# JettHuang/jet-pbrt

Hardware: AMD Instinct MI355X
Metric: Msamples/sec (whole node) + per-pixel L2 vs CPU ref, cornell_box 1024spp (higher is better)
Workload: dtype f32

## Files before the change

### jet-pbrt_amd/csrc/jp_common.h

```cpp
#pragma once
#include "jp_shading.h"

using namespace jp;

extern __shared__ float4 s_dyn[];

#define JP_SHADE_CLASSES 6

struct DevCounters
{
	unsigned int n_queue[2];
	unsigned int n_shadow;
	unsigned int pad;
	unsigned long long closest, closest_hit, shadow, shadow_occ;
	unsigned long long cert_fallback;
};

struct Queues
{
	float4 *ray_o[2], *ray_d[2], *beta[2];
	float2 *hit;
	float4 *lacc;
	float4 *sh_o;
	float4 *sh_d, *sh_c;
	unsigned int *blk_q[2], *blk_sh;
	unsigned int cap;
	unsigned int R;
};

struct RenderConst
{
	int width, height, spp, max_depth;
	unsigned int seed;
	int band_rows, shard_index, shard_count;
	int npix;
	int local_rows;
	int s0, sbatch;
	int n_planes;
	int tiled;
	int compact;
	int slot_bits;
	int sampler_debug;
	int class_mask;
	int lane_index, lane_count, lane_rows;
};

__device__ __forceinline__ float rngf(const RenderConst& rc, uint32_t key, uint32_t dim) { return rc.sampler_debug ? 0.5f : jp_rng_float(key, dim); }

#define FLAG_BOUNCE(f) ((f) & 0xff)
#define FLAG_SPEC(f)   (((f) >> 8) & 1)
#define FLAG_DIM(f)    (((unsigned)(f)) >> 16)
#define MK_FLAGS(bounce, spec, dim) (((bounce) & 0xff) | ((spec) ? 0x100 : 0) | ((int)(dim) << 16))

__device__ __forceinline__ void pixel_of(const RenderConst& rc, int pix, int& x, int& y)
{
	int lx, r;
	if (rc.tiled)
	{
		const int t = pix >> 6, i = pix & 63, tpr = rc.width >> 4;
		const int ty = t / tpr, tx = t - ty * tpr;
		lx = (tx << 4) + (i & 15); r = (ty << 2) + (i >> 4);
	}
	else { r = pix / rc.width; lx = pix - r * rc.width; }
	x = lx;
	if (rc.lane_count > 1) { const int m = r / rc.lane_rows; r = (rc.lane_index + m * rc.lane_count) * rc.lane_rows + (r - m * rc.lane_rows); }
	const int j = r / rc.band_rows;
	y = (rc.shard_index + j * rc.shard_count) * rc.band_rows + (r - j * rc.band_rows);
}

__device__ __forceinline__ unsigned int wave_take(unsigned int* ctr, unsigned int n)
{
	unsigned int v = 0;
	if ((threadIdx.x & 63) == 0) v = atomicAdd(ctr, n);
	return (unsigned int)__builtin_amdgcn_readfirstlane((int)v);
}


#define JP_TEX_IMAGE_TAG 0x80000000u
#define JP_TEX_COLOR_TAG 0x40000000u
struct TexView
{
	const int4* desc;
	const float4* col;
	const unsigned int* texels;
	const int* mat_tex;
	const float2* prim_uv;
	unsigned int* side;
};
```

### jet-pbrt_amd/csrc/jp_device.h

```cpp
#pragma once
#include <hip/hip_runtime.h>
#include <stdint.h>
#include "jetpbrt_amd.h"
#include "jp_counter_rng.h"

#define JP_BLOCK 256
#define JP_STACK_DEPTH 32

namespace jp
{
struct V3 { float x, y, z; };
__device__ __forceinline__ V3 mk(float x, float y, float z) { V3 v; v.x = x; v.y = y; v.z = z; return v; }
__device__ __forceinline__ V3 operator+(V3 a, V3 b) { return mk(a.x + b.x, a.y + b.y, a.z + b.z); }
__device__ __forceinline__ V3 operator-(V3 a, V3 b) { return mk(a.x - b.x, a.y - b.y, a.z - b.z); }
__device__ __forceinline__ V3 operator-(V3 a) { return mk(-a.x, -a.y, -a.z); }
__device__ __forceinline__ V3 operator*(V3 a, float s) { return mk(a.x * s, a.y * s, a.z * s); }
__device__ __forceinline__ V3 operator*(float s, V3 a) { return mk(a.x * s, a.y * s, a.z * s); }
__device__ __forceinline__ V3 operator/(V3 a, float s) { return mk(a.x / s, a.y / s, a.z / s); }
__device__ __forceinline__ V3 cmul(V3 a, V3 b) { return mk(a.x * b.x, a.y * b.y, a.z * b.z); }
__device__ __forceinline__ V3 cdiv(V3 a, V3 b) { return mk(a.x / b.x, a.y / b.y, a.z / b.z); }
__device__ __forceinline__ V3 splat(float v) { return mk(v, v, v); }
__device__ __forceinline__ V3 csqrt(V3 a) { return mk(sqrtf(a.x), sqrtf(a.y), sqrtf(a.z)); }
__device__ __forceinline__ float dot(V3 a, V3 b) { return a.x * b.x + a.y * b.y + a.z * b.z; }
__device__ __forceinline__ float len2(V3 a) { return a.x * a.x + a.y * a.y + a.z * a.z; }
__device__ __forceinline__ float len(V3 a) { return sqrtf(len2(a)); }
__device__ __forceinline__ V3 normalize(V3 a) { return a / len(a); }
__device__ __forceinline__ V3 cross(V3 a, V3 v) { return mk(a.y * v.z - a.z * v.y, a.z * v.x - a.x * v.z, a.x * v.y - a.y * v.x); }
__device__ __forceinline__ float absdot(V3 a, V3 b) { return fabsf(dot(a, b)); }
__device__ __forceinline__ bool isblack(V3 c) { return c.x == 0.f && c.y == 0.f && c.z == 0.f; }
__device__ __forceinline__ float smin(float a, float b) { return (b < a) ? b : a; }
__device__ __forceinline__ float smax(float a, float b) { return (a < b) ? b : a; }
__device__ __forceinline__ float maxcomp(V3 c) { float m = (c.y < c.z) ? c.z : c.y; return (c.x < m) ? m : c.x; }
__device__ __forceinline__ float clampf(float v, float lo, float hi) { if (v < lo) return lo; else if (v > hi) return hi; else return v; }
__device__ __forceinline__ V3 xyz(float4 v) { return mk(v.x, v.y, v.z); }

#define JP_PI      3.14159274101257324219f
#define JP_INF     __int_as_float(0x7f800000)

struct SceneView
{
	const float4* nodes; int n_nodes;
	const float4* prims; const int4* meta; int n_prims;
	const float4* mats;
	const int* mat_type; int n_mats;
	const float4* lights;
	int n_lights;
	const float4* shade_tab;
	float3 env_sum;
	int n_env;
	float world_radius;
	JpCamera cam;
	const float4* flat; int n_flat;
	const uint4* wide; int n_wide;
	const uint4* q4; int n_q4;
	const float4* refbox; float cert_pad, cert_pad_eye;
};

__device__ __forceinline__ bool tri_hit(V3 p0, V3 p1, V3 p2, V3 n, V3 o, V3 d, float tmin, float& tmax)
{
	const V3 oa = p0 - o;
	const float distance = dot(n, oa) / dot(n, d);
	if (!((distance > tmin) && (distance < tmax))) return false;
	const V3 ob = p1 - o, oc = p2 - o;
	const V3 v0 = cross(oc, ob), v1 = cross(ob, oa), v2 = cross(oa, oc);
	const float v0d = dot(v0, d), v1d = dot(v1, d), v2d = dot(v2, d);
	if (((v0d < 0) && (v1d < 0) && (v2d < 0)) || ((v0d >= 0) && (v1d >= 0) && (v2d >= 0))) { tmax = distance; return true; }
	return false;
}
__device__ __forceinline__ bool rect_hit(V3 p0, V3 p1, V3 p2, V3 p3, V3 n, V3 o, V3 d, float tmin, float& tmax)
{
	const V3 oa = p0 - o;
	const float distance = dot(n, oa) / dot(n, d);
	if (!((distance > tmin) && (distance < tmax))) return false;
	const V3 ob = p1 - o, oc = p2 - o, od = p3 - o;
	const V3 v0 = cross(oc, ob), v1 = cross(ob, oa), v2 = cross(oa, od), v3 = cross(od, oc);
	const float v0d = dot(v0, d), v1d = dot(v1, d), v2d = dot(v2, d), v3d = dot(v3, d);
	if (((v0d < 0) && (v1d < 0) && (v2d < 0) && (v3d < 0)) || ((v0d >= 0) && (v1d >= 0) && (v2d >= 0) && (v3d >= 0))) { tmax = distance; return true; }
	return false;
}
__device__ __forceinline__ bool sph_hit(V3 c, float r, V3 o, V3 d, float tmin, float& tmax)
{
	V3 oc = o - c;
	float a = len2(d);
	float half_b = dot(oc, d);
	float cc = len2(oc) - r * r;
	float disc = half_b * half_b - a * cc;
	if (disc > 0.0f)
	{
		float root = sqrtf(disc);
		float time;
		float root1 = (-half_b - root) / a;
		if (root1 < tmax && root1 > tmin) time = root1;
		else
		{
			float root2 = (-half_b + root) / a;
			if (root2 < tmax && root2 > tmin) time = root2;
			else return false;
		}
		tmax = time;
		return true;
	}
	return false;
}

__device__ __forceinline__ bool disk_hit(V3 c, float r, V3 n, V3 o, V3 d, float tmin, float& tmax)
{
	const float dn = dot(d, n);
	if (fabsf(dn - 0.f) <= 1.1920928955078125e-07f * smax(1.f, smax(fabsf(dn), fabsf(0.f)))) return false;
	const V3 op = c - o;
	const float distance = dot(n, op) / dot(n, d);
	if ((distance > tmin) && (distance < tmax))
	{
		const V3 hp = o + distance * d;
		if (len(c - hp) <= r) { tmax = distance; return true; }
	}
	return false;
}

template <int kS, typename PrimPtr>
__device__ __forceinline__ bool prim_hit(PrimPtr prims, int pi, V3 o, V3 d, float tmin, float& tmax)
{
	const float4 g0 = prims[kS * pi + 0], g1 = prims[kS * pi + 1], g2 = prims[kS * pi + 2], g3 = prims[kS * pi + 3];
	const int type = __float_as_int(g3.w);
	if (type == JP_SHAPE_TRIANGLE) return tri_hit(xyz(g0), xyz(g1), xyz(g2), xyz(g3), o, d, tmin, tmax);
	if (type == JP_SHAPE_SPHERE) return sph_hit(xyz(g0), g0.w, o, d, tmin, tmax);
	if (type == JP_SHAPE_DISK) return disk_hit(xyz(g0), g0.w, xyz(g1), o, d, tmin, tmax);
	return rect_hit(xyz(g0), xyz(g1), xyz(g2), mk(g0.w, g1.w, g2.w), xyz(g3), o, d, tmin, tmax);
}

template <bool kAnyHit, int kS, typename NodePtr, typename PrimPtr>
__device__ __forceinline__ int traverse(NodePtr nodes, PrimPtr prims, V3 o, V3 d, float tmin, float& tmax, int* stack)
{
	const float ix = 1.0f / d.x, iy = 1.0f / d.y, iz = 1.0f / d.z;
	int hit = -1, sp = 0, cur = 0;
	for (;;)
	{
		bool alive = true;
		while (cur >= 0)
		{
			const float4 n0 = nodes[kS * cur + 0], n1 = nodes[kS * cur + 1], n2 = nodes[kS * cur + 2], n3 = nodes[kS * cur + 3];
			const float lx0 = (n0.x - o.x) * ix, lx1 = (n0.w - o.x) * ix;
			const float ly0 = (n0.y - o.y) * iy, ly1 = (n1.x - o.y) * iy;
			const float lz0 = (n0.z - o.z) * iz, lz1 = (n1.y - o.z) * iz;
			const float ln = fmaxf(fmaxf(fminf(lx0, lx1), fminf(ly0, ly1)), fmaxf(fminf(lz0, lz1), tmin));
			const float lf = fminf(fminf(fmaxf(lx0, lx1), fmaxf(ly0, ly1)), fminf(fmaxf(lz0, lz1), tmax));
			const float rx0 = (n1.z - o.x) * ix, rx1 = (n2.y - o.x) * ix;
			const float ry0 = (n1.w - o.y) * iy, ry1 = (n2.z - o.y) * iy;
			const float rz0 = (n2.x - o.z) * iz, rz1 = (n2.w - o.z) * iz;
			const float rn = fmaxf(fmaxf(fminf(rx0, rx1), fminf(ry0, ry1)), fmaxf(fminf(rz0, rz1), tmin));
			const float rf = fminf(fminf(fmaxf(rx0, rx1), fmaxf(ry0, ry1)), fminf(fmaxf(rz0, rz1), tmax));
			const bool hl = ln <= lf * 1.000002f, hr = rn <= rf * 1.000002f;
			const int cl = __float_as_int(n3.x), cr = __float_as_int(n3.y);
			if (hl && hr)
			{
				const bool leftFirst = kAnyHit ? true : (ln <= rn);
				cur = leftFirst ? cl : cr;
				stack[sp * JP_BLOCK] = leftFirst ? cr : cl; sp++;
			}
			else if (hl) cur = cl;
			else if (hr) cur = cr;
			else if (sp > 0) { sp--; cur = stack[sp * JP_BLOCK]; }
			else { alive = false; break; }
		}
		if (!alive) break;
		const int e = -cur - 1, first = e >> 4, count = (e & 15) + 1;
		for (int k = 0; k < count; k++)
			if (prim_hit<kS>(prims, first + k, o, d, tmin, tmax)) { hit = first + k; if (kAnyHit) return hit; }
		if (sp > 0) { sp--; cur = stack[sp * JP_BLOCK]; } else break;
	}
	return hit;
}

__device__ __forceinline__ bool ref_box_exact(float4 n0, float4 n1, V3 o, V3 d, float tmin, float tmax)
{
	float bt0 = tmin, bt1 = tmax;
	{
		const float lo = (n0.x - o.x) / d.x, hi = (n1.x - o.x) / d.x;
		bt0 = smax(smin(lo, hi), bt0); bt1 = smin(smax(lo, hi), bt1);
		if (bt1 <= bt0) return false;
	}
	{
		const float lo = (n0.y - o.y) / d.y, hi = (n1.y - o.y) / d.y;
		bt0 = smax(smin(lo, hi), bt0); bt1 = smin(smax(lo, hi), bt1);
		if (bt1 <= bt0) return false;
	}
	{
		const float lo = (n0.z - o.z) / d.z, hi = (n1.z - o.z) / d.z;
		bt0 = smax(smin(lo, hi), bt0); bt1 = smin(smax(lo, hi), bt1);
		if (bt1 <= bt0) return false;
	}
	return true;
}
__device__ __forceinline__ bool ref_box(float4 n0, float4 n1, V3 o, V3 d, V3 rd, float tmin, float tmax)
{
	const float x0 = (n0.x - o.x) * rd.x, x1 = (n1.x - o.x) * rd.x;
	const float y0 = (n0.y - o.y) * rd.y, y1 = (n1.y - o.y) * rd.y;
	const float z0 = (n0.z - o.z) * rd.z, z1 = (n1.z - o.z) * rd.z;
	const float t0 = fmaxf(fmaxf(fminf(x0, x1), fminf(y0, y1)), fmaxf(fminf(z0, z1), tmin));
	const float t1 = fminf(fminf(fmaxf(x0, x1), fmaxf(y0, y1)), fminf(fmaxf(z0, z1), tmax));
	const float s = x0 + x1 + y0 + y1 + z0 + z1;
	const float margin = 2e-6f * (fabsf(t0) + fabsf(t1));
	const float gap = t1 - t0;
	if (fabsf(s) <= 3.0e38f && fabsf(gap) > margin) return gap > 0.f;
	return ref_box_exact(n0, n1, o, d, tmin, tmax);
}

template <bool kAnyHit>
__device__ __forceinline__ int traverse_ref(const float4* __restrict__ nodes, const float4* __restrict__ prims, V3 o, V3 d, float tmin, float& tmax, int* stack)
{
	const V3 rd = mk(__builtin_amdgcn_rcpf(d.x), __builtin_amdgcn_rcpf(d.y), __builtin_amdgcn_rcpf(d.z));
	int hit = -1, sp = 0, cur = 0;
	for (;;)
	{
		const float4 n0 = nodes[2 * cur], n1 = nodes[2 * cur + 1];
		const bool ok = ref_box(n0, n1, o, d, rd, tmin, tmax);
		const int left = __float_as_int(n0.w), right = __float_as_int(n1.w);
		if (ok && left >= 0) { stack[sp * JP_BLOCK] = right; sp++; cur = left; continue; }
		if (ok)
		{
			const int first = -left - 1;
			for (int k = 0; k < right; k++)
				if (prim_hit<4>(prims, first + k, o, d, tmin, tmax)) { hit = first + k; if (kAnyHit) return hit; }
		}
		if (sp == 0) break;
		sp--; cur = stack[sp * JP_BLOCK];
	}
	return hit;
}

typedef const __attribute__((address_space(4))) float* ConstFPtr;
typedef unsigned long long u64;
template <bool k64> struct FlatMask { typedef unsigned int type; };
template <> struct FlatMask<true> { typedef u64 type; };
template <bool k64> __device__ __forceinline__ int mask_count(typename FlatMask<k64>::type m) { return k64 ? __popcll((u64)m) : __popc((unsigned int)m); }

template <bool k64>
__device__ __forceinline__ typename FlatMask<k64>::type flat_boxes(const float4* flat_g, int n_flat, V3 o, V3 d, float tmin, float tmax)
{
	typedef typename FlatMask<k64>::type M;
	ConstFPtr flat = (ConstFPtr)flat_g;
	const float ix = __builtin_amdgcn_rcpf(d.x), iy = __builtin_amdgcn_rcpf(d.y), iz = __builtin_amdgcn_rcpf(d.z);
	M mask = 0;
	#define JP_FLAT_BOX(i) \
	{ \
		const float x0 = (flat[8 * (i) + 0] - o.x) * ix, x1 = (flat[8 * (i) + 4] - o.x) * ix; \
		const float y0 = (flat[8 * (i) + 1] - o.y) * iy, y1 = (flat[8 * (i) + 5] - o.y) * iy; \
		const float z0 = (flat[8 * (i) + 2] - o.z) * iz, z1 = (flat[8 * (i) + 6] - o.z) * iz; \
		const float tn = fmaxf(fmaxf(fminf(x0, x1), fminf(y0, y1)), fmaxf(fminf(z0, z1), tmin)); \
		const float tf = fminf(fminf(fmaxf(x0, x1), fmaxf(y0, y1)), fminf(fmaxf(z0, z1), tmax)); \
		M bits = (M)__float_as_uint(flat[8 * (i) + 3]); \
		if (k64) bits |= (M)((u64)__float_as_uint(flat[8 * (i) + 7]) << 32); \
		if (tn <= tf * 1.000002f) mask |= bits; \
	}
	int i0 = 0;
	for (; i0 + 4 <= n_flat; i0 += 4)
	{
		#pragma unroll
		for (int u = 0; u < 4; u++) JP_FLAT_BOX(i0 + u)
	}
	for (; i0 < n_flat; i0++) JP_FLAT_BOX(i0)
	#undef JP_FLAT_BOX
	return mask;
}

template <bool kAnyHit, bool k64, int kS, typename PrimPtr>
__device__ __forceinline__ int flat_prims(typename FlatMask<k64>::type mask, PrimPtr prims, V3 o, V3 d, float tmin, float& tmax)
{
	int hit = -1;
#ifdef JP_DBG_FLAT_P1ONLY
	mask = mask == (typename FlatMask<k64>::type)0x12345677u ? 1u : 0u;
#endif
	while (mask)
	{
		const int p = (k64 ? __ffsll((unsigned long long)mask) : __ffs((int)mask)) - 1;
		mask &= mask - 1;
		if (prim_hit<kS>(prims, p, o, d, tmin, tmax)) { hit = p; if (kAnyHit) return hit; }
	}
	return hit;
}

template <bool kAnyHit, int kS, typename PrimPtr>
__device__ __forceinline__ int traverse_flat(const float4* flat_g, int n_flat, int n_prims, PrimPtr prims, V3 o, V3 d, float tmin, float& tmax)
{
	if (n_prims > 32) return flat_prims<kAnyHit, true, kS>(flat_boxes<true>(flat_g, n_flat, o, d, tmin, tmax), prims, o, d, tmin, tmax);
	return flat_prims<kAnyHit, false, kS>(flat_boxes<false>(flat_g, n_flat, o, d, tmin, tmax), prims, o, d, tmin, tmax);
}

template <bool kAnyHit, typename PrimPtr>
__device__ __forceinline__ int traverse_wide(const uint4* __restrict__ wide, PrimPtr prims, V3 o, V3 d, float tmin, float& tmax, unsigned int* stack)
{
	const float ix = 1.0f / d.x, iy = 1.0f / d.y, iz = 1.0f / d.z;
	const unsigned int octinv = 7u - ((d.x < 0 ? 1u : 0u) | (d.y < 0 ? 2u : 0u) | (d.z < 0 ? 4u : 0u));
	unsigned int ngx = 0, ngy = 0x80000000u;
	int hit = -1, sp = 0;
	for (;;)
	{
		unsigned int tgx = 0, tgy = 0;
		if (ngy > 0x00ffffffu)
		{
			const unsigned int bit = 31u - (unsigned int)__clz((int)ngy);
			ngy &= ~(1u << bit);
			if (ngy > 0x00ffffffu) { stack[(2 * sp) * JP_BLOCK] = ngx; stack[(2 * sp + 1) * JP_BLOCK] = ngy; sp++; }
			const unsigned int slot = (bit - 24u) ^ octinv;
			const unsigned int rel = (unsigned int)__popc(ngy & 0xffu & ~(0xffffffffu << slot));
			const unsigned int idx = ngx + rel;
			const uint4 q0 = wide[5 * idx + 0], q1 = wide[5 * idx + 1], q2 = wide[5 * idx + 2], q3 = wide[5 * idx + 3], q4 = wide[5 * idx + 4];
			const float sx = __uint_as_float(((q0.w & 0xffu) ) << 23), sy = __uint_as_float(((q0.w >> 8) & 0xffu) << 23), sz = __uint_as_float(((q0.w >> 16) & 0xffu) << 23);
			const float px = __uint_as_float(q0.x) - o.x, py = __uint_as_float(q0.y) - o.y, pz = __uint_as_float(q0.z) - o.z;
			unsigned int hm = 0;
			#pragma unroll
			for (int i = 0; i < 8; i++)
			{
				const int sh = 8 * (i & 3);
				const unsigned int m = ((i < 4 ? q1.z : q1.w) >> sh) & 0xffu;
				const float lx = (float)(((i < 4 ? q2.x : q2.y) >> sh) & 0xffu), ly = (float)(((i < 4 ? q2.z : q2.w) >> sh) & 0xffu), lz = (float)(((i < 4 ? q3.x : q3.y) >> sh) & 0xffu);
				const float hx = (float)(((i < 4 ? q3.z : q3.w) >> sh) & 0xffu), hy = (float)(((i < 4 ? q4.x : q4.y) >> sh) & 0xffu), hz = (float)(((i < 4 ? q4.z : q4.w) >> sh) & 0xffu);
				const float x0 = fmaf(lx, sx, px) * ix, x1 = fmaf(hx, sx, px) * ix;
				const float y0 = fmaf(ly, sy, py) * iy, y1 = fmaf(hy, sy, py) * iy;
				const float z0 = fmaf(lz, sz, pz) * iz, z1 = fmaf(hz, sz, pz) * iz;
				const float tn = fmaxf(fmaxf(fminf(x0, x1), fminf(y0, y1)), fmaxf(fminf(z0, z1), tmin));
				const float tf = fminf(fminf(fmaxf(x0, x1), fmaxf(y0, y1)), fminf(fmaxf(z0, z1), tmax));
				if (m != 0u && tn <= tf * 1.000002f)
				{
					const bool inner = (m & 0x18u) == 0x18u;
					const unsigned int bits = inner ? 1u : (m >> 5), at = inner ? 24u + ((m & 7u) ^ octinv) : (m & 31u);
					hm |= bits << at;
				}
			}
			ngx = q1.x; ngy = (hm & 0xff000000u) | (q0.w >> 24);
			tgx = q1.y; tgy = hm & 0x00ffffffu;
		}
		while (tgy)
		{
			const int j = __ffs((int)tgy) - 1;
			tgy &= tgy - 1;
			if (prim_hit<4>(prims, (int)tgx + j, o, d, tmin, tmax)) { hit = (int)tgx + j; if (kAnyHit) return hit; }
		}
		if (ngy <= 0x00ffffffu)
		{
			if (sp == 0) break;
			sp--; ngx = stack[(2 * sp) * JP_BLOCK]; ngy = stack[(2 * sp + 1) * JP_BLOCK];
		}
	}
	return hit;
}

struct WalkStack
{
	int* lds; int* spill; int cap; unsigned int stride;
// ... 276 lines not shown
```

### jet-pbrt_amd/csrc/jp_kernels.hip

```cpp
#include "jp_common.h"
#include "jp_tex.h"
#include "jp_xbsdf.h"

#include <cstdio>
#include <cstring>
#include <string>
#include <vector>
#include <algorithm>
#include <cmath>
#include <mutex>
#include <thread>
#include "jp_lbvh.h"
#include "jp_ploc.h"

__global__ void __launch_bounds__(JP_BLOCK) k_raygen(SceneView sc, Queues q, RenderConst rc, DevCounters* cnt)
{
	const unsigned int total = (unsigned int)rc.npix * rc.sbatch;
	const unsigned int nchunks = (total + JP_BLOCK - 1) / JP_BLOCK;
	const unsigned int G = gridDim.x, b = blockIdx.x;
	if (b == 0 && threadIdx.x == 0) { cnt->n_queue[0] = total; cnt->n_queue[1] = 0; cnt->n_shadow = 0; }
	unsigned int filled = 0;
	const unsigned int K = (nchunks + G - 1) / G, npb = (unsigned int)rc.npix / JP_BLOCK;
	for (unsigned int k = 0, j0 = 0; k < K; k++, j0 += JP_BLOCK)
	{
		unsigned int c;
		if (rc.compact) { const unsigned int qi = b * K + k; if (qi >= nchunks) break; const unsigned int pb = qi / (unsigned int)rc.sbatch, sl = qi - pb * (unsigned int)rc.sbatch; c = sl * npb + pb; }
		else { c = b + k * G; if (c >= nchunks) break; }
		const unsigned int slot = c * JP_BLOCK + threadIdx.x;
		if (slot < total)
		{
			const unsigned int i = b * q.R + j0 + threadIdx.x;
			const int pix = slot % rc.npix, s = rc.s0 + slot / rc.npix;
			int x, y; pixel_of(rc, pix, x, y);
			const uint32_t key = jp_rng_key(rc.seed, (uint32_t)x, (uint32_t)y, (uint32_t)s);
			const float fx = (float)x + rngf(rc, key, 0), fy = (float)y + rngf(rc, key, 1);
			const V3 front = mk(sc.cam.front[0], sc.cam.front[1], sc.cam.front[2]);
			const V3 right = mk(sc.cam.right[0], sc.cam.right[1], sc.cam.right[2]);
			const V3 up = mk(sc.cam.up[0], sc.cam.up[1], sc.cam.up[2]);
			V3 dir = front + right * (fx / sc.cam.res_x - 0.5f) + up * (0.5f - fy / sc.cam.res_y);
			dir = normalize(dir);
			q.ray_o[0][i] = make_float4(sc.cam.pos[0], sc.cam.pos[1], sc.cam.pos[2], __int_as_float((int)slot));
			q.ray_d[0][i] = make_float4(dir.x, dir.y, dir.z, __int_as_float(MK_FLAGS(0, 0, 2)));
			q.beta[0][i] = make_float4(1.f, 1.f, 1.f, __int_as_float((int)key));
			q.lacc[slot] = make_float4(0.f, 0.f, 0.f, 0.f);
		}
		const unsigned int left = total - c * JP_BLOCK;
		filled += left < JP_BLOCK ? left : JP_BLOCK;
	}
	if (threadIdx.x == 0) q.blk_q[0][b] = filled;
}


#if defined(JP_SHADE_TIMING) || defined(JP_TRAV_TIMING)
__device__ unsigned long long g_shade_t[16];
#define JP_TSX(i) do { const unsigned long long t_ = __builtin_amdgcn_s_memtime(); t_acc[i] += t_ - t_last; t_last = t_; } while (0)
#endif
#ifdef JP_SHADE_TIMING
#define JP_TS(i) JP_TSX(i)
#else
#define JP_TS(i) do { } while (0)
#endif
#ifdef JP_TRAV_TIMING
#define JP_TT(i) JP_TSX(i)
#else
#define JP_TT(i) do { } while (0)
#endif
template <int kMode>
struct SceneAccess;
template <> struct SceneAccess<0>
{
	const float4 *nodes, *prims; int* stack; int depth;
	__device__ __forceinline__ SceneAccess(const SceneView& sc, int depth_) : nodes(sc.nodes), prims(sc.prims), stack((int*)s_dyn + threadIdx.x), depth(depth_) {}
	template <bool kAnyHit> __device__ __forceinline__ int trace(const SceneView&, V3 o, V3 d, float tmin, float& tmax) const
	{ return traverse<kAnyHit, 4>(nodes, prims, o, d, tmin, tmax, stack); }
};
template <> struct SceneAccess<1>
{
	float4 *nodes, *prims; int* stack; int depth;
	__device__ __forceinline__ SceneAccess(const SceneView& sc, int depth_) : depth(depth_)
	{
		stack = (int*)s_dyn + threadIdx.x;
		nodes = s_dyn + (depth * JP_BLOCK) / 4;
		prims = nodes + 5 * sc.n_nodes;
		for (int i = threadIdx.x; i < 4 * sc.n_nodes; i += JP_BLOCK) nodes[5 * (i >> 2) + (i & 3)] = sc.nodes[i];
		for (int i = threadIdx.x; i < 4 * sc.n_prims; i += JP_BLOCK) prims[5 * (i >> 2) + (i & 3)] = sc.prims[i];
		__syncthreads();
	}
	template <bool kAnyHit> __device__ __forceinline__ int trace(const SceneView&, V3 o, V3 d, float tmin, float& tmax) const
	{ return traverse<kAnyHit, 5>(nodes, prims, o, d, tmin, tmax, stack); }
};
template <> struct SceneAccess<2>
{
	float4* prims;
	__device__ __forceinline__ SceneAccess(const SceneView& sc, int)
	{
		prims = s_dyn;
		for (int i = threadIdx.x; i < 4 * sc.n_prims; i += JP_BLOCK) prims[5 * (i >> 2) + (i & 3)] = sc.prims[i];
		__syncthreads();
	}
	template <bool kAnyHit> __device__ __forceinline__ int trace(const SceneView& sc, V3 o, V3 d, float tmin, float& tmax) const
	{ return traverse_flat<kAnyHit, 5>(sc.flat, sc.n_flat, sc.n_prims, prims, o, d, tmin, tmax); }
};

template <> struct SceneAccess<3>
{
	const float4* prims; unsigned int* stack;
	__device__ __forceinline__ SceneAccess(const SceneView& sc, int) : prims(sc.prims), stack((unsigned int*)s_dyn + threadIdx.x) {}
	template <bool kAnyHit> __device__ __forceinline__ int trace(const SceneView& sc, V3 o, V3 d, float tmin, float& tmax) const
	{ return traverse_wide<kAnyHit>(sc.wide, prims, o, d, tmin, tmax, stack); }
};

template <> struct SceneAccess<4>
{
	WalkStack stack;
	__device__ __forceinline__ SceneAccess(const SceneView&, int depth) { stack.lds = (int*)s_dyn + threadIdx.x; stack.spill = nullptr; stack.cap = depth - 1; stack.stride = 0; }
	template <bool kAnyHit> __device__ __forceinline__ int trace(const SceneView& sc, V3 o, V3 d, float tmin, float& tmax) const
	{ return walk_ray<4, kAnyHit>(sc, o, d, tmin, tmax, stack); }
};

template <> struct SceneAccess<6>
{
	WalkStack stack;
	__device__ __forceinline__ SceneAccess(const SceneView&, int depth) { stack.lds = (int*)s_dyn + threadIdx.x; stack.spill = nullptr; stack.cap = depth - 1; stack.stride = 0; }
	template <bool kAnyHit> __device__ __forceinline__ int trace(const SceneView& sc, V3 o, V3 d, float tmin, float& tmax) const
	{ return walk_ray<6, kAnyHit>(sc, o, d, tmin, tmax, stack); }
};

template <> struct SceneAccess<5>
{
	const float4 *nodes, *prims; int* stack;
	__device__ __forceinline__ SceneAccess(const SceneView& sc, int) : nodes(sc.nodes), prims(sc.prims), stack((int*)s_dyn + threadIdx.x) {}
	template <bool kAnyHit> __device__ __forceinline__ int trace(const SceneView&, V3 o, V3 d, float tmin, float& tmax) const
	{ return traverse_ref<kAnyHit>(nodes, prims, o, d, tmin, tmax, stack); }
};

template <int kMode>
__global__ void __launch_bounds__(JP_BLOCK) k_extend(SceneView sc, Queues q, int cur, int depth, DevCounters* cnt)
{
	SceneAccess<kMode> acc(sc, depth);
	const unsigned int b = blockIdx.x, n = q.blk_q[cur][b], rbase = b * q.R;
	if (b == 0 && threadIdx.x == 0) { cnt->closest += cnt->n_queue[cur]; cnt->n_queue[cur ^ 1] = 0; cnt->n_shadow = 0; }
	unsigned int h = 0;
	float4 ro = make_float4(0, 0, 0, 0), rd = make_float4(0, 0, 1, 0);
	if (threadIdx.x < n) { ro = q.ray_o[cur][rbase + threadIdx.x]; rd = q.ray_d[cur][rbase + threadIdx.x]; }
	for (unsigned int j = threadIdx.x; j < n; j += JP_BLOCK)
	{
		const unsigned int i = rbase + j;
		const float4 co = ro, cd = rd;
		if (j + JP_BLOCK < n) { ro = q.ray_o[cur][i + JP_BLOCK]; rd = q.ray_d[cur][i + JP_BLOCK]; }
		float tmax = JP_INF;
		const int hit = acc.template trace<false>(sc, xyz(co), xyz(cd), 0.001f, tmax);
		q.hit[i] = make_float2(tmax, __int_as_float(hit));
		h += hit >= 0 ? 1u : 0u;
	}
	for (int off = 32; off > 0; off >>= 1) h += __shfl_down(h, off);
	if ((threadIdx.x & 63) == 0 && h) atomicAdd(&cnt->closest_hit, (unsigned long long)h);
}

#ifndef JP_SHADE_TILE
#define JP_SHADE_TILE 8192
#endif
template <bool kTab, bool kPrims, bool kStage, bool kSort, bool kTex>
__device__ __forceinline__ void shade_body(SceneView sc, Queues q, RenderConst rc, int cur, DevCounters* cnt, const TexView& tv)
{
	static_assert(kTab || !kPrims, "k_shade: primitive records in LDS only together with the tables");
	constexpr int kWaves = JP_BLOCK / 64, kMaxSeg = (JP_SHADE_TILE / JP_BLOCK) * kWaves;
	static_assert(JP_SHADE_TILE % JP_BLOCK == 0 && JP_SHADE_TILE <= 65536, "k_shade: tile positions are 16-bit");
	__shared__ unsigned short s_idx[kSort ? JP_SHADE_TILE : 1];
	__shared__ unsigned char s_key[kSort ? JP_SHADE_TILE : 1];
	__shared__ unsigned int s_cnt[kSort ? JP_SHADE_CLASSES * kMaxSeg : 1];
	__shared__ unsigned int s_wsum[kWaves];
	__shared__ unsigned int s_ctr[3];
	const unsigned int lane = threadIdx.x & 63u;
	const int n_tab = 2 * sc.n_lights + 4 * sc.n_mats + (sc.n_mats + 3) / 4, n_tab_all = n_tab + (kPrims ? 8 * sc.n_prims : 0);
	float4* s_lights = s_dyn;
	float4* s_mats = s_lights + 2 * sc.n_lights;
	int* s_mtype = (int*)(s_mats + 4 * sc.n_mats);
	float4* s_prims = s_dyn + n_tab;
	int4* s_meta = (int4*)(s_prims + 4 * sc.n_prims);
	const float4* s_frames = s_prims + 5 * sc.n_prims;
	float4* s_stage = s_dyn + n_tab_all + threadIdx.x;
	const unsigned int b = blockIdx.x, n = q.blk_q[cur][b];
	const int nxt = cur ^ 1;
#ifdef JP_SHADE_TIMING
	unsigned long long t_acc[10] = { 0, 0, 0, 0, 0, 0, 0, 0, 0, 0 }, t_last = __builtin_amdgcn_s_memtime();
#endif
	if (kTab)
	{
		for (int i = threadIdx.x; i < n_tab_all; i += 2 * JP_BLOCK)
		{
			const bool two = i + JP_BLOCK < n_tab_all;
			const float4 a = sc.shade_tab[i], c2 = two ? sc.shade_tab[i + JP_BLOCK] : a;
			s_dyn[i] = a; if (two) s_dyn[i + JP_BLOCK] = c2;
		}
	}
	if (n == 0) { if (threadIdx.x == 0) { q.blk_q[nxt][b] = 0; q.blk_sh[b] = 0; } return; }
	if (threadIdx.x == 0) { s_ctr[0] = 0; s_ctr[1] = 0; s_ctr[2] = 0; }
	__syncthreads();
	const float4* lights = kTab ? (const float4*)s_lights : sc.lights;
	const float4* mats = kTab ? (const float4*)s_mats : sc.mats;
	const int* mat_type = kTab ? (const int*)s_mtype : sc.mat_type;
	const float4* prims = kPrims ? (const float4*)s_prims : sc.prims;
	const int4* meta_t = kPrims ? (const int4*)s_meta : sc.meta;
	const unsigned int rbase = b * q.R;
	const unsigned int t0 = 0, count = n;
	JP_TS(0);
	if (kSort)
	{
		constexpr unsigned int seg = kMaxSeg, nctr = JP_SHADE_CLASSES * kMaxSeg;
		const unsigned int tid = threadIdx.x;
		const unsigned int plane = tid & 63u, wave = tid >> 6, npass = (count + JP_BLOCK - 1) / JP_BLOCK;
		const unsigned long long ltm = (1ull << plane) - 1ull;
		#pragma unroll 1
		for (unsigned int r0 = 0; r0 < npass; r0 += 8)
		{
			int pi[8];
			#pragma unroll
			for (int u = 0; u < 8; u++)
			{
				const unsigned int j = (r0 + u) * JP_BLOCK + tid;
				pi[u] = j < count ? __float_as_int(q.hit[rbase + t0 + j].y) : -2;
			}
			#pragma unroll
			for (int u = 0; u < 8; u++)
			{
				const unsigned int r = r0 + u;
				if (r >= npass) break;
				unsigned int key = JP_SHADE_CLASSES;
				if (pi[u] != -2)
				{
					int m = -1; if (pi[u] >= 0) m = meta_t[pi[u]].y;
					key = m >= 0 ? 1u + (unsigned int)mat_type[m] : 0u;
				}
				s_key[r * JP_BLOCK + tid] = (unsigned char)key;
				unsigned int mine = 0;
				#pragma unroll
				for (int c = 0; c < JP_SHADE_CLASSES; c++)
				{
					unsigned int nc = 0;
					if ((rc.class_mask >> c) & 1) nc = (unsigned int)__popcll(__ballot(key == (unsigned int)c));
					if (plane == (unsigned int)c) mine = nc;
				}
				if (plane < JP_SHADE_CLASSES) s_cnt[plane * seg + r * kWaves + wave] = mine;
			}
		}
		__syncthreads();
		{
			static_assert(JP_SHADE_CLASSES * kMaxSeg <= 3 * JP_BLOCK, "k_shade: three counters per thread");
			unsigned int v[3], t = 0;
			#pragma unroll
			for (int i = 0; i < 3; i++)
			{
				const unsigned int at = 3 * tid + i;
				v[i] = (at < nctr && (at % seg) / kWaves < npass) ? s_cnt[at] : 0u; t += v[i];
			}
			unsigned int incl = t;
			#pragma unroll
			for (int off = 1; off < 64; off <<= 1) { const unsigned int o = __shfl_up(incl, off); if (plane >= (unsigned int)off) incl += o; }
			if (plane == 63) s_wsum[wave] = incl;
			__syncthreads();
			unsigned int base = incl - t;
			#pragma unroll
			for (int w = 0; w < kWaves; w++) if ((unsigned int)w < wave) base += s_wsum[w];
			#pragma unroll
			for (int i = 0; i < 3; i++) { const unsigned int at = 3 * tid + i; if (at < nctr) s_cnt[at] = base; base += v[i]; }
		}
		__syncthreads();
		#pragma unroll 1
		for (unsigned int r = 0; r < npass; r++)
		{
			const unsigned int key = s_key[r * JP_BLOCK + tid];
			unsigned int pre = 0;
			#pragma unroll
			for (int c = 0; c < JP_SHADE_CLASSES; c++)
			{
				if (!((rc.class_mask >> c) & 1)) continue;
				const unsigned long long m = __ballot(key == (unsigned int)c);
				if (key == (unsigned int)c) pre = (unsigned int)__popcll(m & ltm);
			}
			if (key < JP_SHADE_CLASSES) s_idx[s_cnt[key * seg + r * kWaves + wave] + pre] = (unsigned short)(r * JP_BLOCK + tid);
		}
		__syncthreads();
	}
	float4 ro_n = make_float4(0, 0, 0, 0), rd_n = ro_n, rb_n = ro_n; float2 h_n = make_float2(0, 0); unsigned int s_n = 0;
	JP_TS(1);
	const unsigned int nch = (count + 63u) >> 6;
	unsigned int tk = wave_take(&s_ctr[0], 1u);
	unsigned int c0 = (nch - 1u - tk) << 6;
	if (tk < nch && c0 + lane < count) { const unsigned int pos = c0 + lane, i0 = rbase + t0 + (kSort ? (unsigned int)s_idx[pos] : pos); ro_n = q.ray_o[cur][i0]; rd_n = q.ray_d[cur][i0]; rb_n = q.beta[cur][i0]; h_n = q.hit[i0]; if (kTex) s_n = tv.side[i0]; }
	while (tk < nch)
	{
		const bool valid = c0 + lane < count;
#ifdef JP_SHADE_TIMING
		JP_TS(2);
		asm volatile("s_waitcnt vmcnt(0)" ::: "memory");
		JP_TS(3);
#endif
#ifdef JP_SHADE_NO_PREFETCH
		if (valid) { const unsigned int pos = c0 + lane, i0 = rbase + t0 + (kSort ? (unsigned int)s_idx[pos] : pos); ro_n = q.ray_o[cur][i0]; rd_n = q.ray_d[cur][i0]; rb_n = q.beta[cur][i0]; h_n = q.hit[i0]; if (kTex) s_n = tv.side[i0]; }
		const float4 ro = ro_n, rd = rd_n, rb = rb_n; const float2 h = h_n; const unsigned int sw = s_n;
		tk = wave_take(&s_ctr[0], 1u); c0 = (nch - 1u - tk) << 6;
#else
		const float4 ro = ro_n, rd = rd_n, rb = rb_n; const float2 h = h_n; const unsigned int sw = s_n;
		tk = wave_take(&s_ctr[0], 1u); c0 = (nch - 1u - tk) << 6;
		if (tk < nch && c0 + lane < count)
		{
			const unsigned int pos = c0 + lane;
			const unsigned int i1 = rbase + t0 + (kSort ? (unsigned int)s_idx[pos] : pos);
			ro_n = q.ray_o[cur][i1]; rd_n = q.ray_d[cur][i1]; rb_n = q.beta[cur][i1]; h_n = q.hit[i1]; if (kTex) s_n = tv.side[i1];
		}
#endif
		bool shaded = false, wantNee = false, alive = false;
		V3 o = mk(0, 0, 0), d = mk(0, 0, 1), beta = mk(0, 0, 0), p = mk(0, 0, 0), N = mk(0, 0, 1);
		int slot = 0, bounce = 0; bool spec = false; unsigned int dim = 0; uint32_t key = 0;
		Closure c; c.kind = CL_LAMBERT; Frame fr; fr.s = fr.t = fr.n = mk(0, 0, 1);
		if (valid)
		{
			o = xyz(ro); d = xyz(rd); beta = xyz(rb);
			slot = __float_as_int(ro.w); key = (uint32_t)__float_as_int(rb.w);
			const int flags = __float_as_int(rd.w);
			bounce = FLAG_BOUNCE(flags); spec = FLAG_SPEC(flags); dim = FLAG_DIM(flags);
			const int pi = __float_as_int(h.y);
			const bool found = pi >= 0;
			int mat = -1, hitprim = 0; bool nflip = false, tabframe = kPrims;
			V3 Le = splat(0);
			if (found)
			{
				const float4 g3 = prims[4 * pi + 3];
				const int4 meta = meta_t[pi];
				const int type = __float_as_int(g3.w);
				p = o + h.x * d;
				if (type == JP_SHAPE_TRIANGLE) N = xyz(g3);
				else if (type == JP_SHAPE_RECTANGLE) { nflip = !(dot(xyz(g3), d) <= 0); N = nflip ? -xyz(g3) : xyz(g3); }
				else if (type == JP_SHAPE_DISK) N = xyz(prims[4 * pi + 1]);
				else { const float4 g0 = prims[4 * pi]; N = normalize(p - xyz(g0)); tabframe = false; }
				hitprim = pi;
				mat = meta.y;
				if (meta.z >= 0 && (bounce == 0 || spec))
				{
					const V3 wo = -d;
					if (dot(N, wo) > 0.f) Le = xyz(lights[2 * meta.z]);
				}
			}
			else if (bounce == 0 || spec)
			{
				for (int li = 0; li < sc.n_lights; li++)
				{
					const float4 l0 = lights[2 * li];
					if (__float_as_int(l0.w) == JP_LIGHT_ENVIRONMENT && !isblack(xyz(l0)))
					{
						float4 L = q.lacc[slot];
						V3 a = mk(L.x, L.y, L.z) + cmul(beta, xyz(l0));
						q.lacc[slot] = make_float4(a.x, a.y, a.z, 0.f);
					}
				}
			}
			if (!isblack(Le))
			{
				float4 L = q.lacc[slot];
				V3 a = mk(L.x, L.y, L.z) + cmul(beta, Le);
				q.lacc[slot] = make_float4(a.x, a.y, a.z, 0.f);
			}
			if (found && bounce < rc.max_depth)
			{
				if (mat < 0) alive = true;
				else
				{
					float up = 0.f;
					const int mtype = mat_type[mat];
					if (mtype == JP_MAT_PLASTIC) up = rngf(rc, key, dim++);
					if (kTex && sw != 0u) make_closure_tex(mats, mtype, mat, up, tex_color(tv, sw), c);
					else make_closure(mats, mtype, mat, up, c);
#ifdef JP_DBG_SKIP_FRAME
					fr.n = N; fr.s = mk(N.y, N.z, N.x); fr.t = mk(N.z, N.x, N.y);
#else
					if (kPrims && tabframe)
					{
						const float4 fn = s_frames[3 * hitprim], fs = s_frames[3 * hitprim + 1], ft = s_frames[3 * hitprim + 2];
						fr.n = nflip ? -xyz(fn) : xyz(fn); fr.s = xyz(fs); fr.t = nflip ? -xyz(ft) : xyz(ft);
					}
					else fr = frame_from_z(N);
#endif
					shaded = true;
					wantNee = !is_delta(c);
#ifdef JP_DBG_SKIP_NEE
					wantNee = false;
#endif
				}
			}
		}
		JP_TS(4);
		unsigned int qs = 0;
		if (!kStage)
		{
			const unsigned long long mn = __ballot(wantNee);
			if (mn) qs = rbase + wave_take(&s_ctr[2], (unsigned int)__popcll(mn)) + (unsigned int)__popcll(mn & ((1ull << lane) - 1ull));
		}
		V3 nd = d, nbeta = beta; int nbounce = bounce; bool nspec = spec;
		V3 wo = mk(0, 0, 1);
		int k = 0;
		if (shaded)
		{
			const V3 wo_w = -d;
			wo = to_local(fr, wo_w);
			closure_set_wo(c, wo);
			if (wantNee)
			{
				for (int li = 0; li < sc.n_lights; li++)
				{
					const unsigned int d0 = dim; dim += 2;
					const float4 lrad = lights[2 * li];
					if (isblack(xyz(lrad))) continue;
					const float ux = rngf(rc, key, d0), uy = rngf(rc, key, d0 + 1);
					LightSample ls = sample_li(sc, prims, lights, li, p, N, ux, uy);
					if (isblack(ls.Li) || ls.pdf == 0.f) continue;
					const V3 f = eval_local(c, wo, to_local(fr, ls.wi));
					if (isblack(f)) continue;
					const V3 sdir = __float_as_int(lrad.w) == JP_LIGHT_AREA ? ls.wi : normalize(ls.pos - p);
					const float dist = ls.dist >= 0.f ? ls.dist : len(p - ls.pos);
					const V3 contrib = cmul(cmul(beta, f), ls.Li) * absdot(ls.wi, N) / ls.pdf;
					if (k < rc.n_planes)
					{
						if (kStage)
						{
							s_stage[(2 * k) * JP_BLOCK] = make_float4(sdir.x, sdir.y, sdir.z, dist - 0.001f);
							s_stage[(2 * k + 1) * JP_BLOCK] = make_float4(contrib.x, contrib.y, contrib.z, 0.f);
						}
						else
						{
							q.sh_d[(size_t)k * q.cap + qs] = make_float4(sdir.x, sdir.y, sdir.z, dist - 0.001f);
							q.sh_c[(size_t)k * q.cap + qs] = make_float4(contrib.x, contrib.y, contrib.z, 0.f);
						}
						k++;
					}
				}
				if (!kStage) q.sh_o[qs] = make_float4(p.x, p.y, p.z, __int_as_float(slot | (k << rc.slot_bits)));
			}
		}
		JP_TS(5);
#ifdef JP_DBG_SKIP_SAMPLE
		if (false)
#else
		if (shaded)
#endif
		{
			const float ux = rngf(rc, key, dim), uy = rngf(rc, key, dim + 1); dim += 2;
			BsdfSample bs = sample_local(c, wo, ux, uy);
			bs.wi = to_world(fr, bs.wi);
			if (!(isblack(bs.f) || bs.pdf == 0.f))
			{
				nspec = (bs.flags & BS_SPECULAR) != 0;
				if (bounce >= 3)
				{
					const float qq = smax(0.05f, 1 - maxcomp(bs.f));
					const float ur = rngf(rc, key, dim++);
					if (!(ur < qq))
					{
						nbeta = cmul(beta, bs.f * absdot(bs.wi, N) / (bs.pdf * (1 - qq)));
						alive = true;
					}
				}
				else
				{
					nbeta = cmul(beta, bs.f * absdot(bs.wi, N) / bs.pdf);
					alive = true;
				}
				nd = bs.wi; nbounce = bounce + 1;
			}
		}
		JP_TS(6);
		unsigned int j = 0;
		const unsigned long long lt = (1ull << lane) - 1ull;
		const unsigned long long ma = __ballot(alive);
		if (kStage)
		{
			const unsigned long long ms = __ballot(k > 0);
			if (ma | ms)
			{
				const unsigned int base = wave_take(&s_ctr[1], (unsigned int)__popcll(ma) | ((unsigned int)__popcll(ms) << 16));
				j = rbase + (base & 0xffffu) + (unsigned int)__popcll(ma & lt);
				qs = rbase + (base >> 16) + (unsigned int)__popcll(ms & lt);
			}
			if (k > 0)
			{
				q.sh_o[qs] = make_float4(p.x, p.y, p.z, __int_as_float(slot | (k << rc.slot_bits)));
				for (int kk = 0; kk < k; kk++)
				{
					q.sh_d[(size_t)kk * q.cap + qs] = s_stage[(2 * kk) * JP_BLOCK];
					q.sh_c[(size_t)kk * q.cap + qs] = s_stage[(2 * kk + 1) * JP_BLOCK];
				}
			}
		}
		else if (ma) j = rbase + wave_take(&s_ctr[1], (unsigned int)__popcll(ma)) + (unsigned int)__popcll(ma & lt);
		if (alive)
		{
			q.ray_o[nxt][j] = make_float4(p.x, p.y, p.z, __int_as_float(slot));
			q.ray_d[nxt][j] = make_float4(nd.x, nd.y, nd.z, __int_as_float(MK_FLAGS(nbounce, nspec, dim)));
			q.beta[nxt][j] = make_float4(nbeta.x, nbeta.y, nbeta.z, __int_as_float((int)key));
		}
		JP_TS(7);
#ifdef JP_SHADE_TIMING
		asm volatile("s_waitcnt vmcnt(0)" ::: "memory");
		JP_TS(9);
#endif
	}
	JP_TS(2);
	__syncthreads();
	JP_TS(8);
#ifdef JP_SHADE_TIMING
	if (lane == 0) for (int i = 0; i < 10; i++) atomicAdd(&g_shade_t[i], t_acc[i]);
	if (lane == 0) atomicAdd(&g_shade_t[15], 1ull);
#endif
	if (threadIdx.x == 0)
	{
		const unsigned int run_q = kStage ? (s_ctr[1] & 0xffffu) : s_ctr[1], run_sh = kStage ? (s_ctr[1] >> 16) : s_ctr[2];
		q.blk_q[nxt][b] = run_q; q.blk_sh[b] = run_sh;
		if (run_q) atomicAdd(&cnt->n_queue[nxt], run_q);
		if (run_sh) atomicAdd(&cnt->n_shadow, run_sh);
	}
}
template <bool kTab, bool kPrims, bool kStage, bool kSort>
__global__ void __launch_bounds__(JP_BLOCK) k_shade(SceneView sc, Queues q, RenderConst rc, int cur, DevCounters* cnt)
{
	const TexView tv = {};
	shade_body<kTab, kPrims, kStage, kSort, false>(sc, q, rc, cur, cnt, tv);
}

template <int kMode>
__global__ void __launch_bounds__(JP_BLOCK, 4) k_shadow(SceneView sc, Queues q, RenderConst rc, int depth, DevCounters* cnt)
{
#ifdef JP_TRAV_TIMING
	unsigned long long t_acc[10] = { 0, 0, 0, 0, 0, 0, 0, 0, 0, 0 }, t_last = __builtin_amdgcn_s_memtime();
#endif
	SceneAccess<kMode> acc(sc, depth);
	const unsigned int b = blockIdx.x, E = q.blk_sh[b], rbase = b * q.R;
	JP_TT(0);
	unsigned int rays = 0, occ = 0;
	float4 so_n = make_float4(0, 0, 0, 0), sd_n = make_float4(0, 0, 1, 0);
	if (threadIdx.x < E) { so_n = q.sh_o[rbase + threadIdx.x]; sd_n = q.sh_d[rbase + threadIdx.x]; }
	for (unsigned int j = threadIdx.x; j < E; j += JP_BLOCK)
	{
		const unsigned int e = rbase + j;
#ifdef JP_TRAV_TIMING
		JP_TT(1);
		asm volatile("s_waitcnt vmcnt(0)" ::: "memory");
		JP_TT(2);
#endif
		const float4 so = so_n; float4 sd = sd_n;
		if (j + JP_BLOCK < E) { so_n = q.sh_o[e + JP_BLOCK]; sd_n = q.sh_d[e + JP_BLOCK]; }
		const int packed = __float_as_int(so.w);
		const int slot = packed & ((1 << rc.slot_bits) - 1), n = (int)((unsigned int)packed >> rc.slot_bits);
		if (n == 0) continue;
		bool any = false;
		const float4 L = q.lacc[slot];
		V3 a = mk(L.x, L.y, L.z);
		for (int k = 0; k < n; k++)
		{
			const float4 c4 = q.sh_c[(size_t)k * q.cap + e];
			float tmax = sd.w;
			const V3 dir = xyz(sd);
			if (k + 1 < n) sd = q.sh_d[(size_t)(k + 1) * q.cap + e];
			JP_TT(3);
#ifdef JP_TRAV_TIMING
			int hit;
			if constexpr (kMode == 2)
			{
				const unsigned int m = flat_boxes<false>(sc.flat, sc.n_flat, xyz(so), dir, 0.001f, tmax);
				JP_TT(4);
				hit = flat_prims<true, false, 5>(m, acc.prims, xyz(so), dir, 0.001f, tmax);
				JP_TT(5);
			}
			else hit = acc.template trace<true>(sc, xyz(so), dir, 0.001f, tmax);
#else
			const int hit = acc.template trace<true>(sc, xyz(so), dir, 0.001f, tmax);
#endif
			rays++;
			if (hit >= 0) occ++;
			else { a = a + xyz(c4); any = true; }
			JP_TT(6);
		}
		if (any) q.lacc[slot] = make_float4(a.x, a.y, a.z, 0.f);
		JP_TT(7);
	}
#ifdef JP_TRAV_TIMING
	JP_TT(1);
	if ((threadIdx.x & 63) == 0) { for (int i = 0; i < 8; i++) atomicAdd(&g_shade_t[i], t_acc[i]); atomicAdd(&g_shade_t[15], 1ull); }
#endif
	for (int off = 32; off > 0; off >>= 1) { rays += __shfl_down(rays, off); occ += __shfl_down(occ, off); }
	if ((threadIdx.x & 63) == 0) { if (rays) atomicAdd(&cnt->shadow, (unsigned long long)rays); if (occ) atomicAdd(&cnt->shadow_occ, (unsigned long long)occ); }
}

template <int kMode, bool kAnyHit, bool kVote>
__device__ __forceinline__ void persist_turn(Walker<kMode>& w, const SceneView& sc, const WalkStack& stack, bool pool)
{
	const int nh = __popcll(__ballot(!w.done && w.heavy())), nl = __popcll(__ballot(!w.done && !w.heavy()));
	const bool heavyTurn = kVote ? nh > nl : w.heavy();
	if (kVote) { JP_TURN(heavyTurn ? 3 : 0, 1); JP_TURN(heavyTurn ? 4 : 1, heavyTurn ? nh : nl); JP_TURN(heavyTurn ? 5 : 2, nh + nl); if (!pool) { JP_TURN(8, 1); JP_TURN(9, nh + nl); JP_TURN(10, heavyTurn ? nh : nl); } }
	if (!w.done && (w.heavy() == heavyTurn)) w.template step<kAnyHit>(sc, stack);
}
__device__ __forceinline__ unsigned int lane_rank(unsigned long long m) { return __builtin_amdgcn_mbcnt_hi((unsigned int)(m >> 32), __builtin_amdgcn_mbcnt_lo((unsigned int)m, 0u)); }

#ifndef JP_CERT_WAVES
#define JP_CERT_WAVES 8
#endif
template <int kMode, int kRefill, bool kVote>
__global__ void __launch_bounds__(JP_BLOCK, (kMode == 6 ? JP_CERT_WAVES : 8)) k_extend_persist(SceneView sc, Queues q, int cur_q, int stack_cap, int* spill, DevCounters* cnt)
{
	__shared__ unsigned int s_next;
	const WalkStack stack = { (int*)s_dyn + threadIdx.x, spill + blockIdx.x * JP_BLOCK + threadIdx.x, (kMode == 4 || kMode == 6) ? stack_cap - 1 : stack_cap, gridDim.x * JP_BLOCK };
	const unsigned int b = blockIdx.x, n = q.blk_q[cur_q][b], rbase = b * q.R;
	if (b == 0 && threadIdx.x == 0) { cnt->closest += cnt->n_queue[cur_q]; cnt->n_queue[cur_q ^ 1] = 0; cnt->n_shadow = 0; }
	if (threadIdx.x == 0) s_next = 0;
	__syncthreads();
	const int lane = threadIdx.x & 63;
	Walker<kMode> w; w.done = true; w.hit = -1; w.tmax = JP_INF;
	unsigned int ridx = 0xffffffffu, h = 0;
	bool pool = n > 0;
	for (;;)
	{
		const unsigned long long idle = __ballot(w.done);
		const int nidle = __popcll(idle);
		if (nidle == 64 || (pool && nidle >= kRefill))
		{
			if (w.done && ridx != 0xffffffffu)
			{
				int hp = w.hit;
				if constexpr (kMode == 6) { if (!w.certain(sc)) hp = -2; }
				q.hit[rbase + ridx] = make_float2(w.tmax, __int_as_float(hp)); h += hp >= 0 ? 1u : 0u; ridx = 0xffffffffu;
			}
			if (!pool) break;
			const int first = __ffsll((long long)idle) - 1;
			unsigned int start = 0;
			if (lane == first) start = atomicAdd(&s_next, (unsigned int)nidle);
			start = __shfl(start, first);
			{ constexpr bool kAnyHit = false; (void)kAnyHit; JP_TURN(6, 1); JP_TURN(7, nidle); }
			pool = start + (unsigned int)nidle < n;
			if (w.done)
			{
				const unsigned int my = start + lane_rank(idle);
				if (my < n)
				{
					const float4 ro = q.ray_o[cur_q][rbase + my], rd = q.ray_d[cur_q][rbase + my];
					w.start(xyz(ro), xyz(rd), 0.001f, JP_INF);
					if constexpr (kMode == 6) w.mark_origin(sc);
					ridx = my;
				}
			}
			if (start >= n && nidle == 64) break;
			continue;
		}
		persist_turn<kMode, false, kVote>(w, sc, stack, pool);
	}
	if constexpr (kMode == 6)
	{
		__syncthreads();
		for (unsigned int i = threadIdx.x; i < n; i += JP_BLOCK)
		{
			if (__float_as_int(q.hit[rbase + i].y) != -2) continue;
			const float4 ro = q.ray_o[cur_q][rbase + i], rd = q.ray_d[cur_q][rbase + i];
			float tm = JP_INF;
// ... 395 lines not shown
```

### jet-pbrt_amd/csrc/jp_render.h

```cpp
#pragma once
namespace
{
enum { CLS_EXTEND = 0, CLS_SHADE = 1, CLS_SHADOW = 2, CLS_OTHER = 3, CLS_PATH = 4 };

int ensure_queues(JpContext* c, unsigned int cap, int planes, unsigned int nblocks)
{
	if (c->cap >= cap && c->planes_alloc >= planes && c->blk_alloc >= nblocks) return JP_OK;
	cap = std::max(cap, c->cap); planes = std::max(planes, c->planes_alloc); nblocks = std::max(nblocks, c->blk_alloc);
	free_queues(c); c->blk_alloc = 0;
	auto alloc = [&](void** p, size_t bytes) -> bool { if (hipMalloc(p, bytes) != hipSuccess) return false; c->qbufs.push_back(*p); return true; };
	Queues& q = c->q; bool ok = true;
	for (int b = 0; b < 2 && ok; b++) ok = alloc((void**)&q.ray_o[b], (size_t)cap * 16) && alloc((void**)&q.ray_d[b], (size_t)cap * 16) && alloc((void**)&q.beta[b], (size_t)cap * 16)
	                                       && alloc((void**)&q.blk_q[b], (size_t)nblocks * 4);
	ok = ok && alloc((void**)&q.hit, (size_t)cap * 8) && alloc((void**)&q.lacc, (size_t)cap * 16) && alloc((void**)&q.sh_o, (size_t)cap * 16)
	     && alloc((void**)&q.sh_d, (size_t)cap * 16 * planes) && alloc((void**)&q.sh_c, (size_t)cap * 16 * planes) && alloc((void**)&q.blk_sh, (size_t)nblocks * 4);
	if (!ok) { free_queues(c); return fail(JP_ERR_DEVICE, "jp_render: out of device memory for the path queues"); }
	c->cap = cap; c->planes_alloc = planes; c->blk_alloc = nblocks;
	return JP_OK;
}

struct Stamper
{
	JpContext* c; int cls; size_t a;
	Stamper(JpContext* c, int cls) : c(c), cls(cls), a(0)
	{
		if (!c->profiling) return;
		if (c->evused + 2 > c->evpool.size()) { size_t old = c->evpool.size(); c->evpool.resize(old + 64); for (size_t i = old; i < c->evpool.size(); i++) hipEventCreate(&c->evpool[i]); }
		a = c->evused; c->evused += 2;
		hipEventRecord(c->evpool[a], c->stream);
	}
	~Stamper() { if (!c->profiling) return; hipEventRecord(c->evpool[a + 1], c->stream); JpContext::Stamp s = { cls, a, a + 1 }; c->stamps.push_back(s); }
};

struct Shard { int band, count, index, local_rows, lane_rows; };
int shard_of(const JpRenderParams* rp, Shard& s, int lane_index = 0, int lane_count = 1, int lane_group = 4)
{
	if (rp->width <= 0 || rp->height <= 0 || rp->spp <= 0 || rp->max_depth < 0 || rp->max_depth > 200) return fail(JP_ERR_INVALID_ARGUMENT, "jp_render: bad width/height/spp/max_depth");
	if (rp->integrator < JP_INTEGRATOR_PATH || rp->integrator > JP_INTEGRATOR_DEBUG_NORMAL) return fail(JP_ERR_INVALID_ARGUMENT, "jp_render: unknown integrator");
	if (rp->integrator == JP_INTEGRATOR_WHITTED && rp->max_depth > JP_WHITTED_MAX_DEPTH) return fail(JP_ERR_UNSUPPORTED, "jp_render: the Whitted integrator supports max_depth <= 16");
	if (rp->sampler_mode != JP_SAMPLER_COUNTER && rp->sampler_mode != JP_SAMPLER_DEBUG) return fail(JP_ERR_UNSUPPORTED, "jp_render: the device path implements the counter sampler only (the sequential mt19937_64 stream is not reproducible in parallel)");
	s.band = rp->band_rows > 0 ? rp->band_rows : 20;
	s.count = rp->shard_count > 1 ? rp->shard_count : 1;
	s.index = s.count > 1 ? rp->shard_index : 0;
	if (s.index < 0 || s.index >= s.count) return fail(JP_ERR_INVALID_ARGUMENT, "jp_render: shard_index out of range");
	const int nbands = (rp->height + s.band - 1) / s.band;
	s.local_rows = 0;
	for (int b = s.index; b < nbands; b += s.count) s.local_rows += std::min(s.band, rp->height - b * s.band);
	s.lane_rows = 0;
	for (int g0 = lane_index * lane_group; g0 < s.local_rows; g0 += lane_count * lane_group) s.lane_rows += std::min(lane_group, s.local_rows - g0);
	return JP_OK;
}

inline bool refill_walks(const ScenePlan& p) { return p.persist && (p.trav_mode == 0 || p.trav_mode == 3 || p.trav_mode == 5); }
inline int refill_row(const ScenePlan& p) { return p.persist >= 32 ? 2 : (p.persist >= 16 ? 1 : 0); }
inline int extend_depth(const ScenePlan& p) { return (p.trav_mode == 5 ? p.cert : p.use_q4) ? p.stack_depth_q4 : p.stack_depth; }
inline int shadow_depth(const ScenePlan& p) { return (p.trav_mode == 5 ? p.cert : p.q4_shadow) ? p.stack_depth_q4 : (p.trav_mode == 3 ? (int)(p.lds_bytes_shadow / (JP_BLOCK * sizeof(int))) : p.stack_depth); }
inline int deepest_walk(const ScenePlan& p) { return std::max(std::max(p.stack_depth, p.stack_depth_q4), p.trav_mode == 3 ? (int)(p.lds_bytes_shadow / (JP_BLOCK * sizeof(int))) : 0); }
inline size_t spill_need(const ScenePlan& p, int deep, unsigned int G) { return deep >= p.stack_lds_words ? (size_t)(deep - p.stack_lds_words + 1) * G * JP_BLOCK : 1; }

typedef void (*ExtendKernel)(SceneView, Queues, int, int, DevCounters*);
typedef void (*ExtendRefillKernel)(SceneView, Queues, int, int, int*, DevCounters*);
struct ExtendLaunch { ExtendRefillKernel refill; ExtendKernel plain; size_t lds; int words; };
template <int M> ExtendRefillKernel extend_refill(const ScenePlan& p)
{
	static const ExtendRefillKernel k[3][2] = { { k_extend_persist<M, 8, false>, k_extend_persist<M, 8, true> }, { k_extend_persist<M, 16, false>, k_extend_persist<M, 16, true> }, { k_extend_persist<M, 32, false>, k_extend_persist<M, 32, true> } };
	return k[refill_row(p)][p.vote];
}
ExtendLaunch extend_kernel(const ScenePlan& p)
{
	if (!refill_walks(p)) return { nullptr, p.trav_mode == 5 ? k_extend<5> : (p.trav_mode == 2 ? k_extend<2> : (p.trav_mode == 1 ? k_extend<1> : k_extend<0>)), p.lds_bytes, p.stack_depth };
	const int words = std::min(extend_depth(p), p.stack_lds_words);
	const ExtendRefillKernel k = p.trav_mode == 5 ? (p.cert ? extend_refill<6>(p) : extend_refill<5>(p)) : (p.use_q4 ? extend_refill<4>(p) : extend_refill<0>(p));
	return { k, nullptr, (size_t)words * JP_BLOCK * sizeof(int), words };
}

typedef void (*ShadowKernel)(SceneView, Queues, RenderConst, int, DevCounters*);
typedef void (*ShadowRefillKernel)(SceneView, Queues, RenderConst, int, int*, DevCounters*);
struct ShadowLaunch { ShadowRefillKernel refill; ShadowKernel plain; size_t lds; int words; bool cert_fell_back; };
template <int M> ShadowRefillKernel shadow_refill(const ScenePlan& p)
{
	static const ShadowRefillKernel k[3][2] = { { k_shadow_persist<M, 8, false>, k_shadow_persist<M, 8, true> }, { k_shadow_persist<M, 16, false>, k_shadow_persist<M, 16, true> }, { k_shadow_persist<M, 32, false>, k_shadow_persist<M, 32, true> } };
	return k[refill_row(p)][p.vote];
}
ShadowLaunch shadow_kernel(const ScenePlan& p, unsigned int R)
{
	const int words = std::min(shadow_depth(p), p.stack_lds_words);
	const size_t plds = (size_t)words * JP_BLOCK * sizeof(int) + (((size_t)R * p.n_planes + 31) / 32) * 4 * (p.cert ? 2 : 1);
	if (!refill_walks(p) || plds > 64 * 1024)
		return { nullptr, p.trav_mode == 3 ? k_shadow<3> : (p.trav_mode == 5 ? k_shadow<5> : (p.trav_mode == 2 ? k_shadow<2> : (p.trav_mode == 1 ? k_shadow<1> : k_shadow<0>))), p.trav_mode == 3 ? p.lds_bytes_shadow : p.lds_bytes, p.stack_depth, p.cert };
	const ShadowRefillKernel k = p.trav_mode == 5 ? (p.cert ? shadow_refill<6>(p) : shadow_refill<5>(p)) : (p.q4_shadow ? shadow_refill<4>(p) : (p.trav_mode == 3 ? shadow_refill<3>(p) : shadow_refill<0>(p)));
	return { k, nullptr, plds, words, false };
}

typedef void (*ShadeKernel)(SceneView, Queues, RenderConst, int, DevCounters*);
typedef void (*ShadeTexKernel)(SceneView, Queues, RenderConst, int, DevCounters*, TexView);
struct ShadeKernels { ShadeKernel plain; ShadeTexKernel tex; };
template <bool kTab, bool kPrims, bool kStage> ShadeKernels shade_row(bool sort)
{
	ShadeKernels k = { sort ? k_shade<kTab, kPrims, kStage, true> : k_shade<kTab, kPrims, kStage, false>, sort ? k_shade_tex<kTab, kPrims, kStage, true> : k_shade_tex<kTab, kPrims, kStage, false> };
	return k;
}
ShadeKernels shade_kernels(const ScenePlan& p)
{
	if (p.shade_prims_in_lds) return p.stage_nee ? shade_row<true, true, true>(p.shade_sort) : shade_row<true, true, false>(p.shade_sort);
	if (p.tables_in_lds) return p.stage_nee ? shade_row<true, false, true>(p.shade_sort) : shade_row<true, false, false>(p.shade_sort);
	return shade_row<false, false, false>(p.shade_sort);
}

typedef void (*OtherKernel)(SceneView, Queues, RenderConst, int, int, DevCounters*);
OtherKernel other_kernel(const ScenePlan& p) { return p.trav_mode == 5 ? k_other<5> : (p.trav_mode == 2 ? k_other<2> : (p.trav_mode == 1 ? k_other<1> : k_other<0>)); }

typedef void (*TraceKernel)(SceneView, int, int, const float*, const float*, const float*, const float*, int*, float*, int*, float*);
typedef void (*SurfaceKernel)(SceneView, TexView, int, int, const float*, const float*, const float*, const float*, int*, float*, float*);
struct TraceLaunch { TraceKernel trace; SurfaceKernel surface; size_t lds; int depth; };
template <int M> TraceLaunch trace_row(size_t lds, int depth) { TraceLaunch t = { k_trace<M>, k_surface<M>, lds, depth }; return t; }
TraceLaunch trace_kernel(const ScenePlan& p, int tw)
{
	const size_t q4lds = (size_t)p.stack_depth_q4 * JP_BLOCK * sizeof(int);
	if (p.trav_mode == 3 && tw == 2) { TraceLaunch t = { k_trace<3>, nullptr, p.lds_bytes_shadow, p.stack_depth }; return t; }
	if (p.trav_mode == 5 && p.cert && q4lds <= 64 * 1024 && tw != 3) return trace_row<6>(q4lds, p.stack_depth_q4);
	if (p.trav_mode == 5) return trace_row<5>(p.lds_bytes, p.stack_depth);
	if (p.use_q4 && q4lds <= 64 * 1024 && tw != 1) return trace_row<4>(q4lds, p.stack_depth_q4);
	return p.trav_mode == 2 ? trace_row<2>(p.lds_bytes, p.stack_depth) : (p.trav_mode == 1 ? trace_row<1>(p.lds_bytes, p.stack_depth) : trace_row<0>(p.lds_bytes, p.stack_depth));
}

int render_one(JpContext* c, const JpRenderParams* rp, float* film_dev, bool sync, int lane_index = 0, int lane_count = 1, int lane_group = 4, bool ev0_recorded = false)
{
	if (!c->plan.have_scene) return fail(JP_ERR_NO_SCENE, "jp_render: no scene uploaded");
	const ScenePlan& p = c->plan; Shard sh;
	if (const int e = shard_of(rp, sh, lane_index, lane_count, lane_group); e != JP_OK) return e;
	HIP_TRY(hipSetDevice(c->device));
	const long long npix = (long long)sh.lane_rows * rp->width;

	if (!ev0_recorded) HIP_TRY(hipEventRecord(c->ev0, c->stream));
	HIP_TRY(hipMemsetAsync(film_dev, 0, sizeof(float) * 3 * (size_t)rp->width * rp->height, c->stream));
	HIP_TRY(hipMemsetAsync(c->d_cnt, 0, sizeof(DevCounters), c->stream));
	c->evused = 0; c->stamps.clear();
	unsigned long long samples = 0;
	if (npix > 0)
	{
		if (npix > (1 << 24)) return fail(JP_ERR_UNSUPPORTED, "jp_render: more than 2^24 pixels per shard");
		const int slot_bits = p.n_planes <= 31 ? 27 : 24;
		const unsigned int PMAX = slot_bits == 27 ? (1u << 26) : (1u << 24);
		size_t freeB = 0, totalB = 0; hipMemGetInfo(&freeB, &totalB);
		const size_t per = 136 + 32 * (size_t)p.n_planes;
		size_t budget = std::min<size_t>((size_t)24 << 30, (freeB / (size_t)std::max(1, lane_count) + (c->cap ? (size_t)c->cap * (136 + 32 * (size_t)c->planes_alloc) : 0)) / 2);
		if (c->opt.max_slots > 0) budget = std::min<size_t>(budget, (size_t)c->opt.max_slots * per);
		int sbatch = 1; unsigned int P = 0, G = 1, R = JP_BLOCK, cap = 0;
		for (int attempt = 0;; attempt++)
		{
			const unsigned int pcap = (unsigned int)std::min<size_t>(PMAX, std::max<size_t>((size_t)npix, budget / per));
			sbatch = (int)std::max<long long>(1, std::min<long long>(rp->spp, pcap / npix));
			{
				const int nb = (rp->spp + sbatch - 1) / sbatch;
				sbatch = (rp->spp + nb - 1) / nb;
			}
			if ((long long)sbatch * npix > (long long)PMAX) return fail(JP_ERR_UNSUPPORTED, "jp_render: shard too large for one batch");
			P = (unsigned int)((long long)sbatch * npix);
			const unsigned int nchunks = (P + JP_BLOCK - 1) / JP_BLOCK;
			G = std::max(1u, std::min(nchunks, (unsigned int)(c->n_cus * c->blocks_per_cu)));
			G = std::max(G, (nchunks + JP_SHADE_TILE / JP_BLOCK - 1) / (JP_SHADE_TILE / JP_BLOCK));
			R = ((nchunks + G - 1) / G) * JP_BLOCK;
			cap = G * R;
			const int st = ensure_queues(c, cap, p.n_planes, G);
			if (st == JP_OK) break;
			if (sbatch <= 1 || attempt >= 6) return st;
			budget = (size_t)sbatch / 2 * (size_t)npix * per;
		}
		c->q.cap = cap; c->q.R = R;
		const bool tex = p.textured && rp->integrator == JP_INTEGRATOR_PATH;
		if (tex && c->side_n < cap)
		{
			if (c->d_side) { HIP_TRY(hipStreamSynchronize(c->stream)); hipFree(c->d_side); } c->d_side = nullptr; c->side_n = 0;
			HIP_TRY(hipMalloc((void**)&c->d_side, (size_t)cap * sizeof(unsigned int))); c->side_n = cap;
		}
		TexView tv = p.tv; tv.side = c->d_side;
		const size_t need = spill_need(p, p.persist ? deepest_walk(p) : 0, G);
		if (c->spill_words < need) { if (c->d_spill) hipFree(c->d_spill); c->d_spill = nullptr; HIP_TRY(hipMalloc((void**)&c->d_spill, need * sizeof(int))); c->spill_words = need; }
		if (c->pix_acc_n < (size_t)npix) { if (c->d_pix_acc) hipFree(c->d_pix_acc); c->d_pix_acc = nullptr; HIP_TRY(hipMalloc((void**)&c->d_pix_acc, (size_t)npix * 16)); c->pix_acc_n = (size_t)npix; }

		RenderConst rc; rc.width = rp->width; rc.height = rp->height; rc.spp = rp->spp; rc.max_depth = rp->max_depth; rc.seed = rp->seed;
		rc.band_rows = sh.band; rc.shard_index = sh.index; rc.shard_count = sh.count; rc.npix = (int)npix; rc.local_rows = sh.lane_rows; rc.n_planes = p.n_planes;
		rc.lane_index = lane_index; rc.lane_count = lane_count; rc.lane_rows = lane_group; rc.class_mask = p.class_mask; rc.sampler_debug = rp->sampler_mode == JP_SAMPLER_DEBUG ? 1 : 0;
		rc.slot_bits = slot_bits;
		rc.tiled = 0;
		rc.compact = (p.trav_mode != 2 && p.trav_mode != 1 && npix % JP_BLOCK == 0) ? 1 : 0;
		if (c->opt.compact_regions != 0) rc.compact = (c->opt.compact_regions > 0 && npix % JP_BLOCK == 0) ? 1 : 0;
		const int grid = (int)G;
		const ExtendLaunch ek = extend_kernel(p); const ShadowLaunch sk = shadow_kernel(p, R); const ShadeKernels hk = shade_kernels(p); const OtherKernel ok = other_kernel(p);
		for (int s0 = 0; s0 < rp->spp; s0 += sbatch)
		{
			rc.s0 = s0; rc.sbatch = std::min(sbatch, rp->spp - s0);
			{ Stamper t(c, CLS_OTHER); hipLaunchKernelGGL(k_raygen, dim3(grid), dim3(JP_BLOCK), 0, c->stream, p.sv, c->q, rc, c->d_cnt); }
			if (rp->integrator != JP_INTEGRATOR_PATH)
			{
				Stamper t(c, CLS_OTHER);
				const int ogrid = (int)std::min<unsigned int>((P + JP_BLOCK - 1) / JP_BLOCK, (unsigned int)(c->n_cus * 16));
				hipLaunchKernelGGL(ok, dim3(ogrid), dim3(JP_BLOCK), p.lds_bytes, c->stream, p.sv, c->q, rc, rp->integrator, p.stack_depth, c->d_cnt);
			}
			int cur = 0;
			int iters = rp->integrator != JP_INTEGRATOR_PATH ? 0 : rp->max_depth + 1;
			for (int it = 0;; it++)
			{
				if (it >= iters)
				{
					if (rp->integrator != JP_INTEGRATOR_PATH || !p.has_null_material || it > iters + 64) break;
					DevCounters h; HIP_TRY(hipMemcpyAsync(&h, c->d_cnt, sizeof(h), hipMemcpyDeviceToHost, c->stream)); HIP_TRY(hipStreamSynchronize(c->stream));
					if (h.n_queue[cur] == 0) break;
				}
				{
					Stamper t(c, CLS_EXTEND);
					if (ek.refill) hipLaunchKernelGGL(ek.refill, dim3(grid), dim3(JP_BLOCK), ek.lds, c->stream, p.sv, c->q, cur, ek.words, c->d_spill, c->d_cnt);
					else hipLaunchKernelGGL(ek.plain, dim3(grid), dim3(JP_BLOCK), ek.lds, c->stream, p.sv, c->q, cur, ek.words, c->d_cnt);
				}
				{
					Stamper t(c, CLS_SHADE);
					if (tex)
					{
						hipLaunchKernelGGL(k_texel, dim3(grid), dim3(JP_BLOCK), 0, c->stream, p.sv, c->q, cur, tv);
						hipLaunchKernelGGL(hk.tex, dim3(grid), dim3(JP_BLOCK), p.shade_lds_bytes, c->stream, p.sv, c->q, rc, cur, c->d_cnt, tv);
					}
					else hipLaunchKernelGGL(hk.plain, dim3(grid), dim3(JP_BLOCK), p.shade_lds_bytes, c->stream, p.sv, c->q, rc, cur, c->d_cnt);
				}
				HIP_TRY(hipGetLastError());
				if (it < rp->max_depth || p.has_null_material)
				{
					Stamper t(c, CLS_SHADOW);
					if (sk.cert_fell_back) c->cert_fell_back = true;
					if (sk.refill) hipLaunchKernelGGL(sk.refill, dim3(grid), dim3(JP_BLOCK), sk.lds, c->stream, p.sv, c->q, rc, sk.words, c->d_spill, c->d_cnt);
					else hipLaunchKernelGGL(sk.plain, dim3(grid), dim3(JP_BLOCK), sk.lds, c->stream, p.sv, c->q, rc, sk.words, c->d_cnt);
					HIP_TRY(hipGetLastError());
				}
				cur ^= 1;
			}
			{ Stamper t(c, CLS_OTHER); hipLaunchKernelGGL(k_resolve, dim3((unsigned int)std::min<long long>(c->n_cus * 8, (npix + JP_BLOCK - 1) / JP_BLOCK)), dim3(JP_BLOCK), 0, c->stream, c->q, rc, c->d_pix_acc, film_dev, s0 == 0 ? 1 : 0, s0 + rc.sbatch >= rp->spp ? 1 : 0); }
			samples += (unsigned long long)rc.sbatch * (unsigned long long)npix;
		}
		HIP_TRY(hipGetLastError());
	}
	HIP_TRY(hipEventRecord(c->ev1, c->stream));
	c->own_samples = samples;
	if (sync) HIP_TRY(hipStreamSynchronize(c->stream));
	return JP_OK;
}

__global__ void __launch_bounds__(JP_BLOCK) k_add_film(float* __restrict__ dst, const float* __restrict__ src, size_t n)
{
	for (size_t i = (size_t)blockIdx.x * JP_BLOCK + threadIdx.x; i < n; i += (size_t)gridDim.x * JP_BLOCK) dst[i] += src[i];
}

int make_lanes(JpContext* c, int extra)
{
	if (!c->ev_added && hipEventCreateWithFlags(&c->ev_added, hipEventDisableTiming) != hipSuccess) return fail(JP_ERR_DEVICE, "jp_render: event allocation failed");
	while ((int)c->lanes.size() < extra)
	{
		JpContext* l = new JpContext;
		l->device = c->device; l->is_lane = true; l->n_cus = c->n_cus; l->blocks_per_cu = c->blocks_per_cu; l->opt = c->opt; l->opt_env = c->opt_env;
		std::memset(&l->counters, 0, sizeof(l->counters)); std::memset(&l->q, 0, sizeof(l->q));
		if (hipStreamCreateWithFlags(&l->stream, hipStreamNonBlocking) != hipSuccess || hipEventCreate(&l->ev0) != hipSuccess || hipEventCreate(&l->ev1) != hipSuccess
		    || hipMalloc((void**)&l->d_cnt, sizeof(DevCounters)) != hipSuccess)
		{ jp_destroy_context(l); return fail(JP_ERR_DEVICE, "jp_render: stream/event allocation for an extra lane failed"); }
		c->lanes.push_back(l);
	}
	return JP_OK;
}

void sync_lane_scene(JpContext* c, JpContext* l)
{
	l->plan = c->plan;
	if (!l->plan.textured && l->d_side) { hipStreamSynchronize(l->stream); hipFree(l->d_side); l->d_side = nullptr; l->side_n = 0; }
	l->profiling = c->profiling; l->opt = c->opt;
}

bool fused_eligible(const JpContext* c, const JpRenderParams* rp)
{
	if (c->opt.fused <= 0) return false;
	if (c->is_lane || !c->plan.have_scene || rp->integrator != JP_INTEGRATOR_PATH) return false;
	if (!c->plan.tables_in_lds || c->plan.n_planes > 4) return false;
	if (c->plan.cert) return false;
	if (c->plan.textured) return false;
	if (c->plan.trav_mode == 2) return c->plan.shade_prims_in_lds;
	return c->plan.trav_mode == 0 || c->plan.trav_mode == 3 || c->plan.trav_mode == 5;
}

typedef void (*PathKernel)(SceneView, Queues, RenderConst, PathConst, int*, DevCounters*);
PathKernel path_kernel(const ScenePlan& p)
{
	const bool so = p.shade_sort;
	switch (p.trav_mode)
	{
	case 2: return so ? k_path<2, 2, true, true, true> : k_path<2, 2, true, false, true>;
	case 3:
		if (p.use_q4) return p.q4_shadow ? (so ? k_path<4, 4, false, true, true> : k_path<4, 4, false, false, true>) : (so ? k_path<4, 3, false, true, true> : k_path<4, 3, false, false, true>);
		return so ? k_path<0, 3, false, true, true> : k_path<0, 3, false, false, true>;
	case 5: return so ? k_path<5, 5, false, true, false> : k_path<5, 5, false, false, false>;
	default:
		if (p.use_q4) return so ? k_path<4, 4, false, true, true> : k_path<4, 4, false, false, true>;
		return so ? k_path<0, 0, false, true, true> : k_path<0, 0, false, false, true>;
	}
}

int render_fused(JpContext* c, const JpRenderParams* rp, float* film_dev, bool sync)
{
	const ScenePlan& p = c->plan; Shard sh;
	if (const int e = shard_of(rp, sh); e != JP_OK) return e;
	HIP_TRY(hipSetDevice(c->device));
	const long long npix = (long long)sh.local_rows * rp->width;

	HIP_TRY(hipEventRecord(c->ev0, c->stream));
	HIP_TRY(hipMemsetAsync(film_dev, 0, sizeof(float) * 3 * (size_t)rp->width * rp->height, c->stream));
	HIP_TRY(hipMemsetAsync(c->d_cnt, 0, sizeof(DevCounters), c->stream));
	c->evused = 0; c->stamps.clear();
	unsigned long long samples = 0;
	c->last_fused = 1; c->last_lanes = 1;
	if (npix > 0)
	{
		if (npix > (1 << 24)) return fail(JP_ERR_UNSUPPORTED, "jp_render: more than 2^24 pixels per shard");
		const PathKernel kern = path_kernel(p);
		const bool flat = p.trav_mode == 2;
		const int modeE = flat ? 2 : (p.trav_mode == 5 ? 5 : 0);
		size_t freeB = 0, totalB = 0; hipMemGetInfo(&freeB, &totalB);
		size_t budget = std::min<size_t>((size_t)4 << 30, (freeB + c->flacc_n * 16) / 4);
		if (c->opt.max_slots > 0) budget = std::min<size_t>(budget, (size_t)c->opt.max_slots * 16);
		const size_t PMAX = (size_t)1 << 26;
		const size_t pcap = std::min<size_t>(PMAX, std::max<size_t>((size_t)npix, budget / 16));
		int sbatch = (int)std::max<long long>(1, std::min<long long>(rp->spp, (long long)(pcap / (size_t)npix)));
		{ const int nb = (rp->spp + sbatch - 1) / sbatch; sbatch = (rp->spp + nb - 1) / nb; }
		unsigned int R = 1024;
		{ const int v = c->opt.fused_region; if (v >= JP_BLOCK && v <= 8192) R = (unsigned int)(v / JP_BLOCK) * JP_BLOCK; }
		int S = 16;
		{ const int v = c->opt.fused_job_spp; if (v >= 1 && v <= 128) S = v; }
		const int n_tab = 2 * p.sv.n_lights + 4 * p.sv.n_mats + (p.sv.n_mats + 3) / 4, n_tab_all = n_tab + (flat ? 8 * p.sv.n_prims : 0);
		const int deepE = extend_depth(p), deepS = shadow_depth(p);
		const int ecap = flat ? 0 : std::min(deepE, p.stack_lds_words), scap = flat ? 0 : std::min(deepS, p.stack_lds_words);
		PathLds L = path_lds_layout(modeE, n_tab_all, p.sv.n_prims, R, p.n_planes, ecap, scap, p.shade_sort);
		while (L.total > 64 * 1024 && R > JP_BLOCK) { R -= JP_BLOCK; L = path_lds_layout(modeE, n_tab_all, p.sv.n_prims, R, p.n_planes, ecap, scap, p.shade_sort); }
		if (L.total > 64 * 1024) return fail(JP_ERR_UNSUPPORTED, "jp_render: the fused schedule's LDS layout does not fit this scene (JETPBRT_FUSED=0 selects the per-bounce launches)");
		S = std::max(1, std::min(S, std::min(sbatch, (int)(R / 64))));
		int PG = (int)(R / (unsigned int)S); if (PG >= 64) PG &= ~63;
		if ((long long)PG > npix) PG = (int)npix;
		const int npg = (int)((npix + PG - 1) / PG), nsb = (sbatch + S - 1) / S;
		const unsigned long long njobs = (unsigned long long)npg * nsb;
		if (njobs >= (1ull << 32)) return fail(JP_ERR_UNSUPPORTED, "jp_render: too many jobs per batch");
		HIP_TRY(hipFuncSetAttribute((const void*)kern, hipFuncAttributeMaxDynamicSharedMemorySize, (int)L.total));
		int per_cu = 0;
		HIP_TRY(hipOccupancyMaxActiveBlocksPerMultiprocessor(&per_cu, (const void*)kern, JP_BLOCK, L.total));
		per_cu = std::max(1, per_cu);
		{ const int v = c->opt.fused_workgroups; if (v >= 1 && v <= 16) per_cu = v; }
		const unsigned int G = (unsigned int)std::min<unsigned long long>(njobs, (unsigned long long)c->n_cus * per_cu);
		const unsigned int cap = G * R;
		if (c->fcap < cap || c->fplanes < p.n_planes)
		{
			HIP_TRY(hipStreamSynchronize(c->stream));
			const unsigned int ncap = std::max(cap, c->fcap); const int npl = std::max(p.n_planes, c->fplanes);
			const size_t keep_lacc = c->flacc_n; float4* keep = c->fq.lacc;
			for (void* p : c->fbufs) if (p != (void*)keep) hipFree(p);
			c->fbufs.clear(); if (keep) c->fbufs.push_back(keep);
			c->fcap = 0; c->fplanes = 0;
			Queues& q = c->fq; float4* lacc = keep; std::memset(&q, 0, sizeof(q)); q.lacc = lacc; c->flacc_n = keep_lacc;
			auto alloc = [&](void** p, size_t bytes) -> bool { if (hipMalloc(p, bytes) != hipSuccess) return false; c->fbufs.push_back(*p); return true; };
			bool ok = true;
			for (int b = 0; b < 2 && ok; b++) ok = alloc((void**)&q.ray_o[b], (size_t)ncap * 16) && alloc((void**)&q.ray_d[b], (size_t)ncap * 16) && alloc((void**)&q.beta[b], (size_t)ncap * 16);
			ok = ok && alloc((void**)&q.sh_o, (size_t)ncap * 16) && alloc((void**)&q.sh_d, (size_t)ncap * 16 * npl) && alloc((void**)&q.sh_c, (size_t)ncap * 16 * npl);
			if (!ok) { free_fused(c); return fail(JP_ERR_DEVICE, "jp_render: out of device memory for the region queues"); }
			c->fcap = ncap; c->fplanes = npl;
		}
		const size_t P = (size_t)sbatch * (size_t)npix;
		if (c->flacc_n < P)
		{
			HIP_TRY(hipStreamSynchronize(c->stream));
			if (c->fq.lacc) { c->fbufs.erase(std::remove(c->fbufs.begin(), c->fbufs.end(), (void*)c->fq.lacc), c->fbufs.end()); hipFree(c->fq.lacc); c->fq.lacc = nullptr; c->flacc_n = 0; }
			void* pl = nullptr; if (hipMalloc(&pl, P * 16) != hipSuccess) return fail(JP_ERR_DEVICE, "jp_render: out of device memory for the batch's radiance array");
			c->fq.lacc = (float4*)pl; c->fbufs.push_back(pl); c->flacc_n = P;
		}
		c->fq.cap = c->fcap; c->fq.R = R;
		const int nbatches = (rp->spp + sbatch - 1) / sbatch;
		if (c->jobs_n < (size_t)nbatches) { HIP_TRY(hipStreamSynchronize(c->stream)); if (c->d_jobs) hipFree(c->d_jobs); c->d_jobs = nullptr; c->jobs_n = 0; HIP_TRY(hipMalloc((void**)&c->d_jobs, (size_t)nbatches * 4)); c->jobs_n = (size_t)nbatches; }
		HIP_TRY(hipMemsetAsync(c->d_jobs, 0, (size_t)nbatches * 4, c->stream));
		const size_t need = spill_need(p, flat ? 0 : std::max(deepE, deepS), G);
		if (c->spill_words < need) { HIP_TRY(hipStreamSynchronize(c->stream)); if (c->d_spill) hipFree(c->d_spill); c->d_spill = nullptr; c->spill_words = 0; HIP_TRY(hipMalloc((void**)&c->d_spill, need * sizeof(int))); c->spill_words = need; }
		if (c->pix_acc_n < (size_t)npix) { HIP_TRY(hipStreamSynchronize(c->stream)); if (c->d_pix_acc) hipFree(c->d_pix_acc); c->d_pix_acc = nullptr; HIP_TRY(hipMalloc((void**)&c->d_pix_acc, (size_t)npix * 16)); c->pix_acc_n = (size_t)npix; }

		RenderConst rc; std::memset(&rc, 0, sizeof(rc));
		rc.width = rp->width; rc.height = rp->height; rc.spp = rp->spp; rc.max_depth = rp->max_depth; rc.seed = rp->seed;
		rc.band_rows = sh.band; rc.shard_index = sh.index; rc.shard_count = sh.count; rc.npix = (int)npix; rc.local_rows = sh.local_rows; rc.n_planes = p.n_planes;
		rc.lane_index = 0; rc.lane_count = 1; rc.lane_rows = 4; rc.class_mask = p.class_mask; rc.sampler_debug = rp->sampler_mode == JP_SAMPLER_DEBUG ? 1 : 0;
		rc.slot_bits = JP_PATH_LI_BITS;
		rc.tiled = (rp->width % 16 == 0 && sh.local_rows % 4 == 0 && PG % 64 == 0 && p.trav_mode != 2) ? 1 : 0;
		PathConst pc; pc.R = R; pc.PG = PG; pc.S = S; pc.npg = npg; pc.nsb = nsb; pc.ecap = ecap; pc.scap = scap;
		pc.max_iters = rp->max_depth + 1 + (p.has_null_material ? 64 : 0);
		c->last_region = (int)R; c->last_wgs = (int)G;
		for (int s0 = 0, bi = 0; s0 < rp->spp; s0 += sbatch, bi++)
		{
			rc.s0 = s0; rc.sbatch = std::min(sbatch, rp->spp - s0);
			pc.nsb = (rc.sbatch + S - 1) / S; pc.job = c->d_jobs + bi;
			const unsigned int g = (unsigned int)std::min<unsigned long long>((unsigned long long)npg * pc.nsb, (unsigned long long)G);
			{ Stamper t(c, CLS_PATH); hipLaunchKernelGGL(kern, dim3(g), dim3(JP_BLOCK), L.total, c->stream, p.sv, c->fq, rc, pc, c->d_spill, c->d_cnt); }
			HIP_TRY(hipGetLastError());
			{ Stamper t(c, CLS_OTHER); hipLaunchKernelGGL(k_resolve, dim3((unsigned int)std::min<long long>(c->n_cus * 8, (npix + JP_BLOCK - 1) / JP_BLOCK)), dim3(JP_BLOCK), 0, c->stream, c->fq, rc, c->d_pix_acc, film_dev, s0 == 0 ? 1 : 0, s0 + rc.sbatch >= rp->spp ? 1 : 0); }
			HIP_TRY(hipGetLastError());
			samples += (unsigned long long)rc.sbatch * (unsigned long long)npix;
		}
	}
	HIP_TRY(hipEventRecord(c->ev1, c->stream));
	c->own_samples = samples;
	if (sync) HIP_TRY(hipStreamSynchronize(c->stream));
	return JP_OK;
}

int render_impl(JpContext* c, const JpRenderParams* rp, float* film_dev, bool sync)
{
	if (!c || !rp || !film_dev) return fail(JP_ERR_INVALID_ARGUMENT, "jp_render: null argument");
	c->last_lanes = 1; c->last_fused = 0; c->last_textured = 0;
	if (c->plan.textured && rp->integrator == JP_INTEGRATOR_WHITTED) return fail(JP_ERR_UNSUPPORTED, "jp_render: the Whitted integrator does not sample textures (scene uploaded by jp_upload_scene_textured)");
	if (fused_eligible(c, rp)) return render_fused(c, rp, film_dev, sync);
	c->last_textured = c->plan.textured && rp->integrator == JP_INTEGRATOR_PATH ? 1 : 0;
	int forcedL = 0, group = 4;
	if (c->opt.lanes >= 1 && c->opt.lanes <= 4) forcedL = c->opt.lanes;
	if (c->opt.lane_rows >= 1 && c->opt.lane_rows <= 64) group = c->opt.lane_rows;
	int L = 1; Shard sh;
	if (!c->is_lane && c->plan.have_scene && !c->plan.has_null_material && rp->integrator == JP_INTEGRATOR_PATH && shard_of(rp, sh) == JP_OK)
	{
		const long long rows = sh.local_rows, groups = (rows + group - 1) / group;
		if (forcedL) L = (int)std::min<long long>(forcedL, std::max<long long>(1, groups));
		else
		{
			const long long samples = rows * rp->width * (long long)rp->spp;
			if (groups >= 3 && samples >= (2ll << 24)) L = 3;
			else if (groups >= 2 && samples >= (2ll << 24)) L = 2;
		}
	}
	if (L <= 1) return render_one(c, rp, film_dev, sync);

	HIP_TRY(hipSetDevice(c->device));
	int st = make_lanes(c, L - 1); if (st != JP_OK) return st;
	const size_t n = (size_t)rp->width * rp->height * 3;
	HIP_TRY(hipEventRecord(c->ev0, c->stream));
	const int bpc_single = c->blocks_per_cu, bpc_lane = c->bpc_from_env ? c->blocks_per_cu : std::max(4, 16 / L);
	for (int k = 1; k < L && st == JP_OK; k++)
	{
		JpContext* l = c->lanes[k - 1];
		sync_lane_scene(c, l);
		if (l->film_n < n) { if (l->d_film) { HIP_TRY(hipStreamSynchronize(c->stream)); hipFree(l->d_film); } l->d_film = nullptr; l->film_n = 0; HIP_TRY(hipMalloc((void**)&l->d_film, n * sizeof(float))); l->film_n = n; c->added_valid = false; }
		if (c->added_valid) HIP_TRY(hipStreamWaitEvent(l->stream, c->ev_added, 0));
		l->blocks_per_cu = bpc_lane;
		st = render_one(l, rp, l->d_film, false, k, L, group);
	}
	if (st == JP_OK) { c->blocks_per_cu = bpc_lane; st = render_one(c, rp, film_dev, false, 0, L, group, true); c->blocks_per_cu = bpc_single; }
	if (st != JP_OK) return st;
	for (int k = 1; k < L; k++)
	{
		JpContext* l = c->lanes[k - 1];
		HIP_TRY(hipStreamWaitEvent(c->stream, l->ev1, 0));
		hipLaunchKernelGGL(k_add_film, dim3((unsigned int)std::min<size_t>((size_t)c->n_cus * 8, (n + JP_BLOCK - 1) / JP_BLOCK)), dim3(JP_BLOCK), 0, c->stream, film_dev, (const float*)l->d_film, n);
	}
	HIP_TRY(hipEventRecord(c->ev_added, c->stream)); c->added_valid = true;
	HIP_TRY(hipEventRecord(c->ev1, c->stream));
	c->last_lanes = L;
	if (sync) HIP_TRY(hipStreamSynchronize(c->stream));
	return JP_OK;
}

int finish_one(JpContext* c, JpCounters& o)
{
	HIP_TRY(hipStreamSynchronize(c->stream));
	DevCounters h; HIP_TRY(hipMemcpy(&h, c->d_cnt, sizeof(h), hipMemcpyDeviceToHost));
	o.closest_rays += h.closest; o.closest_hits += h.closest_hit; o.shadow_rays += h.shadow; o.shadow_occluded += h.shadow_occ; o.certified_fallback_rays += h.cert_fallback;
	for (const JpContext::Stamp& s : c->stamps)
	{
		float t = 0.f; if (hipEventElapsedTime(&t, c->evpool[s.a], c->evpool[s.b]) != hipSuccess) continue;
		if (s.cls == CLS_EXTEND) { o.extend_ms += t; o.extend_launches++; }
		else if (s.cls == CLS_SHADE) { o.shade_ms += t; o.shade_launches++; }
		else if (s.cls == CLS_SHADOW) { o.shadow_ms += t; o.shadow_launches++; }
		else if (s.cls == CLS_PATH) { o.path_ms += t; o.path_launches++; }
		else o.other_ms += t;
	}
	return JP_OK;
}

int finish_counters(JpContext* c)
{
	HIP_TRY(hipSetDevice(c->device));
	JpCounters& o = c->counters;
	unsigned long long samples = c->own_samples;
	std::memset(&o, 0, sizeof(o));
	int st = finish_one(c, o); if (st != JP_OK) return st;
	for (int k = 1; k < c->last_lanes; k++)
	{ samples += c->lanes[k - 1]->own_samples; st = finish_one(c->lanes[k - 1], o); if (st != JP_OK) return st; }
	float ms = 0.f; if (hipEventElapsedTime(&ms, c->ev0, c->ev1) != hipSuccess) ms = 0.f;
	o.render_ms = ms; o.samples = samples;
	return JP_OK;
}
}

extern "C" {

int jp_render_device(JpContext* c, const JpRenderParams* rp, void* film_rgb_device, int sync) { return render_impl(c, rp, (float*)film_rgb_device, sync != 0); }

int jp_render(JpContext* c, const JpRenderParams* rp, float* film_host)
{
	if (!c || !rp || !film_host) return fail(JP_ERR_INVALID_ARGUMENT, "jp_render: null argument");
	if (rp->width <= 0 || rp->height <= 0) return fail(JP_ERR_INVALID_ARGUMENT, "jp_render: bad width/height");
	HIP_TRY(hipSetDevice(c->device));
	size_t n = (size_t)rp->width * rp->height * 3;
	if (c->film_n < n) { if (c->d_film) hipFree(c->d_film); c->d_film = nullptr; HIP_TRY(hipMalloc((void**)&c->d_film, n * sizeof(float))); c->film_n = n; }
	if (c->h_film_n < n) { if (c->h_film) hipHostFree(c->h_film); c->h_film = nullptr; c->h_film_n = 0; if (hipHostMalloc((void**)&c->h_film, n * sizeof(float), hipHostMallocDefault) == hipSuccess) c->h_film_n = n; else c->h_film = nullptr; }
	int st = render_impl(c, rp, c->d_film, false); if (st != JP_OK) return st;
	float* stage = c->h_film ? c->h_film : film_host;
	HIP_TRY(hipMemcpyAsync(stage, c->d_film, n * sizeof(float), hipMemcpyDeviceToHost, c->stream));
	HIP_TRY(hipStreamSynchronize(c->stream));
	if (stage != film_host) std::memcpy(film_host, stage, n * sizeof(float));
	return JP_OK;
}

int jp_render_rgb8(JpContext* c, const JpRenderParams* rp, uint8_t* rgb8_host, float* film_host)
{
	if (!c || !rp || !rgb8_host) return fail(JP_ERR_INVALID_ARGUMENT, "jp_render_rgb8: null argument");
	if (rp->width <= 0 || rp->height <= 0) return fail(JP_ERR_INVALID_ARGUMENT, "jp_render_rgb8: bad width/height");
	HIP_TRY(hipSetDevice(c->device));
	const size_t n = (size_t)rp->width * rp->height * 3;
	if (c->film_n < n) { if (c->d_film) hipFree(c->d_film); c->d_film = nullptr; HIP_TRY(hipMalloc((void**)&c->d_film, n * sizeof(float))); c->film_n = n; }
	if (c->rgb8_n < n) { if (c->d_rgb8) hipFree(c->d_rgb8); c->d_rgb8 = nullptr; c->rgb8_n = 0; HIP_TRY(hipMalloc((void**)&c->d_rgb8, n)); c->rgb8_n = n; }
	if (c->h_rgb8_n < n) { if (c->h_rgb8) hipHostFree(c->h_rgb8); c->h_rgb8 = nullptr; c->h_rgb8_n = 0; if (hipHostMalloc((void**)&c->h_rgb8, n, hipHostMallocDefault) == hipSuccess) c->h_rgb8_n = n; else c->h_rgb8 = nullptr; }
	if (!c->d_gamma) { HIP_TRY(hipMalloc((void**)&c->d_gamma, 255 * sizeof(float))); HIP_TRY(hipMemcpy(c->d_gamma, host_gamma_thresholds(), 255 * sizeof(float), hipMemcpyHostToDevice)); }
	int st = render_impl(c, rp, c->d_film, false); if (st != JP_OK) return st;
	hipLaunchKernelGGL(k_tonemap8, dim3((unsigned int)std::min<size_t>((size_t)c->n_cus * 8, (n + JP_BLOCK - 1) / JP_BLOCK)), dim3(JP_BLOCK), 0, c->stream, (const float*)c->d_film, c->d_rgb8, (const float*)c->d_gamma, n);
	unsigned char* stage = c->h_rgb8 ? c->h_rgb8 : rgb8_host;
	HIP_TRY(hipMemcpyAsync(stage, c->d_rgb8, n, hipMemcpyDeviceToHost, c->stream));
	if (film_host) HIP_TRY(hipMemcpyAsync(film_host, c->d_film, n * sizeof(float), hipMemcpyDeviceToHost, c->stream));
	HIP_TRY(hipStreamSynchronize(c->stream));
	if (stage != rgb8_host) std::memcpy(rgb8_host, stage, n);
	return JP_OK;
}

int jp_synchronize(JpContext* c) { if (!c) return fail(JP_ERR_INVALID_ARGUMENT, "jp_synchronize: null context"); HIP_TRY(hipSetDevice(c->device)); HIP_TRY(hipStreamSynchronize(c->stream)); return JP_OK; }
int jp_set_profiling(JpContext* c, int enabled) { if (!c) return fail(JP_ERR_INVALID_ARGUMENT, "jp_set_profiling: null context"); c->profiling = enabled != 0; return JP_OK; }
int jp_get_counters(JpContext* c, JpCounters* out)
{
// ... 163 lines not shown
```

### jet-pbrt_amd/csrc/jp_runtime.h

```cpp
#pragma once

static thread_local std::string g_err;
static int fail(int code, const std::string& msg) { g_err = msg; return code; }
#define HIP_TRY(expr) do { hipError_t _e = (expr); if (_e != hipSuccess) return fail(JP_ERR_DEVICE, std::string(#expr) + ": " + hipGetErrorString(_e)); } while (0)

static inline bool opt_flag(int v, bool dflt) { return v == 0 ? dflt : v > 0; }

static void options_from_environment(JpOptions& o)
{
	struct Item { const char* name; int kind; void* field; int as; };
	const Item items[] = {
		{ "JETPBRT_LANES", 0, &o.lanes, 0 }, { "JETPBRT_LANE_ROWS", 0, &o.lane_rows, 0 }, { "JETPBRT_BLOCKS_PER_CU", 0, &o.blocks_per_cu, 0 }, { "JETPBRT_MAX_SLOTS", 3, &o.max_slots, 0 },
		{ "JETPBRT_COMPACT_REGIONS", 1, &o.compact_regions, 0 }, { "JETPBRT_FUSED", 1, &o.fused, 0 }, { "JETPBRT_REGION", 0, &o.fused_region, 0 }, { "JETPBRT_JOB_SPP", 0, &o.fused_job_spp, 0 },
		{ "JETPBRT_FUSED_WGS", 0, &o.fused_workgroups, 0 }, { "JETPBRT_TRAVERSAL", 6, &o.traversal, 0 }, { "JETPBRT_Q4", 1, &o.q4, 0 }, { "JETPBRT_Q4_SHADOW", 1, &o.q4_shadow, 0 },
		{ "JETPBRT_PERSIST", 2, &o.persist, 0 }, { "JETPBRT_VOTE", 1, &o.vote, 0 }, { "JETPBRT_STACK_LDS", 0, &o.stack_lds_words, 0 }, { "JETPBRT_SHADE_SORT", 1, &o.shade_sort, 0 },
		{ "JETPBRT_DEVICE_TREE", 4, &o.device_tree, 0 }, { "JETPBRT_DEVICE_WIDE", 1, &o.device_wide, 0 }, { "JETPBRT_BVH_MAXLEAF", 0, &o.bvh_max_leaf, 0 },
		{ "JETPBRT_PLOC_RADIUS", 0, &o.ploc_radius, 0 }, { "JETPBRT_PLOC_MAX_ROUNDS", 0, &o.ploc_max_rounds, 0 }, { "JETPBRT_CERTIFIED", 1, &o.certified, 0 },
		{ "JETPBRT_CERT_SLACK", 7, &o.cert_slack, 0 }, { "JETPBRT_CERT_SLACK_EYE", 7, &o.cert_slack_eye, 0 }, { "JETPBRT_CERT_EYE", 7, &o.cert_eye_tau, 0 },
		{ "JETPBRT_SINCOSF", 2, &o.libm_sincosf, 0 }, { "JETPBRT_LIBM", 2, &o.libm_xbsdf, 0 },
		{ "JETPBRT_TRACE_BINARY", 5, &o.trace_walk, 1 }, { "JETPBRT_TRACE_WIDE", 5, &o.trace_walk, 2 }, { "JETPBRT_TRACE_VERBATIM", 5, &o.trace_walk, 3 }, { "JETPBRT_BOX_PAD", 7, &o.box_pad, 0 },
	};
	for (const Item& it : items)
	{
		const char* e = getenv(it.name);
		if (!e || !*e) continue;
		switch (it.kind)
		{
			case 0: *(int32_t*)it.field = atoi(e); break;
			case 1: *(int32_t*)it.field = atoi(e) != 0 ? 1 : -1; break;
			case 2: { const int v = atoi(e); *(int32_t*)it.field = v != 0 ? v : -1; break; }
			case 3: *(int64_t*)it.field = atoll(e); break;
			case 4: *(int32_t*)it.field = std::string(e) == "lbvh" ? 2 : 1; break;
			case 5: *(int32_t*)it.field = it.as; break;
			case 6: { const int v = atoi(e); if (v >= 0 && v <= 3) *(int32_t*)it.field = 1 + v; break; }
			case 7: { const float v = (float)atof(e); *(float*)it.field = v != 0.f ? v : -1.f; break; }
		}
	}
}

struct ScenePlan
{
	bool have_scene = false;
	SceneView sv; TexView tv = {}; bool textured = false;
	int trav_mode = 0, stack_depth = 1, stack_depth_q4 = 0; bool scene_in_lds = false, shade_prims_in_lds = false; size_t lds_bytes = 0, lds_bytes_shadow = 0;
	bool cert = false;
	bool use_q4 = false, q4_shadow = false;
	bool vote = false; int persist = 0;
	int n_planes = 1; bool has_null_material = false;
	bool tables_in_lds = false, stage_nee = false; size_t shade_lds_bytes = 0;
	int class_mask = 0x3f; bool shade_sort = false;
	int stack_lds_words = 12;
};

struct JpContext
{
	int device = 0;
	JpOptions opt{}, opt_env{};
	hipStream_t stream = nullptr;
	int n_cus = 256;
	ScenePlan plan;
	void *d_flat = nullptr, *d_wide = nullptr, *d_q4 = nullptr;
	void* d_refbox = nullptr; bool cert_fell_back = false; int cert_eye_leaves = 0;
	void *d_nodes = nullptr, *d_prims = nullptr, *d_meta = nullptr, *d_mats = nullptr, *d_mat_type = nullptr, *d_lights = nullptr, *d_shade_tab = nullptr;
	int sincosf_mode = 0, libm_mode = 0;
	bool build_on_device = false; float build_ms = 0.f; int bvh_height = 0, bvh_nodes = 0;
	Queues q = {}; unsigned int cap = 0; int planes_alloc = 0; unsigned int blk_alloc = 0; int blocks_per_cu = 16;
	std::vector<void*> qbufs;
	float4* d_pix_acc = nullptr; size_t pix_acc_n = 0;
	int* d_spill = nullptr; size_t spill_words = 0;
	float* d_film = nullptr; size_t film_n = 0;
	float *d_bsdf_in = nullptr, *d_bsdf_out = nullptr; int* d_bsdf_fl = nullptr; size_t bsdf_cap = 0;
	float* d_gamma = nullptr; unsigned char* d_rgb8 = nullptr; size_t rgb8_n = 0; unsigned char* h_rgb8 = nullptr; size_t h_rgb8_n = 0;
	float* h_film = nullptr; size_t h_film_n = 0;
	DevCounters* d_cnt = nullptr;
	hipEvent_t ev0 = nullptr, ev1 = nullptr;
	bool profiling = false;
	std::vector<hipEvent_t> evpool; size_t evused = 0;
	struct Stamp { int cls; size_t a, b; };
	std::vector<Stamp> stamps;
	JpCounters counters;
	std::vector<JpContext*> lanes; bool is_lane = false; unsigned long long own_samples = 0; bool bpc_from_env = false;
	hipEvent_t ev_added = nullptr; bool added_valid = false; int last_lanes = 1;
	Queues fq = {}; std::vector<void*> fbufs; unsigned int fcap = 0; int fplanes = 0; size_t flacc_n = 0;
	unsigned int* d_jobs = nullptr; size_t jobs_n = 0;
	int last_fused = 0, last_region = 0, last_wgs = 0;
	int n_textures = 0, n_tex_mats = 0; long long texel_bytes = 0; int last_textured = 0;
	void *d_tex_desc = nullptr, *d_tex_col = nullptr, *d_texels = nullptr, *d_mat_tex = nullptr, *d_prim_uv = nullptr;
	unsigned int* d_side = nullptr; size_t side_n = 0;
};

static void free_scene(JpContext* c)
{
	void** ps[] = { &c->d_flat, &c->d_wide, &c->d_q4, &c->d_refbox, &c->d_nodes, &c->d_prims, &c->d_meta, &c->d_mats, &c->d_mat_type, &c->d_lights, &c->d_shade_tab,
	                &c->d_tex_desc, &c->d_tex_col, &c->d_texels, &c->d_mat_tex, &c->d_prim_uv };
	for (void** p : ps) { if (*p) hipFree(*p); *p = nullptr; }
	c->plan.have_scene = false;
	c->plan.tv = TexView(); c->plan.textured = false; c->n_textures = c->n_tex_mats = 0; c->texel_bytes = 0;
	if (c->d_side) hipFree(c->d_side);
	c->d_side = nullptr; c->side_n = 0;
}
static void free_queues(JpContext* c)
{
	for (void* p : c->qbufs) hipFree(p);
	c->qbufs.clear(); c->cap = 0; c->planes_alloc = 0;
}
static void free_fused(JpContext* c)
{
	for (void* p : c->fbufs) hipFree(p);
	c->fbufs.clear(); c->fcap = 0; c->fplanes = 0; c->flacc_n = 0;
	if (c->d_jobs) hipFree(c->d_jobs); c->d_jobs = nullptr; c->jobs_n = 0;
}

static int probe_host_sincosf()
{
	static int cached = -1;
	if (cached >= 0) return cached;
	bool okF = true, okN = true;
	uint32_t st = 0x12345u;
	for (int i = 0; i < 200000 && (okF || okN); i++)
	{
		st = st * 1664525u + 1013904223u;
		float y;
		if (i < 150000) y = (float)(st >> 8) * (1.0f / 16777216.0f) * 6.2831855f;
		else if (i < 180000) y = (float)(st >> 8) * (1.0f / 16777216.0f) * 0.01f;
		else y = ((float)(st >> 8) * (1.0f / 16777216.0f) - 0.5f) * 200.f;
		float hs, hc; ::sincosf(y, &hs, &hc);
		const float h1 = ::sinf(y), h2 = ::cosf(y);
		float as, ac, bs, bc;
		jp::sincosf_libm<true>(y, &as, &ac); jp::sincosf_libm<false>(y, &bs, &bc);
		uint32_t uhs, uhc, u1, u2, uas, uac, ubs, ubc;
		std::memcpy(&uhs, &hs, 4); std::memcpy(&uhc, &hc, 4); std::memcpy(&u1, &h1, 4); std::memcpy(&u2, &h2, 4);
		std::memcpy(&uas, &as, 4); std::memcpy(&uac, &ac, 4); std::memcpy(&ubs, &bs, 4); std::memcpy(&ubc, &bc, 4);
		if (uhs != u1 || uhc != u2) { okF = okN = false; }
		if (uas != uhs || uac != uhc) okF = false;
		if (ubs != uhs || ubc != uhc) okN = false;
	}
	cached = okF ? 1 : (okN ? 2 : 0);
	return cached;
}

static int probe_host_libm()
{
	static int cached = -1;
	if (cached >= 0) return cached;
	bool fma_cpu = false;
#if defined(__x86_64__)
	fma_cpu = __builtin_cpu_supports("fma") && __builtin_cpu_supports("avx2");
#endif
	auto same = [](float a, float b) { uint32_t x, y; std::memcpy(&x, &a, 4); std::memcpy(&y, &b, 4); return x == y || (a != a && b != b); };
	auto run = [&](bool fmab) {
		uint32_t st = 0x2545f491u;
		auto rnd = [&]() { st = st * 1664525u + 1013904223u; return st; };
		auto u01 = [&]() { return (float)(rnd() >> 8) * (1.0f / 16777216.0f); };
		for (int i = 0; i < 200000; i++)
		{
			float x, y;
			switch (i & 3)
			{
			case 0: { const uint32_t a = rnd(), b = rnd(); std::memcpy(&x, &a, 4); std::memcpy(&y, &b, 4); break; }
			case 1: x = u01(); y = u01() * 8.f; break;
			case 2: x = (u01() - 0.5f) * 250.f; y = (u01() - 0.5f) * 64.f; break;
			default: x = u01() * 1e-3f; y = 1.f / (u01() * 100.f + 1.f); break;
			}
			const float e = fmab ? jp::lm::expf_libm<true>(x) : jp::lm::expf_libm<false>(x), l = fmab ? jp::lm::logf_libm<true>(x) : jp::lm::logf_libm<false>(x);
			const float pw = fmab ? jp::lm::powf_libm<true>(x, y) : jp::lm::powf_libm<false>(x, y);
			if (!same(e, ::expf(x)) || !same(l, ::logf(x)) || !same(pw, ::powf(x, y))) return false;
			const float a = (i & 3) == 0 ? x : x * 2.f - 1.f;
			if (!same(jp::lm::acosf_libm(a), ::acosf(a)) || !same(jp::lm::atanf_libm(x), ::atanf(x))) return false;
			bool ok; const float t = jp::lm::tanf_libm(x * 8.f, &ok);
			if (ok && !same(t, ::tanf(x * 8.f))) return false;
		}
		return true;
	};
	int mode = 0;
	if (run(fma_cpu)) mode = 1 | (fma_cpu ? 2 : 0);
	else if (run(!fma_cpu)) mode = 1 | (fma_cpu ? 0 : 2);
	cached = mode;
	return cached;
}

static inline unsigned char host_gamma_encoding(float x)
{
	const float c = x < 0.f ? 0.f : (x > 1.f ? 1.f : x);
	return (unsigned char)(std::pow(c, (float)(1 / 2.2)) * 255.0);
}
static const float* host_gamma_thresholds()
{
	static float thr[255]; static std::once_flag once;
	std::call_once(once, []() {
		for (int k = 1; k <= 255; k++)
		{
			uint32_t lo = 0, hi = 0x3f800000u;
			while (hi - lo > 1) { const uint32_t mid = lo + (hi - lo) / 2; float f; std::memcpy(&f, &mid, 4); if (host_gamma_encoding(f) >= k) hi = mid; else lo = mid; }
			std::memcpy(&thr[k - 1], &hi, 4);
		}
	});
	return thr;
}
static unsigned long long host_gamma_sweep(int n_threads)
{
	const float* thr = host_gamma_thresholds();
	n_threads = std::max(1, std::min(64, n_threads));
	std::vector<unsigned long long> bad((size_t)n_threads, 0ull);
	std::vector<std::thread> pool;
	const uint64_t total = 0x3f800000ull + 1;
	for (int t = 0; t < n_threads; t++)
		pool.emplace_back([&, t]() {
			const uint64_t a = total * t / n_threads, b = total * (t + 1) / n_threads;
			int k = 0;
			{ const uint32_t u = (uint32_t)a; float f; std::memcpy(&f, &u, 4); while (k < 255 && thr[k] <= f) k++; }
			unsigned long long nb = 0;
			for (uint64_t i = a; i < b; i++)
			{
				const uint32_t u = (uint32_t)i; float f; std::memcpy(&f, &u, 4);
				while (k < 255 && thr[k] <= f) k++;
				if (host_gamma_encoding(f) != (unsigned char)k) nb++;
			}
			bad[(size_t)t] = nb;
		});
	for (auto& th : pool) th.join();
	unsigned long long s2 = 0; for (unsigned long long v : bad) s2 += v;
	return s2;
}

extern "C" {

const char* jp_last_error(void) { return g_err.c_str(); }
int jp_gamma_thresholds(float* out255) { if (!out255) return fail(JP_ERR_INVALID_ARGUMENT, "jp_gamma_thresholds: null argument"); std::memcpy(out255, host_gamma_thresholds(), 255 * sizeof(float)); return JP_OK; }
int jp_abi_version(void) { return JP_ABI_VERSION; }
long long jp_gamma_sweep(int n_threads) { return (long long)host_gamma_sweep(n_threads); }
int jp_probe_libm_sincosf(void) { return probe_host_sincosf(); }
int jp_probe_libm_xbsdf(void) { return probe_host_libm(); }

int jp_create_context(int device_id, JpContext** out)
{
	if (!out) return fail(JP_ERR_INVALID_ARGUMENT, "jp_create_context: out is null");
	*out = nullptr;
	int n = 0;
	if (hipGetDeviceCount(&n) != hipSuccess || n <= 0) return fail(JP_ERR_NO_DEVICE, "jp_create_context: no HIP device visible (this library has no CPU fallback)");
	if (device_id < 0 || device_id >= n) return fail(JP_ERR_NO_DEVICE, "jp_create_context: device id out of range");
	HIP_TRY(hipSetDevice(device_id));
	JpContext* c = new JpContext;
	c->device = device_id;
	std::memset(&c->counters, 0, sizeof(c->counters));
	std::memset(&c->q, 0, sizeof(c->q));
	std::memset(&c->opt_env, 0, sizeof(JpOptions)); c->opt_env.struct_bytes = (int32_t)sizeof(JpOptions);
	options_from_environment(c->opt_env);
	c->opt = c->opt_env;
	if (c->opt.blocks_per_cu >= 1 && c->opt.blocks_per_cu <= 256) { c->blocks_per_cu = c->opt.blocks_per_cu; c->bpc_from_env = true; }
	hipDeviceProp_t prop;
	if (hipGetDeviceProperties(&prop, device_id) == hipSuccess) c->n_cus = prop.multiProcessorCount;
	if (hipStreamCreateWithFlags(&c->stream, hipStreamNonBlocking) != hipSuccess || hipEventCreate(&c->ev0) != hipSuccess || hipEventCreate(&c->ev1) != hipSuccess
	    || hipMalloc((void**)&c->d_cnt, sizeof(DevCounters)) != hipSuccess)
	{ delete c; return fail(JP_ERR_DEVICE, "jp_create_context: stream/event/counter allocation failed"); }
	c->sincosf_mode = c->opt.libm_sincosf == 0 ? probe_host_sincosf() : (c->opt.libm_sincosf < 0 ? 0 : std::min(2, c->opt.libm_sincosf));
	{ hipError_t e = hipMemcpyToSymbol(HIP_SYMBOL(jp::g_sincosf_mode), &c->sincosf_mode, sizeof(int)); if (e != hipSuccess) { jp_destroy_context(c); return fail(JP_ERR_DEVICE, std::string("jp_create_context: hipMemcpyToSymbol: ") + hipGetErrorString(e)); } }
	c->libm_mode = c->opt.libm_xbsdf == 0 ? probe_host_libm() : (c->opt.libm_xbsdf < 0 ? 0 : (c->opt.libm_xbsdf & 3));
	{ hipError_t e = hipMemcpyToSymbol(HIP_SYMBOL(jp::xb::g_libm_mode), &c->libm_mode, sizeof(int)); if (e != hipSuccess) { jp_destroy_context(c); return fail(JP_ERR_DEVICE, std::string("jp_create_context: hipMemcpyToSymbol: ") + hipGetErrorString(e)); } }
	*out = c;
	return JP_OK;
}

int jp_set_options(JpContext* c, const JpOptions* o)
{
	if (!c) return fail(JP_ERR_INVALID_ARGUMENT, "jp_set_options: null context");
	JpOptions n = c->opt_env;
	if (o)
	{
		if (o->struct_bytes < (int32_t)sizeof(int32_t) || o->struct_bytes > 4096) return fail(JP_ERR_INVALID_ARGUMENT, "jp_set_options: struct_bytes is not a struct size");
		std::memset(&n, 0, sizeof(n));
		std::memcpy(&n, o, std::min<size_t>(sizeof(n), (size_t)o->struct_bytes));
		n.struct_bytes = (int32_t)sizeof(JpOptions);
		if (n.lanes < 0 || n.lanes > 4 || n.lane_rows < 0 || n.lane_rows > 64 || n.blocks_per_cu < 0 || n.blocks_per_cu > 256 || n.max_slots < 0 || n.traversal < 0 || n.traversal > 4
		    || n.stack_lds_words < 0 || n.bvh_max_leaf < 0 || n.bvh_max_leaf > 16 || n.trace_walk < 0 || n.trace_walk > 3 || n.device_tree < 0 || n.device_tree > 2
		    || (n.persist > 0 && n.persist != 8 && n.persist != 16 && n.persist != 32))
			return fail(JP_ERR_INVALID_ARGUMENT, "jp_set_options: field out of range (see JpOptions in jetpbrt_amd.h)");
	}
	const bool libm_changed = n.libm_sincosf != c->opt.libm_sincosf || n.libm_xbsdf != c->opt.libm_xbsdf;
	c->opt = n;
	c->blocks_per_cu = (n.blocks_per_cu >= 1) ? n.blocks_per_cu : 16; c->bpc_from_env = n.blocks_per_cu >= 1;
	for (JpContext* l : c->lanes) { l->blocks_per_cu = c->blocks_per_cu; l->opt = c->opt; }
	if (libm_changed)
	{
		HIP_TRY(hipSetDevice(c->device));
		c->sincosf_mode = n.libm_sincosf == 0 ? probe_host_sincosf() : (n.libm_sincosf < 0 ? 0 : std::min(2, n.libm_sincosf));
		c->libm_mode = n.libm_xbsdf == 0 ? probe_host_libm() : (n.libm_xbsdf < 0 ? 0 : (n.libm_xbsdf & 3));
		HIP_TRY(hipStreamSynchronize(c->stream));
		HIP_TRY(hipMemcpyToSymbol(HIP_SYMBOL(jp::g_sincosf_mode), &c->sincosf_mode, sizeof(int)));
		HIP_TRY(hipMemcpyToSymbol(HIP_SYMBOL(jp::xb::g_libm_mode), &c->libm_mode, sizeof(int)));
	}
	return JP_OK;
}
int jp_get_options(JpContext* c, JpOptions* out)
{
	if (!c || !out) return fail(JP_ERR_INVALID_ARGUMENT, "jp_get_options: null argument");
	*out = c->opt; out->struct_bytes = (int32_t)sizeof(JpOptions);
	return JP_OK;
}

int jp_destroy_context(JpContext* c)
{
	if (!c) return JP_OK;
	hipSetDevice(c->device);
	if (c->stream) hipStreamSynchronize(c->stream);
	for (JpContext* l : c->lanes) { std::memset(&l->plan.sv, 0, sizeof(l->plan.sv)); jp_destroy_context(l); }
	c->lanes.clear();
	if (c->ev_added) hipEventDestroy(c->ev_added);
	if (!c->is_lane) free_scene(c);
	free_queues(c);
	free_fused(c);
	if (c->d_pix_acc) hipFree(c->d_pix_acc);
	if (c->d_side) hipFree(c->d_side);
	if (c->d_spill) hipFree(c->d_spill);
	if (c->d_film) hipFree(c->d_film);
	if (c->h_film) hipHostFree(c->h_film);
	if (c->d_bsdf_in) hipFree(c->d_bsdf_in); if (c->d_bsdf_out) hipFree(c->d_bsdf_out); if (c->d_bsdf_fl) hipFree(c->d_bsdf_fl);
	if (c->d_gamma) hipFree(c->d_gamma);
	if (c->d_rgb8) hipFree(c->d_rgb8);
	if (c->h_rgb8) hipHostFree(c->h_rgb8);
	if (c->d_cnt) hipFree(c->d_cnt);
	for (hipEvent_t e : c->evpool) hipEventDestroy(e);
	if (c->ev0) hipEventDestroy(c->ev0);
	if (c->ev1) hipEventDestroy(c->ev1);
	if (c->stream) hipStreamDestroy(c->stream);
	delete c;
	return JP_OK;
}

}
```

### jet-pbrt_amd/csrc/jp_upload.h

```cpp
#pragma once
namespace
{
struct HV3 { float x, y, z; };
inline HV3 hsub(HV3 a, HV3 b) { HV3 r = { a.x - b.x, a.y - b.y, a.z - b.z }; return r; }
inline HV3 hcross(HV3 a, HV3 v) { HV3 r = { a.y * v.z - a.z * v.y, a.z * v.x - a.x * v.z, a.x * v.y - a.y * v.x }; return r; }
inline float hlen(HV3 a) { return std::sqrt(a.x * a.x + a.y * a.y + a.z * a.z); }
inline HV3 hld(const float* p) { HV3 r = { p[0], p[1], p[2] }; return r; }

struct ItemTree { std::vector<int> left, right; std::vector<float> bounds; int height = 0; };
int item_tree_build(const std::vector<float>& ib, std::vector<int>& idx, int start, int end, ItemTree& t, int depth)
{
	const int node = (int)t.left.size(); t.left.push_back(0); t.right.push_back(0); t.bounds.resize(t.bounds.size() + 6);
	t.height = std::max(t.height, depth);
	float nb[6] = { 1e30f, 1e30f, 1e30f, -1e30f, -1e30f, -1e30f }, cb[6] = { 1e30f, 1e30f, 1e30f, -1e30f, -1e30f, -1e30f };
	for (int i = start; i < end; i++)
	{
		const float* b = &ib[6 * (size_t)idx[i]];
		for (int a = 0; a < 3; a++) { nb[a] = std::min(nb[a], b[a]); nb[3 + a] = std::max(nb[3 + a], b[3 + a]); const float c = 0.5f * (b[a] + b[3 + a]); cb[a] = std::min(cb[a], c); cb[3 + a] = std::max(cb[3 + a], c); }
	}
	std::memcpy(&t.bounds[6 * (size_t)node], nb, sizeof(nb));
	if (end - start == 1) { t.left[node] = -idx[start] - 1; return node; }
	auto area = [](const float* b) { const float dx = b[3] - b[0], dy = b[4] - b[1], dz = b[5] - b[2]; return (dx < 0 || dy < 0 || dz < 0) ? 0.f : dx * dy + dy * dz + dz * dx; };
	const int NB = 16; float bestCost = 3.0e38f; int bestAxis = -1, bestBin = -1;
	for (int a = 0; a < 3; a++)
// ... 254 lines not shown
			w[3] = (uint32_t)eb[0] | ((uint32_t)eb[1] << 8) | ((uint32_t)eb[2] << 16) | (imask << 24);
			w[4] = child_base; w[5] = prim_base; w[6] = pack4(metaB); w[7] = pack4(metaB + 4);
			w[8] = pack4(ql[0]); w[9] = pack4(ql[0] + 4); w[10] = pack4(ql[1]); w[11] = pack4(ql[1] + 4);
			w[12] = pack4(ql[2]); w[13] = pack4(ql[2] + 4); w[14] = pack4(qh[0]); w[15] = pack4(qh[0] + 4);
			w[16] = pack4(qh[1]); w[17] = pack4(qh[1] + 4); w[18] = pack4(qh[2]); w[19] = pack4(qh[2] + 4);
		}
		if (!ok || (int)meta.size() != s->n_primitives)
		{
			use_wide = false; wide.clear(); prims.clear(); meta.clear(); std::fill(devPrimOf.begin(), devPrimOf.end(), -1);
		}
	}

	std::vector<int> order;
	if (!device_build && !ref_sem) { std::vector<int> st; st.push_back(0); while (!st.empty()) { int n = st.back(); st.pop_back(); if (s->bvh_left[n] < 0) continue; hostToDevNode[n] = (int)order.size(); order.push_back(n); st.push_back(s->bvh_right[n]); st.push_back(s->bvh_left[n]); } }
	const float kEmpty[6] = { 1e30f, 1e30f, 1e30f, -1e30f, -1e30f, -1e30f };
	std::vector<int> cert_item_first, cert_item_cnt; std::vector<float> cert_item_box;
	if (device_build) {}
	else if (ref_sem)
	{
		nodes.assign((size_t)2 * s->n_bvh_nodes, make_float4(0, 0, 0, 0));
		std::vector<int> st; st.push_back(0);
		while (!st.empty())
		{
			const int n = st.back(); st.pop_back();
			const float* b = s->bvh_bounds + 6 * (size_t)n;
			int l = s->bvh_left[n], r = s->bvh_right[n];
			if (l < 0)
			{
				const int first = -l - 1, cnt = r;
				const int dfirst = (int)meta.size();
				for (int k = 0; k < cnt; k++) emit_prim(s->bvh_prim_index[first + k]);
				l = -dfirst - 1;
				cert_item_first.push_back(dfirst); cert_item_cnt.push_back(cnt); cert_item_box.insert(cert_item_box.end(), b, b + 6);
			}
			else { st.push_back(r); st.push_back(l); }
			float fl, fr; std::memcpy(&fl, &l, 4); std::memcpy(&fr, &r, 4);
			nodes[2 * (size_t)n] = make_float4(b[0], b[1], b[2], fl); nodes[2 * (size_t)n + 1] = make_float4(b[3], b[4], b[5], fr);
		}
	}
	else if (order.empty())
	{
		float lb[6]; pad_box(0, lb);
		int ref = emit_leaf(0), rr = ref; float fr, fl; std::memcpy(&fl, &ref, 4); std::memcpy(&fr, &rr, 4);
		nodes.push_back(make_float4(lb[0], lb[1], lb[2], lb[3])); nodes.push_back(make_float4(lb[4], lb[5], kEmpty[0], kEmpty[1]));
		nodes.push_back(make_float4(kEmpty[2], kEmpty[3], kEmpty[4], kEmpty[5])); nodes.push_back(make_float4(fl, fr, 0, 0));
	}
	else
	{
		nodes.resize(4 * order.size());
		for (size_t di = 0; di < order.size(); di++)
		{
			int n = order[di], l = s->bvh_left[n], r = s->bvh_right[n];
			float lb[6], rb[6]; pad_box(l, lb); pad_box(r, rb);
			int lref = s->bvh_left[l] < 0 ? emit_leaf(l) : hostToDevNode[l];
			int rref = s->bvh_left[r] < 0 ? emit_leaf(r) : hostToDevNode[r];
			float fl, fr; std::memcpy(&fl, &lref, 4); std::memcpy(&fr, &rref, 4);
			nodes[4 * di + 0] = make_float4(lb[0], lb[1], lb[2], lb[3]); nodes[4 * di + 1] = make_float4(lb[4], lb[5], rb[0], rb[1]);
			nodes[4 * di + 2] = make_float4(rb[2], rb[3], rb[4], rb[5]); nodes[4 * di + 3] = make_float4(fl, fr, 0, 0);
		}
	}
	if ((size_t)s->n_primitives >= (1u << 27)) return fail(JP_ERR_UNSUPPORTED, "jp_upload_scene: too many primitives for the leaf reference encoding");

	auto collapse_q4 = [&](size_t n_nodes, auto isInner, auto leftOf, auto rightOf, auto boxOf, auto leafRefOf, auto flagOf, std::vector<uint32_t>& q4, int& q4_height) -> bool
	{
		struct Item { int bnode; uint32_t idx; int depth; };
		auto area = [](const float* b) { float dx = b[3] - b[0], dy = b[4] - b[1], dz = b[5] - b[2]; return dx * dy + dy * dz + dz * dx; };
		std::vector<Item> queue; queue.reserve(n_nodes / 2 + 16); queue.push_back({ 0, 0u, 1 });
		q4.clear(); q4_height = 0; q4.reserve((n_nodes / 2 + 16) * 16); q4.assign(16, 0u);
		bool ok = true;
		for (size_t qi = 0; qi < queue.size() && ok; qi++)
		{
			const Item it = queue[qi];
			q4_height = std::max(q4_height, it.depth);
			int ch[4]; float cb[4][6]; int nc = 0;
			ch[nc] = leftOf(it.bnode); boxOf(ch[nc], cb[nc]); nc++;
			ch[nc] = rightOf(it.bnode); boxOf(ch[nc], cb[nc]); nc++;
			while (nc < 4)
			{
				int best = -1; float bestA = -1.f;
				for (int k = 0; k < nc; k++) if (isInner(ch[k]) && area(cb[k]) > bestA) { bestA = area(cb[k]); best = k; }
				if (best < 0) break;
				const int n = ch[best];
				ch[best] = leftOf(n); boxOf(ch[best], cb[best]);
				ch[nc] = rightOf(n); boxOf(ch[nc], cb[nc]); nc++;
			}
			float lo[3] = { 1e30f, 1e30f, 1e30f }, hi[3] = { -1e30f, -1e30f, -1e30f };
			for (int k = 0; k < nc; k++) for (int a = 0; a < 3; a++) { lo[a] = std::min(lo[a], cb[k][a]); hi[a] = std::max(hi[a], cb[k][3 + a]); }
			int eb[3]; float sc3[3];
			for (int a = 0; a < 3; a++)
			{
				int e = (int)std::ceil(std::log2(std::max((hi[a] - lo[a]) / 255.f, 1e-30f)));
				e = std::max(-120, std::min(120, e));
				eb[a] = e + 127; sc3[a] = std::ldexp(1.0f, e);
			}
			for (int k = 0; k < nc; k++) for (int a = 0; a < 3; a++) { const float ex = 1e-6f * (hi[a] - lo[a]); cb[k][a] -= ex; cb[k][3 + a] += ex; }
			for (int a = 0; a < 3; a++) { const float ex = 1e-6f * (hi[a] - lo[a]); lo[a] -= ex; hi[a] += ex; }
			for (int a = 0; a < 3; a++)
			{
				int e = (int)std::ceil(std::log2(std::max((hi[a] - lo[a]) / 255.f, 1e-30f)));
				e = std::max(-120, std::min(120, e));
				eb[a] = e + 127; sc3[a] = std::ldexp(1.0f, e);
			}
			uint8_t ql[3][4], qh[3][4]; uint32_t refs[4] = { 0xffffffffu, 0xffffffffu, 0xffffffffu, 0xffffffffu }, valid = 0, flags = 0;
			for (int k = 0; k < 4; k++) for (int a = 0; a < 3; a++) { ql[a][k] = 255; qh[a][k] = 0; }
			for (int k = 0; k < nc && ok; k++)
			{
				valid |= 1u << k;
				const int n = ch[k];
				if (flagOf(n)) flags |= 1u << k;
				int r;
				if (isInner(n)) { r = (int)(q4.size() / 16); queue.push_back({ n, (uint32_t)r, it.depth + 1 }); q4.resize(q4.size() + 16, 0u); }
				else r = leafRefOf(n);
				std::memcpy(&refs[k], &r, 4);
				for (int a = 0; a < 3; a++)
				{
					int q0 = (int)std::floor((cb[k][a] - lo[a]) / sc3[a]), q1 = (int)std::ceil((cb[k][3 + a] - lo[a]) / sc3[a]);
					q0 = std::max(0, std::min(255, q0)); q1 = std::max(0, std::min(255, q1));
					while (q0 > 0 && std::fmaf((float)q0, sc3[a], lo[a]) > cb[k][a]) q0--;
					while (q1 < 255 && std::fmaf((float)q1, sc3[a], lo[a]) < cb[k][3 + a]) q1++;
					if (std::fmaf((float)q1, sc3[a], lo[a]) < cb[k][3 + a] || std::fmaf((float)q0, sc3[a], lo[a]) > cb[k][a]) { ok = false; break; }
					ql[a][k] = (uint8_t)q0; qh[a][k] = (uint8_t)q1;
				}
			}
			if (!ok) break;
			auto pack4 = [](const uint8_t* v) { return (uint32_t)v[0] | ((uint32_t)v[1] << 8) | ((uint32_t)v[2] << 16) | ((uint32_t)v[3] << 24); };
			uint32_t* w = &q4[(size_t)it.idx * 16];
			std::memcpy(&w[0], &lo[0], 4); std::memcpy(&w[1], &lo[1], 4); std::memcpy(&w[2], &lo[2], 4);
			w[3] = (uint32_t)eb[0] | ((uint32_t)eb[1] << 8) | ((uint32_t)eb[2] << 16) | (valid << 24);
			w[4] = refs[0]; w[5] = refs[1]; w[6] = refs[2]; w[7] = refs[3];
			w[8] = pack4(ql[0]); w[9] = pack4(ql[1]); w[10] = pack4(ql[2]); w[11] = pack4(qh[0]);
			w[12] = pack4(qh[1]); w[13] = pack4(qh[2]); w[14] = flags; w[15] = 0;
		}
		return ok;
	};
	std::vector<uint32_t> q4; int q4_height = 0;
	bool use_q4 = !device_build && !ref_sem && s->n_primitives > 1024 && s->bvh_left[0] >= 0 && !order.empty();
	use_q4 = use_q4 && opt_flag(op.q4, true);
	if (use_q4)
	{
		const bool ok = collapse_q4((size_t)s->n_bvh_nodes, [&](int n) { return s->bvh_left[n] >= 0; }, [&](int n) { return s->bvh_left[n]; }, [&](int n) { return s->bvh_right[n]; },
		                            [&](int n, float* bb) { pad_box(n, bb); }, [&](int n) { return emit_leaf(n); }, [](int) { return false; }, q4, q4_height);
		if (!ok || (int)meta.size() != s->n_primitives) { use_q4 = false; q4.clear(); }
	}

	const bool want_cert = s->bvh_reference_semantics == 2 && op.certified >= 0;
	bool use_cert = want_cert && ref_sem && s->n_primitives > 1024 && cert_item_first.size() >= 64;
	std::vector<float4> refbox; float cert_pad = 0.f, cert_pad_eye = 0.f;
	if (use_cert)
	{
		const int ni = (int)cert_item_first.size();
		ItemTree it; std::vector<int> idx(ni); for (int i = 0; i < ni; i++) idx[i] = i;
		it.left.reserve(2 * (size_t)ni); it.right.reserve(2 * (size_t)ni); it.bounds.reserve(12 * (size_t)ni);
		item_tree_build(cert_item_box, idx, 0, ni, it, 1);
		auto box_of = [&](int n, float* bb) {
			for (int a = 0; a < 3; a++)
			{
				const float lo = it.bounds[6 * (size_t)n + a], hi = it.bounds[6 * (size_t)n + 3 + a];
				const float m = std::max(std::fabs(lo), std::fabs(hi)), e = m * 1e-6f + 1e-6f + extra_pad;
				bb[a] = lo - e; bb[3 + a] = hi + e;
			}
		};
		bool ok = it.left[0] >= 0 && it.height + 2 <= 48;
		for (int i = 0; i < ni && ok; i++) if (cert_item_cnt[i] < 1 || cert_item_cnt[i] > 16) ok = false;
		const float tau = op.cert_eye_tau == 0.f ? 5e-3f : std::max(0.f, op.cert_eye_tau);
		std::vector<char> item_eye(ni, 0), node_eye(it.left.size(), 0); int n_eye = 0;
		for (int i = 0; i < ni && ok; i++)
			for (int k = 0; k < cert_item_cnt[i]; k++)
			{
				const size_t p = (size_t)cert_item_first[i] + k;
				int type; std::memcpy(&type, &prims[4 * p + 3].w, 4);
				if (type == JP_SHAPE_SPHERE) continue;
				const float4 g0 = prims[4 * p], gn = type == JP_SHAPE_DISK ? prims[4 * p + 1] : prims[4 * p + 3];
				const double vx = (double)g0.x - s->camera.pos[0], vy = (double)g0.y - s->camera.pos[1], vz = (double)g0.z - s->camera.pos[2];
				const double nl = std::sqrt((double)gn.x * gn.x + (double)gn.y * gn.y + (double)gn.z * gn.z), dist = std::sqrt(vx * vx + vy * vy + vz * vz);
				if (std::fabs(vx * gn.x + vy * gn.y + vz * gn.z) <= tau * dist * nl + 1e-30) { if (!item_eye[i]) n_eye++; item_eye[i] = 1; }
			}
		if (ok) for (size_t n = it.left.size(); n-- > 0;) node_eye[n] = it.left[n] < 0 ? item_eye[-it.left[n] - 1] : (char)(node_eye[it.left[n]] | node_eye[it.right[n]]);
		c->cert_eye_leaves = n_eye;
		if (ok) ok = collapse_q4(it.left.size(), [&](int n) { return it.left[n] >= 0; }, [&](int n) { return it.left[n]; }, [&](int n) { return it.right[n]; }, box_of,
		                         [&](int n) { const int item = -it.left[n] - 1; return -(((cert_item_first[item] << 4) | (cert_item_cnt[item] - 1)) + 1); }, [&](int n) { return node_eye[n] != 0; }, q4, q4_height);
		if (!ok) { use_cert = false; q4.clear(); }
		else
		{
			refbox.resize((size_t)2 * s->n_primitives);
			double diag = 0;
			for (int i = 0; i < ni; i++)
			{
				const float* b = &cert_item_box[6 * (size_t)i];
				for (int k = 0; k < cert_item_cnt[i]; k++) { const size_t p = (size_t)cert_item_first[i] + k; refbox[2 * p] = make_float4(b[0], b[1], b[2], 0.f); refbox[2 * p + 1] = make_float4(b[3], b[4], b[5], 0.f); }
				diag += std::sqrt((double)(b[3] - b[0]) * (b[3] - b[0]) + (double)(b[4] - b[1]) * (b[4] - b[1]) + (double)(b[5] - b[2]) * (b[5] - b[2]));
			}
			const float K = op.cert_slack == 0.f ? 16384.f : std::max(0.f, op.cert_slack);
			cert_pad = (float)(K * 1.1920929e-7 / std::max(1e-20, diag / ni));
			const float Ke = op.cert_slack_eye == 0.f ? std::min(K, 1024.f) : std::max(0.f, op.cert_slack_eye);
			cert_pad_eye = (float)(Ke * 1.1920929e-7 / std::max(1e-20, diag / ni));
		}
	}

	size_t n4nodes = nodes.size(), n4prims = prims.size(), nmeta = meta.size();
	bool dev_wide = false; int dev_n_wide = 0; bool dev_q4 = false; int dev_n_q4 = 0;
	c->build_on_device = device_build; c->build_ms = 0.f;
	if (device_build)
	{
		for (int p = 0; p < s->n_primitives; p++) emit_prim(p);
		void *d_p0 = nullptr, *d_m0 = nullptr;
		hipError_t e = hipMalloc(&d_p0, prims.size() * sizeof(float4)); if (e == hipSuccess) e = hipMalloc(&d_m0, meta.size() * sizeof(int4));
		if (e == hipSuccess) e = hipMemcpyAsync(d_p0, prims.data(), prims.size() * sizeof(float4), hipMemcpyHostToDevice, c->stream);
		if (e == hipSuccess) e = hipMemcpyAsync(d_m0, meta.data(), meta.size() * sizeof(int4), hipMemcpyHostToDevice, c->stream);
		LbvhResult lr; std::vector<int> sorted;
		bool ploc = op.device_tree != 2;
		int maxLeaf = ploc ? 2 : 3;
		if (op.bvh_max_leaf >= 1 && op.bvh_max_leaf <= 16) maxLeaf = op.bvh_max_leaf;
		if (e == hipSuccess && ploc) { e = ploc_build(c->stream, (const float4*)d_p0, (const int4*)d_m0, s->n_primitives, maxLeaf, op.ploc_radius, op.ploc_max_rounds, lr, sorted); if (e == hipErrorNotReady) { e = hipSuccess; ploc = false; } }
		if (e == hipSuccess && !ploc) e = lbvh_build(c->stream, (const float4*)d_p0, (const int4*)d_m0, s->n_primitives, maxLeaf, lr, sorted);
		if (d_p0) hipFree(d_p0); if (d_m0) hipFree(d_m0);
		if (e != hipSuccess) return fail(JP_ERR_DEVICE, std::string("jp_upload_scene: device BVH build failed: ") + hipGetErrorString(e));
		if (lr.height + 2 > 60)
		{
			hipFree(lr.d_nodes); hipFree(lr.d_prims); hipFree(lr.d_meta);
			return fail(JP_ERR_UNSUPPORTED, "jp_upload_scene: device-built BVH is deeper than the 58-entry traversal stack; hand over a host-built hierarchy for this scene");
		}
		c->d_nodes = lr.d_nodes; c->d_prims = lr.d_prims; c->d_meta = lr.d_meta;
		for (int i = 0; i < s->n_primitives; i++) devPrimOf[sorted[i]] = i;
		height = lr.height; c->build_ms = lr.build_ms;
		n4nodes = (size_t)4 * lr.n_nodes; n4prims = (size_t)4 * s->n_primitives; nmeta = (size_t)s->n_primitives;
		const bool want_wide = opt_flag(op.device_wide, s->n_primitives > 64);
		if (want_wide)
		{
			WideResult wr;
			e = lbvh_build_wide(c->stream, (const float4*)c->d_nodes, s->n_primitives, wr);
			if (e != hipSuccess) return fail(JP_ERR_DEVICE, std::string("jp_upload_scene: device wide-tree build failed: ") + hipGetErrorString(e));
			if (wr.d_wide) { c->d_wide = wr.d_wide; dev_wide = true; dev_n_wide = wr.n_wide; wide_height = wr.height; use_wide = true; c->build_ms += wr.build_ms; }
		}
		const bool want_q4 = s->n_primitives > 1024 && opt_flag(op.q4, true);
		if (want_q4)
		{
			WideResult qr;
			e = lbvh_build_q4(c->stream, (const float4*)c->d_nodes, s->n_primitives, qr);
			if (e != hipSuccess) return fail(JP_ERR_DEVICE, std::string("jp_upload_scene: device 4-wide tree build failed: ") + hipGetErrorString(e));
			if (qr.d_wide) { c->d_q4 = qr.d_wide; dev_q4 = true; dev_n_q4 = qr.n_wide; c->build_ms += qr.build_ms; use_q4 = true; q4_height = qr.height; }
		}
	}
	c->bvh_height = height; c->bvh_nodes = ref_sem ? s->n_bvh_nodes : (int)(n4nodes / 4);

	std::vector<float4> flat;
	if (!device_build && !ref_sem && s->n_primitives <= 64)
	{
		int nleaves = 0; for (int n = 0; n < s->n_bvh_nodes; n++) if (seen[n] && s->bvh_left[n] < 0) nleaves++;
		if (nleaves <= 32)
		{
			for (int n = 0; n < s->n_bvh_nodes; n++)
			{
				if (!seen[n] || s->bvh_left[n] >= 0) continue;
				float bb[6]; pad_box(n, bb);
				int first = -s->bvh_left[n] - 1, cnt = s->bvh_right[n];
				unsigned long long bits = 0;
				for (int k = 0; k < cnt; k++) bits |= 1ull << devPrimOf[s->bvh_prim_index[first + k]];
				const uint32_t lo = (uint32_t)bits, hi = (uint32_t)(bits >> 32); float flo, fhi; std::memcpy(&flo, &lo, 4); std::memcpy(&fhi, &hi, 4);
				flat.push_back(make_float4(bb[0], bb[1], bb[2], flo)); flat.push_back(make_float4(bb[3], bb[4], bb[5], fhi));
			}
		}
	}

	std::vector<float4> mats(4 * std::max(1, s->n_materials)); std::vector<int> mtype(std::max(1, s->n_materials), 0);
	for (int i = 0; i < s->n_materials; i++) { std::memcpy(&mats[4 * i], s->mat_params + (size_t)i * JP_MAT_PARAM_STRIDE, 16 * sizeof(float)); mtype[i] = s->mat_type[i]; }
	std::vector<float4> lights(2 * std::max(1, s->n_lights)); int planes = 0, nenv = 0; float envsum[3] = { 0, 0, 0 };
	for (int i = 0; i < s->n_lights; i++)
	{
		int ty = s->light_type[i]; float tf; std::memcpy(&tf, &ty, 4);
		const float* rad = s->light_radiance + 3 * i;
		lights[2 * i] = make_float4(rad[0], rad[1], rad[2], tf);
		bool black = rad[0] == 0.f && rad[1] == 0.f && rad[2] == 0.f;
		if (!black) planes++;
		float inv_area = 0.f; int dp = -1;
		if (ty == JP_LIGHT_AREA)
		{
			int p = s->light_prim[i]; dp = devPrimOf[p];
			int t = s->prim_shape_type[p], k = s->prim_shape_index[p]; float area;
			if (t == JP_SHAPE_TRIANGLE) area = 0.5f * hlen(hcross(hsub(hld(s->tri_p1 + 3 * k), hld(s->tri_p0 + 3 * k)), hsub(hld(s->tri_p2 + 3 * k), hld(s->tri_p0 + 3 * k))));
			else if (t == JP_SHAPE_RECTANGLE) area = hlen(hcross(hsub(hld(s->rect_p0 + 3 * k), hld(s->rect_p1 + 3 * k)), hsub(hld(s->rect_p2 + 3 * k), hld(s->rect_p1 + 3 * k))));
			else if (t == JP_SHAPE_DISK) { const float kPi = (float)3.14159265358979323846; area = kPi * s->disk_radius[k] * s->disk_radius[k]; }
			else { const float kPi = (float)3.14159265358979323846; float r2 = s->sph_radius[k] * s->sph_radius[k]; area = 4 * kPi * r2; }
			inv_area = 1 / area;
		}
		else if (ty == JP_LIGHT_ENVIRONMENT) { nenv++; envsum[0] += rad[0]; envsum[1] += rad[1]; envsum[2] += rad[2]; }
		float df; std::memcpy(&df, &dp, 4);
		lights[2 * i + 1] = make_float4(df, inv_area, 0, 0);
		if (ty == JP_LIGHT_POINT || ty == JP_LIGHT_DIRECTION) lights[2 * i + 1] = make_float4(s->light_vec[3 * i], s->light_vec[3 * i + 1], s->light_vec[3 * i + 2], 0);
	}

	auto up = [&](void** dst, const void* src, size_t bytes) -> hipError_t {
		hipError_t e = hipMalloc(dst, std::max<size_t>(bytes, 16)); if (e != hipSuccess) return e;
		return hipMemcpy(*dst, src, bytes, hipMemcpyHostToDevice);
	};
	if (!device_build)
	{
		HIP_TRY(up(&c->d_nodes, nodes.data(), nodes.size() * sizeof(float4)));
		HIP_TRY(up(&c->d_prims, prims.data(), prims.size() * sizeof(float4)));
		HIP_TRY(up(&c->d_meta, meta.data(), meta.size() * sizeof(int4)));
	}
	HIP_TRY(up(&c->d_mats, mats.data(), mats.size() * sizeof(float4)));
	HIP_TRY(up(&c->d_mat_type, mtype.data(), mtype.size() * sizeof(int)));
	HIP_TRY(up(&c->d_lights, lights.data(), lights.size() * sizeof(float4)));
	{
		std::vector<float4> tabv;
		tabv.insert(tabv.end(), lights.begin(), lights.begin() + 2 * (size_t)s->n_lights);
		tabv.insert(tabv.end(), mats.begin(), mats.begin() + 4 * (size_t)s->n_materials);
		const size_t at = tabv.size(); tabv.resize(at + ((size_t)s->n_materials + 3) / 4, make_float4(0, 0, 0, 0));
		if (s->n_materials > 0) std::memcpy(&tabv[at], mtype.data(), (size_t)s->n_materials * sizeof(int));
		if (!device_build)
		{
			tabv.insert(tabv.end(), prims.begin(), prims.end());
			const size_t am = tabv.size(); tabv.resize(am + meta.size());
			std::memcpy(&tabv[am], meta.data(), meta.size() * sizeof(int4));
			auto hnorm = [](HV3 a) { const float l = hlen(a); HV3 r = { a.x / l, a.y / l, a.z / l }; return r; };
			for (size_t pi = 0; pi < meta.size(); pi++)
			{
				const float4 g3 = prims[4 * pi + 3], g1 = prims[4 * pi + 1];
				int type; std::memcpy(&type, &g3.w, 4);
				const HV3 nn = type == JP_SHAPE_DISK ? HV3{ g1.x, g1.y, g1.z } : HV3{ g3.x, g3.y, g3.z };
				const HV3 n = hnorm(nn);
				const HV3 tmp = std::fabs(n.x) > 0.99f ? HV3{ 0, 1, 0 } : HV3{ 1, 0, 0 };
				const HV3 t = hnorm(hcross(n, tmp)), sv = hnorm(hcross(t, n));
				tabv.push_back(make_float4(n.x, n.y, n.z, 0)); tabv.push_back(make_float4(sv.x, sv.y, sv.z, 0)); tabv.push_back(make_float4(t.x, t.y, t.z, 0));
			}
		}
		HIP_TRY(up(&c->d_shade_tab, tabv.data(), tabv.size() * sizeof(float4)));
	}
	if (use_wide && !dev_wide) HIP_TRY(up(&c->d_wide, wide.data(), wide.size() * sizeof(uint32_t)));
	if ((use_q4 && !dev_q4) || use_cert) HIP_TRY(up(&c->d_q4, q4.data(), q4.size() * sizeof(uint32_t)));
	if (use_cert) HIP_TRY(up(&c->d_refbox, refbox.data(), refbox.size() * sizeof(float4)));
	if (!flat.empty()) HIP_TRY(up(&c->d_flat, flat.data(), flat.size() * sizeof(float4)));

	ScenePlan& p = c->plan; SceneView& v = p.sv;
	v.nodes = (const float4*)c->d_nodes; v.n_nodes = (int)(n4nodes / 4);
	v.prims = (const float4*)c->d_prims; v.meta = (const int4*)c->d_meta; v.n_prims = (int)nmeta;
	v.mats = (const float4*)c->d_mats; v.mat_type = (const int*)c->d_mat_type; v.n_mats = s->n_materials;
	v.lights = (const float4*)c->d_lights; v.n_lights = s->n_lights; v.shade_tab = (const float4*)c->d_shade_tab;
	v.env_sum = make_float3(envsum[0], envsum[1], envsum[2]); v.n_env = nenv;
	v.world_radius = s->world_radius; v.cam = s->camera;
	v.flat = (const float4*)c->d_flat; v.n_flat = (int)(flat.size() / 2);
	v.wide = (const uint4*)c->d_wide; v.n_wide = dev_wide ? dev_n_wide : (int)(wide.size() / 20);
	v.q4 = (const uint4*)c->d_q4; v.n_q4 = dev_q4 ? dev_n_q4 : (int)(q4.size() / 16);
	v.refbox = (const float4*)c->d_refbox; v.cert_pad = cert_pad; v.cert_pad_eye = cert_pad_eye; p.cert = use_cert;
	p.use_q4 = use_q4; p.q4_shadow = use_q4 && opt_flag(op.q4_shadow, true);
	p.stack_depth = std::max(2, height + 2);
	p.stack_depth_q4 = (use_q4 || use_cert) ? 3 * q4_height + 2 : 0;
	size_t scene_bytes = (n4nodes + n4prims) / 4 * 5 * sizeof(float4);
	size_t prim_bytes = n4prims / 4 * 5 * sizeof(float4);
	size_t stack_bytes = (size_t)p.stack_depth * JP_BLOCK * sizeof(int);
	p.scene_in_lds = !device_build && scene_bytes + stack_bytes <= 40 * 1024;
	p.trav_mode = use_wide ? 3 : ((!flat.empty() && prim_bytes <= 40 * 1024) ? 2 : (p.scene_in_lds ? 1 : 0));
	if (!use_wide && op.traversal > 0) { const int m = op.traversal - 1; if (m == 0 || (m == 1 && p.scene_in_lds)) p.trav_mode = m; }
	if (use_wide) p.scene_in_lds = false;
	if (ref_sem) p.trav_mode = 5;
	p.lds_bytes = p.trav_mode == 2 ? prim_bytes : (p.trav_mode == 1 ? stack_bytes + scene_bytes : stack_bytes);
	p.lds_bytes_shadow = p.trav_mode == 3 ? (size_t)2 * (wide_height + 2) * JP_BLOCK * sizeof(int) : p.lds_bytes;
	{
		size_t tab = ((size_t)2 * s->n_lights + (size_t)4 * s->n_materials) * sizeof(float4) + (size_t)s->n_materials * sizeof(int) + 16;
		p.tables_in_lds = tab <= 16 * 1024;
		const size_t shade_static = (size_t)JP_SHADE_TILE * 3 + (size_t)JP_SHADE_CLASSES * (JP_SHADE_TILE / JP_BLOCK) * (JP_BLOCK / 64) * 4 + 128;
		const size_t prim_part = n4prims * sizeof(float4) + nmeta * sizeof(int4) + 3 * nmeta * sizeof(float4);
		p.shade_prims_in_lds = p.tables_in_lds && p.scene_in_lds && tab + prim_part <= 24 * 1024;
		p.shade_lds_bytes = p.tables_in_lds ? tab + (p.shade_prims_in_lds ? prim_part : 0) : 0;
		const size_t stage_bytes = 16 + (size_t)std::max(1, planes) * 2 * JP_BLOCK * sizeof(float4);
		p.stage_nee = p.tables_in_lds && std::max(1, planes) <= 4 && shade_static + p.shade_lds_bytes + stage_bytes <= 64 * 1024;
		if (p.stage_nee) p.shade_lds_bytes += stage_bytes;
	}
	p.n_planes = std::max(1, planes);
	{
		bool kinds[8] = { false, false, false, false, false, false, false, false }; int nk = 0;
		for (int i = 0; i < s->n_primitives; i++) { const int m = s->prim_material[i]; const int k = m < 0 ? 7 : s->mat_type[m]; if (!kinds[k]) { kinds[k] = true; nk++; } }
		p.stack_lds_words = op.stack_lds_words >= 2 ? (op.stack_lds_words & ~1) : 12;
		p.persist = ((p.trav_mode == 0 || p.trav_mode == 3 || p.trav_mode == 5) && s->n_primitives > 1024) ? 16 : 0;
		if (op.persist != 0) p.persist = op.persist < 0 ? 0 : op.persist;
		p.vote = opt_flag(op.vote, p.trav_mode != 5 || p.cert);
		p.class_mask = 1; for (int k = 0; k < 5; k++) if (kinds[k]) p.class_mask |= 2 << k;
		p.shade_sort = opt_flag(op.shade_sort, nk > 1);
	}
	p.has_null_material = hasNull; c->cert_fell_back = false;
	p.have_scene = true;
	return JP_OK;
}


extern "C" int jp_upload_scene_textured(JpContext* c, const JpScene* s, const JpTextures* t)
{
	if (!c || !s) return fail(JP_ERR_INVALID_ARGUMENT, "jp_upload_scene_textured: null argument");
	if (!t) return jp_upload_scene(c, s);
	if (t->struct_bytes < (int32_t)sizeof(JpTextures)) return fail(JP_ERR_INVALID_ARGUMENT, "jp_upload_scene_textured: JpTextures.struct_bytes smaller than this library's JpTextures");
	if (t->n_textures < 0 || t->n_textures > (1 << 28)) return fail(JP_ERR_INVALID_ARGUMENT, "jp_upload_scene_textured: n_textures out of range");
	if (t->n_textures == 0) return jp_upload_scene(c, s);
	const int nt = t->n_textures;
	if (!t->tex_type || !t->tex_color) return fail(JP_ERR_INVALID_ARGUMENT, "jp_upload_scene_textured: null tex_type / tex_color");
	if (t->n_materials != s->n_materials) return fail(JP_ERR_INVALID_ARGUMENT, "jp_upload_scene_textured: n_materials differs from the scene's");
	if (t->n_triangles != s->n_triangles) return fail(JP_ERR_INVALID_ARGUMENT, "jp_upload_scene_textured: n_triangles differs from the scene's");
	if (t->n_materials > 0 && (!t->mat_texture || !s->mat_type)) return fail(JP_ERR_INVALID_ARGUMENT, "jp_upload_scene_textured: null mat_texture");
	long long pool = 0;
	for (int i = 0; i < nt; i++)
	{
		const int ty = t->tex_type[i];
		if (ty < JP_TEXTURE_SOLID || ty > JP_TEXTURE_IMAGE) return fail(JP_ERR_INVALID_ARGUMENT, "jp_upload_scene_textured: unknown texture type");
		if (ty == JP_TEXTURE_IMAGE)
		{
			if (!t->tex_width || !t->tex_height || !t->tex_offset || !t->texels) return fail(JP_ERR_INVALID_ARGUMENT, "jp_upload_scene_textured: image texture without tex_width / tex_height / tex_offset / texels");
			const long long w = t->tex_width[i], h = t->tex_height[i], off = t->tex_offset[i];
			if (w < 1 || w > 16384 || h < 1 || h > 16384) return fail(JP_ERR_INVALID_ARGUMENT, "jp_upload_scene_textured: image size out of range (1 .. 16384 per side)");
			if (off < 0 || t->n_texel_bytes < 0 || off > t->n_texel_bytes - 3 * w * h) return fail(JP_ERR_INVALID_ARGUMENT, "jp_upload_scene_textured: image texels beyond n_texel_bytes");
			pool += w * h;
		}
		else
		{
			const int nc = ty == JP_TEXTURE_CHECKER ? 6 : 3;
			for (int k = 0; k < nc; k++) if (!std::isfinite(t->tex_color[6 * (size_t)i + k])) return fail(JP_ERR_INVALID_ARGUMENT, "jp_upload_scene_textured: colour not finite");
		}
	}
	if (pool > 0x7fffffffll) return fail(JP_ERR_INVALID_ARGUMENT, "jp_upload_scene_textured: more than 2^31 texels in all");
	int ntm = 0;
	for (int m = 0; m < t->n_materials; m++)
	{
		const int k = t->mat_texture[m];
		if (k < -1 || k >= nt) return fail(JP_ERR_INVALID_ARGUMENT, "jp_upload_scene_textured: mat_texture out of range");
		if (k < 0) continue;
		const int mt = s->mat_type[m];
		if (mt != JP_MAT_MATTE && mt != JP_MAT_MIRROR && mt != JP_MAT_PLASTIC) return fail(JP_ERR_INVALID_ARGUMENT, "jp_upload_scene_textured: a texture on a glass or metal material (its [0..2] is eta, not a colour)");
		ntm++;
	}
	if (s->n_primitives > 0 && (!s->prim_shape_type || !s->prim_shape_index)) return fail(JP_ERR_INVALID_ARGUMENT, "jp_upload_scene_textured: null array");
	const int st = jp_upload_scene(c, s);
	if (st != JP_OK) return st;
	if (ntm == 0) return JP_OK;

	std::vector<int4> desc(nt); std::vector<float4> col(2 * (size_t)nt); std::vector<unsigned int> texels((size_t)pool);
	size_t at = 0;
	for (int i = 0; i < nt; i++)
	{
		const float* cc = t->tex_color + 6 * (size_t)i;
		desc[i] = make_int4(t->tex_type[i], 0, 0, 0);
		col[2 * i] = make_float4(0, 0, 0, 0); col[2 * i + 1] = make_float4(0, 0, 0, 0);
		if (t->tex_type[i] == JP_TEXTURE_IMAGE)
		{
			const int w = t->tex_width[i], h = t->tex_height[i];
			desc[i].y = w; desc[i].z = h; desc[i].w = (int)at;
			const uint8_t* src = t->texels + t->tex_offset[i];
			for (size_t k = 0; k < (size_t)w * h; k++) texels[at + k] = (unsigned int)src[3 * k] | ((unsigned int)src[3 * k + 1] << 8) | ((unsigned int)src[3 * k + 2] << 16) | 0xff000000u;
			at += (size_t)w * h;
		}
		else
		{
			col[2 * i] = make_float4(cc[0], cc[1], cc[2], 0);
			if (t->tex_type[i] == JP_TEXTURE_CHECKER) col[2 * i + 1] = make_float4(cc[3], cc[4], cc[5], 0);
		}
	}
	std::vector<int> mt(t->mat_texture, t->mat_texture + t->n_materials);
	std::vector<float2> puv(3 * (size_t)s->n_primitives, make_float2(0, 0));
	if (t->tri_uv)
		for (int p = 0; p < s->n_primitives; p++)
			if (s->prim_shape_type[p] == JP_SHAPE_TRIANGLE)
			{
				const float* u = t->tri_uv + 6 * (size_t)s->prim_shape_index[p];
				for (int k = 0; k < 3; k++) puv[3 * (size_t)p + k] = make_float2(u[2 * k], u[2 * k + 1]);
			}
	auto put = [&](void** d, const void* src, size_t bytes) -> bool {
		if (bytes == 0) return true;
		if (hipMalloc(d, bytes) != hipSuccess) return false;
		return hipMemcpy(*d, src, bytes, hipMemcpyHostToDevice) == hipSuccess;
	};
	if (!put(&c->d_tex_desc, desc.data(), desc.size() * sizeof(int4)) || !put(&c->d_tex_col, col.data(), col.size() * sizeof(float4))
	    || !put(&c->d_texels, texels.data(), texels.size() * sizeof(unsigned int)) || !put(&c->d_mat_tex, mt.data(), mt.size() * sizeof(int))
	    || !put(&c->d_prim_uv, puv.data(), puv.size() * sizeof(float2)))
	{
		free_scene(c);
		return fail(JP_ERR_DEVICE, "jp_upload_scene_textured: out of device memory for the texture tables");
	}
	TexView& tv = c->plan.tv; tv = TexView();
	tv.desc = (const int4*)c->d_tex_desc; tv.col = (const float4*)c->d_tex_col; tv.texels = (const unsigned int*)c->d_texels;
	tv.mat_tex = (const int*)c->d_mat_tex; tv.prim_uv = (const float2*)c->d_prim_uv;
	c->plan.textured = true; c->n_textures = nt; c->n_tex_mats = ntm; c->texel_bytes = (long long)texels.size() * 4;
	return JP_OK;
}
```

Before: 3001.

## Fuse camera ray generation into first extend and precompute shade sort keys

After: 2987 (median of 2 runs). Within noise of the previous version (-0.5%).

```diff
diff --git a/jet-pbrt_amd/csrc/jp_common.h b/jet-pbrt_amd/csrc/jp_common.h
--- a/jet-pbrt_amd/csrc/jp_common.h
+++ b/jet-pbrt_amd/csrc/jp_common.h
@@ -6,6 +6,10 @@
 extern __shared__ float4 s_dyn[];
 
 #define JP_SHADE_CLASSES 6
+#ifndef JP_SHADE_TILE
+#define JP_SHADE_TILE 8192
+#endif
+#define JP_SORT_SEG ((JP_SHADE_TILE / JP_BLOCK) * (JP_BLOCK / 64))
 
 struct DevCounters
 {
@@ -24,6 +28,7 @@
 	float4 *sh_o;
 	float4 *sh_d, *sh_c;
 	unsigned int *blk_q[2], *blk_sh;
+	unsigned char *skey, *scnt;
 	unsigned int cap;
 	unsigned int R;
 };
@@ -43,6 +48,7 @@
 	int sampler_debug;
 	int class_mask;
 	int lane_index, lane_count, lane_rows;
+	int cam_rays;
 };
 
 __device__ __forceinline__ float rngf(const RenderConst& rc, uint32_t key, uint32_t dim) { return rc.sampler_debug ? 0.5f : jp_rng_float(key, dim); }
@@ -68,6 +74,51 @@
 	y = (rc.shard_index + j * rc.shard_count) * rc.band_rows + (r - j * rc.band_rows);
 }
 
+struct RegionMap { unsigned int total, nchunks, K; };
+__device__ __forceinline__ RegionMap region_map(const RenderConst& rc, unsigned int G)
+{
+	RegionMap m; m.total = (unsigned int)rc.npix * rc.sbatch; m.nchunks = (m.total + JP_BLOCK - 1) / JP_BLOCK; m.K = (m.nchunks + G - 1) / G;
+	return m;
+}
+__device__ __forceinline__ bool region_chunk(const RenderConst& rc, const RegionMap& m, unsigned int b, unsigned int G, unsigned int k, unsigned int& c)
+{
+	if (rc.compact)
+	{
+		const unsigned int qi = b * m.K + k, npb = (unsigned int)rc.npix / JP_BLOCK;
+		if (qi >= m.nchunks) return false;
+		const unsigned int pb = qi / (unsigned int)rc.sbatch, sl = qi - pb * (unsigned int)rc.sbatch; c = sl * npb + pb;
+		return true;
+	}
+	c = b + k * G;
+	return c < m.nchunks;
+}
+
+__device__ __forceinline__ V3 camera_ray(const SceneView& sc, const RenderConst& rc, unsigned int slot, uint32_t& key)
+{
+	const int pix = slot % rc.npix, s = rc.s0 + slot / rc.npix;
+	int x, y; pixel_of(rc, pix, x, y);
+	key = jp_rng_key(rc.seed, (uint32_t)x, (uint32_t)y, (uint32_t)s);
+	const float fx = (float)x + rngf(rc, key, 0), fy = (float)y + rngf(rc, key, 1);
+	const V3 front = mk(sc.cam.front[0], sc.cam.front[1], sc.cam.front[2]);
+	const V3 right = mk(sc.cam.right[0], sc.cam.right[1], sc.cam.right[2]);
+	const V3 up = mk(sc.cam.up[0], sc.cam.up[1], sc.cam.up[2]);
+	V3 dir = front + right * (fx / sc.cam.res_x - 0.5f) + up * (0.5f - fy / sc.cam.res_y);
+	return normalize(dir);
+}
+
+__device__ __forceinline__ unsigned int class_counts(unsigned int key, int class_mask, unsigned int lane)
+{
+	unsigned int mine = 0;
+	#pragma unroll
+	for (int c = 0; c < JP_SHADE_CLASSES; c++)
+	{
+		unsigned int nc = 0;
+		if ((class_mask >> c) & 1) nc = (unsigned int)__popcll(__ballot(key == (unsigned int)c));
+		if (lane == (unsigned int)c) mine = nc;
+	}
+	return mine;
+}
+
 __device__ __forceinline__ unsigned int wave_take(unsigned int* ctr, unsigned int n)
 {
 	unsigned int v = 0;
diff --git a/jet-pbrt_amd/csrc/jp_device.h b/jet-pbrt_amd/csrc/jp_device.h
--- a/jet-pbrt_amd/csrc/jp_device.h
+++ b/jet-pbrt_amd/csrc/jp_device.h
@@ -45,6 +45,7 @@
 	const int* mat_type; int n_mats;
 	const float4* lights;
 	int n_lights;
+	const int* prim_class; int class_mask;
 	const float4* shade_tab;
 	float3 env_sum;
 	int n_env;
diff --git a/jet-pbrt_amd/csrc/jp_kernels.hip b/jet-pbrt_amd/csrc/jp_kernels.hip
--- a/jet-pbrt_amd/csrc/jp_kernels.hip
+++ b/jet-pbrt_amd/csrc/jp_kernels.hip
@@ -15,36 +15,26 @@
 
 __global__ void __launch_bounds__(JP_BLOCK) k_raygen(SceneView sc, Queues q, RenderConst rc, DevCounters* cnt)
 {
-	const unsigned int total = (unsigned int)rc.npix * rc.sbatch;
-	const unsigned int nchunks = (total + JP_BLOCK - 1) / JP_BLOCK;
 	const unsigned int G = gridDim.x, b = blockIdx.x;
-	if (b == 0 && threadIdx.x == 0) { cnt->n_queue[0] = total; cnt->n_queue[1] = 0; cnt->n_shadow = 0; }
+	const RegionMap m = region_map(rc, G);
+	if (b == 0 && threadIdx.x == 0) { cnt->n_queue[0] = m.total; cnt->n_queue[1] = 0; cnt->n_shadow = 0; }
 	unsigned int filled = 0;
-	const unsigned int K = (nchunks + G - 1) / G, npb = (unsigned int)rc.npix / JP_BLOCK;
-	for (unsigned int k = 0, j0 = 0; k < K; k++, j0 += JP_BLOCK)
+	for (unsigned int k = 0, j0 = 0; k < m.K; k++, j0 += JP_BLOCK)
 	{
 		unsigned int c;
-		if (rc.compact) { const unsigned int qi = b * K + k; if (qi >= nchunks) break; const unsigned int pb = qi / (unsigned int)rc.sbatch, sl = qi - pb * (unsigned int)rc.sbatch; c = sl * npb + pb; }
-		else { c = b + k * G; if (c >= nchunks) break; }
+		if (!region_chunk(rc, m, b, G, k, c)) break;
 		const unsigned int slot = c * JP_BLOCK + threadIdx.x;
-		if (slot < total)
+		if (slot < m.total)
 		{
 			const unsigned int i = b * q.R + j0 + threadIdx.x;
-			const int pix = slot % rc.npix, s = rc.s0 + slot / rc.npix;
-			int x, y; pixel_of(rc, pix, x, y);
-			const uint32_t key = jp_rng_key(rc.seed, (uint32_t)x, (uint32_t)y, (uint32_t)s);
-			const float fx = (float)x + rngf(rc, key, 0), fy = (float)y + rngf(rc, key, 1);
-			const V3 front = mk(sc.cam.front[0], sc.cam.front[1], sc.cam.front[2]);
-			const V3 right = mk(sc.cam.right[0], sc.cam.right[1], sc.cam.right[2]);
-			const V3 up = mk(sc.cam.up[0], sc.cam.up[1], sc.cam.up[2]);
-			V3 dir = front + right * (fx / sc.cam.res_x - 0.5f) + up * (0.5f - fy / sc.cam.res_y);
-			dir = normalize(dir);
+			uint32_t key;
+			const V3 dir = camera_ray(sc, rc, slot, key);
 			q.ray_o[0][i] = make_float4(sc.cam.pos[0], sc.cam.pos[1], sc.cam.pos[2], __int_as_float((int)slot));
 			q.ray_d[0][i] = make_float4(dir.x, dir.y, dir.z, __int_as_float(MK_FLAGS(0, 0, 2)));
 			q.beta[0][i] = make_float4(1.f, 1.f, 1.f, __int_as_float((int)key));
 			q.lacc[slot] = make_float4(0.f, 0.f, 0.f, 0.f);
 		}
-		const unsigned int left = total - c * JP_BLOCK;
+		const unsigned int left = m.total - c * JP_BLOCK;
 		filled += left < JP_BLOCK ? left : JP_BLOCK;
 	}
 	if (threadIdx.x == 0) q.blk_q[0][b] = filled;
@@ -70,36 +60,41 @@
 template <> struct SceneAccess<0>
 {
 	const float4 *nodes, *prims; int* stack; int depth;
-	__device__ __forceinline__ SceneAccess(const SceneView& sc, int depth_) : nodes(sc.nodes), prims(sc.prims), stack((int*)s_dyn + threadIdx.x), depth(depth_) {}
+	__device__ __forceinline__ SceneAccess(const SceneView& sc, int depth_, bool = false) : nodes(sc.nodes), prims(sc.prims), stack((int*)s_dyn + threadIdx.x), depth(depth_) {}
 	template <bool kAnyHit> __device__ __forceinline__ int trace(const SceneView&, V3 o, V3 d, float tmin, float& tmax) const
 	{ return traverse<kAnyHit, 4>(nodes, prims, o, d, tmin, tmax, stack); }
+	__device__ __forceinline__ unsigned int cls(const SceneView& sc, int prim) const { return (unsigned int)sc.prim_class[prim]; }
 };
 template <> struct SceneAccess<1>
 {
 	float4 *nodes, *prims; int* stack; int depth;
-	__device__ __forceinline__ SceneAccess(const SceneView& sc, int depth_) : depth(depth_)
+	__device__ __forceinline__ SceneAccess(const SceneView& sc, int depth_, bool with_class = false) : depth(depth_)
 	{
 		stack = (int*)s_dyn + threadIdx.x;
 		nodes = s_dyn + (depth * JP_BLOCK) / 4;
 		prims = nodes + 5 * sc.n_nodes;
 		for (int i = threadIdx.x; i < 4 * sc.n_nodes; i += JP_BLOCK) nodes[5 * (i >> 2) + (i & 3)] = sc.nodes[i];
 		for (int i = threadIdx.x; i < 4 * sc.n_prims; i += JP_BLOCK) prims[5 * (i >> 2) + (i & 3)] = sc.prims[i];
+		if (with_class) for (int i = threadIdx.x; i < sc.n_prims; i += JP_BLOCK) prims[5 * i + 4].x = __int_as_float(sc.prim_class[i]);
 		__syncthreads();
 	}
 	template <bool kAnyHit> __device__ __forceinline__ int trace(const SceneView&, V3 o, V3 d, float tmin, float& tmax) const
 	{ return traverse<kAnyHit, 5>(nodes, prims, o, d, tmin, tmax, stack); }
+	__device__ __forceinline__ unsigned int cls(const SceneView&, int prim) const { return (unsigned int)__float_as_int(prims[5 * prim + 4].x); }
 };
 template <> struct SceneAccess<2>
 {
 	float4* prims;
-	__device__ __forceinline__ SceneAccess(const SceneView& sc, int)
+	__device__ __forceinline__ SceneAccess(const SceneView& sc, int, bool with_class = false)
 	{
 		prims = s_dyn;
 		for (int i = threadIdx.x; i < 4 * sc.n_prims; i += JP_BLOCK) prims[5 * (i >> 2) + (i & 3)] = sc.prims[i];
+		if (with_class) for (int i = threadIdx.x; i < sc.n_prims; i += JP_BLOCK) prims[5 * i + 4].x = __int_as_float(sc.prim_class[i]);
 		__syncthreads();
 	}
 	template <bool kAnyHit> __device__ __forceinline__ int trace(const SceneView& sc, V3 o, V3 d, float tmin, float& tmax) const
 	{ return traverse_flat<kAnyHit, 5>(sc.flat, sc.n_flat, sc.n_prims, prims, o, d, tmin, tmax); }
+	__device__ __forceinline__ unsigned int cls(const SceneView&, int prim) const { return (unsigned int)__float_as_int(prims[5 * prim + 4].x); }
 };
 
 template <> struct SceneAccess<3>
@@ -129,42 +124,95 @@
 template <> struct SceneAccess<5>
 {
 	const float4 *nodes, *prims; int* stack;
-	__device__ __forceinline__ SceneAccess(const SceneView& sc, int) : nodes(sc.nodes), prims(sc.prims), stack((int*)s_dyn + threadIdx.x) {}
+	__device__ __forceinline__ SceneAccess(const SceneView& sc, int, bool = false) : nodes(sc.nodes), prims(sc.prims), stack((int*)s_dyn + threadIdx.x) {}
 	template <bool kAnyHit> __device__ __forceinline__ int trace(const SceneView&, V3 o, V3 d, float tmin, float& tmax) const
 	{ return traverse_ref<kAnyHit>(nodes, prims, o, d, tmin, tmax, stack); }
+	__device__ __forceinline__ unsigned int cls(const SceneView& sc, int prim) const { return (unsigned int)sc.prim_class[prim]; }
 };
 
 template <int kMode>
-__global__ void __launch_bounds__(JP_BLOCK) k_extend(SceneView sc, Queues q, int cur, int depth, DevCounters* cnt)
-{
-	SceneAccess<kMode> acc(sc, depth);
+__device__ __forceinline__ void extend_keys(const SceneAccess<kMode>& acc, const SceneView& sc, const Queues& q, unsigned int b, unsigned int pass, unsigned int i, bool valid, int hit)
+{
+	unsigned int t = threadIdx.x; asm volatile("" : "+v"(t));
+	const unsigned int lane = t & 63u, wave = t >> 6;
+	unsigned int key = JP_SHADE_CLASSES;
+	if (valid) key = hit >= 0 ? acc.cls(sc, hit) : 0u;
+	q.skey[i] = (unsigned char)key;
+	const unsigned int mine = class_counts(key, sc.class_mask, lane);
+	if (lane < JP_SHADE_CLASSES) q.scnt[b * (unsigned int)(JP_SHADE_CLASSES * JP_SORT_SEG) + lane * JP_SORT_SEG + pass * (JP_BLOCK / 64) + wave] = (unsigned char)mine;
+}
+
+template <int kMode>
+__global__ void __launch_bounds__(JP_BLOCK, 8) k_extend(SceneView sc, Queues q, int cur, int depth, DevCounters* cnt)
+{
+	const bool keys = q.skey != nullptr;
+	SceneAccess<kMode> acc(sc, depth, keys);
 	const unsigned int b = blockIdx.x, n = q.blk_q[cur][b], rbase = b * q.R;
 	if (b == 0 && threadIdx.x == 0) { cnt->closest += cnt->n_queue[cur]; cnt->n_queue[cur ^ 1] = 0; cnt->n_shadow = 0; }
 	unsigned int h = 0;
 	float4 ro = make_float4(0, 0, 0, 0), rd = make_float4(0, 0, 1, 0);
 	if (threadIdx.x < n) { ro = q.ray_o[cur][rbase + threadIdx.x]; rd = q.ray_d[cur][rbase + threadIdx.x]; }
-	for (unsigned int j = threadIdx.x; j < n; j += JP_BLOCK)
-	{
-		const unsigned int i = rbase + j;
+	for (unsigned int j0 = 0, pass = 0; j0 < n; j0 += JP_BLOCK, pass++)
+	{
+		const unsigned int j = j0 + threadIdx.x, i = rbase + j;
+		const bool valid = j < n;
 		const float4 co = ro, cd = rd;
 		if (j + JP_BLOCK < n) { ro = q.ray_o[cur][i + JP_BLOCK]; rd = q.ray_d[cur][i + JP_BLOCK]; }
-		float tmax = JP_INF;
-		const int hit = acc.template trace<false>(sc, xyz(co), xyz(cd), 0.001f, tmax);
-		q.hit[i] = make_float2(tmax, __int_as_float(hit));
-		h += hit >= 0 ? 1u : 0u;
+		int hit = -1;
+		if (valid)
+		{
+			float tmax = JP_INF;
+			hit = acc.template trace<false>(sc, xyz(co), xyz(cd), 0.001f, tmax);
+			q.hit[i] = make_float2(tmax, __int_as_float(hit));
+			h += hit >= 0 ? 1u : 0u;
+		}
+		if (keys) extend_keys<kMode>(acc, sc, q, b, pass, i, valid, hit);
 	}
 	for (int off = 32; off > 0; off >>= 1) h += __shfl_down(h, off);
 	if ((threadIdx.x & 63) == 0 && h) atomicAdd(&cnt->closest_hit, (unsigned long long)h);
 }
 
-#ifndef JP_SHADE_TILE
-#define JP_SHADE_TILE 8192
-#endif
+template <int kMode>
+__global__ void __launch_bounds__(JP_BLOCK, 8) k_extend_cam(SceneView sc, Queues q, RenderConst rc, int depth, DevCounters* cnt)
+{
+	const bool keys = q.skey != nullptr;
+	SceneAccess<kMode> acc(sc, depth, keys);
+	const unsigned int G = gridDim.x, b = blockIdx.x, rbase = b * q.R;
+	const RegionMap m = region_map(rc, G);
+	if (b == 0 && threadIdx.x == 0) { cnt->n_queue[0] = m.total; cnt->n_queue[1] = 0; cnt->n_shadow = 0; cnt->closest += m.total; }
+	const V3 o = mk(sc.cam.pos[0], sc.cam.pos[1], sc.cam.pos[2]);
+	unsigned int filled = 0, h = 0;
+	for (unsigned int k = 0; k < m.K; k++)
+	{
+		unsigned int c;
+		if (!region_chunk(rc, m, b, G, k, c)) break;
+		const unsigned int slot = c * JP_BLOCK + threadIdx.x, i = rbase + k * JP_BLOCK + threadIdx.x;
+		const bool valid = slot < m.total;
+		int hit = -1;
+		if (valid)
+		{
+			uint32_t key;
+			const V3 dir = camera_ray(sc, rc, slot, key);
+			float tmax = JP_INF;
+			hit = acc.template trace<false>(sc, o, dir, 0.001f, tmax);
+			q.hit[i] = make_float2(tmax, __int_as_float(hit));
+			q.ray_d[0][i] = make_float4(dir.x, dir.y, dir.z, __int_as_float((int)key));
+			h += hit >= 0 ? 1u : 0u;
+		}
+		if (keys) extend_keys<kMode>(acc, sc, q, b, k, i, valid, hit);
+		const unsigned int left = m.total - c * JP_BLOCK;
+		filled += left < JP_BLOCK ? left : JP_BLOCK;
+	}
+	if (threadIdx.x == 0) q.blk_q[0][b] = filled;
+	for (int off = 32; off > 0; off >>= 1) h += __shfl_down(h, off);
+	if ((threadIdx.x & 63) == 0 && h) atomicAdd(&cnt->closest_hit, (unsigned long long)h);
+}
+
 template <bool kTab, bool kPrims, bool kStage, bool kSort, bool kTex>
 __device__ __forceinline__ void shade_body(SceneView sc, Queues q, RenderConst rc, int cur, DevCounters* cnt, const TexView& tv)
 {
 	static_assert(kTab || !kPrims, "k_shade: primitive records in LDS only together with the tables");
-	constexpr int kWaves = JP_BLOCK / 64, kMaxSeg = (JP_SHADE_TILE / JP_BLOCK) * kWaves;
+	constexpr int kWaves = JP_BLOCK / 64, kMaxSeg = JP_SORT_SEG;
 	static_assert(JP_SHADE_TILE % JP_BLOCK == 0 && JP_SHADE_TILE <= 65536, "k_shade: tile positions are 16-bit");
 	__shared__ unsigned short s_idx[kSort ? JP_SHADE_TILE : 1];
 	__shared__ unsigned char s_key[kSort ? JP_SHADE_TILE : 1];
@@ -204,6 +252,9 @@
 	const int4* meta_t = kPrims ? (const int4*)s_meta : sc.meta;
 	const unsigned int rbase = b * q.R;
 	const unsigned int t0 = 0, count = n;
+	const bool cam = !kTex && rc.cam_rays;
+	const bool xkeys = kSort && !kTex && q.skey != nullptr;
+	const RegionMap rmap = region_map(rc, gridDim.x);
 	JP_TS(0);
 	if (kSort)
 	{
@@ -212,7 +263,7 @@
 		const unsigned int plane = tid & 63u, wave = tid >> 6, npass = (count + JP_BLOCK - 1) / JP_BLOCK;
 		const unsigned long long ltm = (1ull << plane) - 1ull;
 		#pragma unroll 1
-		for (unsigned int r0 = 0; r0 < npass; r0 += 8)
+		for (unsigned int r0 = 0; r0 < npass && !xkeys; r0 += 8)
 		{
 			int pi[8];
 			#pragma unroll
@@ -233,14 +284,7 @@
 					key = m >= 0 ? 1u + (unsigned int)mat_type[m] : 0u;
 				}
 				s_key[r * JP_BLOCK + tid] = (unsigned char)key;
-				unsigned int mine = 0;
-				#pragma unroll
-				for (int c = 0; c < JP_SHADE_CLASSES; c++)
-				{
-					unsigned int nc = 0;
-					if ((rc.class_mask >> c) & 1) nc = (unsigned int)__popcll(__ballot(key == (unsigned int)c));
-					if (plane == (unsigned int)c) mine = nc;
-				}
+				const unsigned int mine = class_counts(key, rc.class_mask, plane);
 				if (plane < JP_SHADE_CLASSES) s_cnt[plane * seg + r * kWaves + wave] = mine;
 			}
 		}
@@ -252,7 +296,7 @@
 			for (int i = 0; i < 3; i++)
 			{
 				const unsigned int at = 3 * tid + i;
-				v[i] = (at < nctr && (at % seg) / kWaves < npass) ? s_cnt[at] : 0u; t += v[i];
+				v[i] = (at < nctr && (at % seg) / kWaves < npass) ? (xkeys ? (unsigned int)q.scnt[(size_t)b * nctr + at] : s_cnt[at]) : 0u; t += v[i];
 			}
 			unsigned int incl = t;
 			#pragma unroll
@@ -269,7 +313,7 @@
 		#pragma unroll 1
 		for (unsigned int r = 0; r < npass; r++)
 		{
-			const unsigned int key = s_key[r * JP_BLOCK + tid];
+			const unsigned int key = xkeys ? (unsigned int)q.skey[rbase + t0 + r * JP_BLOCK + tid] : (unsigned int)s_key[r * JP_BLOCK + tid];
 			unsigned int pre = 0;
 			#pragma unroll
 			for (int c = 0; c < JP_SHADE_CLASSES; c++)
@@ -283,11 +327,24 @@
 		__syncthreads();
 	}
 	float4 ro_n = make_float4(0, 0, 0, 0), rd_n = ro_n, rb_n = ro_n; float2 h_n = make_float2(0, 0); unsigned int s_n = 0;
+	auto fetch = [&](unsigned int pos)
+	{
+		if (kSort) pos = (unsigned int)s_idx[pos];
+		const unsigned int i0 = rbase + t0 + pos;
+		rd_n = q.ray_d[cur][i0]; h_n = q.hit[i0];
+		if (cam)
+		{
+			unsigned int c = 0; region_chunk(rc, rmap, b, gridDim.x, pos / JP_BLOCK, c);
+			ro_n = make_float4(sc.cam.pos[0], sc.cam.pos[1], sc.cam.pos[2], __int_as_float((int)(c * JP_BLOCK + pos % JP_BLOCK)));
+		}
+		else { ro_n = q.ray_o[cur][i0]; rb_n = q.beta[cur][i0]; }
+		if (kTex) s_n = tv.side[i0];
+	};
 	JP_TS(1);
 	const unsigned int nch = (count + 63u) >> 6;
 	unsigned int tk = wave_take(&s_ctr[0], 1u);
 	unsigned int c0 = (nch - 1u - tk) << 6;
-	if (tk < nch && c0 + lane < count) { const unsigned int pos = c0 + lane, i0 = rbase + t0 + (kSort ? (unsigned int)s_idx[pos] : pos); ro_n = q.ray_o[cur][i0]; rd_n = q.ray_d[cur][i0]; rb_n = q.beta[cur][i0]; h_n = q.hit[i0]; if (kTex) s_n = tv.side[i0]; }
+	if (tk < nch && c0 + lane < count) fetch(c0 + lane);
 	while (tk < nch)
 	{
 		const bool valid = c0 + lane < count;
@@ -297,18 +354,13 @@
 		JP_TS(3);
 #endif
 #ifdef JP_SHADE_NO_PREFETCH
-		if (valid) { const unsigned int pos = c0 + lane, i0 = rbase + t0 + (kSort ? (unsigned int)s_idx[pos] : pos); ro_n = q.ray_o[cur][i0]; rd_n = q.ray_d[cur][i0]; rb_n = q.beta[cur][i0]; h_n = q.hit[i0]; if (kTex) s_n = tv.side[i0]; }
+		if (valid) fetch(c0 + lane);
 		const float4 ro = ro_n, rd = rd_n, rb = rb_n; const float2 h = h_n; const unsigned int sw = s_n;
 		tk = wave_take(&s_ctr[0], 1u); c0 = (nch - 1u - tk) << 6;
 #else
 		const float4 ro = ro_n, rd = rd_n, rb = rb_n; const float2 h = h_n; const unsigned int sw = s_n;
 		tk = wave_take(&s_ctr[0], 1u); c0 = (nch - 1u - tk) << 6;
-		if (tk < nch && c0 + lane < count)
-		{
-			const unsigned int pos = c0 + lane;
-			const unsigned int i1 = rbase + t0 + (kSort ? (unsigned int)s_idx[pos] : pos);
-			ro_n = q.ray_o[cur][i1]; rd_n = q.ray_d[cur][i1]; rb_n = q.beta[cur][i1]; h_n = q.hit[i1]; if (kTex) s_n = tv.side[i1];
-		}
+		if (tk < nch && c0 + lane < count) fetch(c0 + lane);
 #endif
 		bool shaded = false, wantNee = false, alive = false;
 		V3 o = mk(0, 0, 0), d = mk(0, 0, 1), beta = mk(0, 0, 0), p = mk(0, 0, 0), N = mk(0, 0, 1);
@@ -316,14 +368,15 @@
 		Closure c; c.kind = CL_LAMBERT; Frame fr; fr.s = fr.t = fr.n = mk(0, 0, 1);
 		if (valid)
 		{
-			o = xyz(ro); d = xyz(rd); beta = xyz(rb);
-			slot = __float_as_int(ro.w); key = (uint32_t)__float_as_int(rb.w);
-			const int flags = __float_as_int(rd.w);
+			o = xyz(ro); d = xyz(rd); beta = cam ? mk(1.f, 1.f, 1.f) : xyz(rb);
+			slot = __float_as_int(ro.w); key = (uint32_t)__float_as_int(cam ? rd.w : rb.w);
+			const int flags = cam ? MK_FLAGS(0, 0, 2) : __float_as_int(rd.w);
 			bounce = FLAG_BOUNCE(flags); spec = FLAG_SPEC(flags); dim = FLAG_DIM(flags);
 			const int pi = __float_as_int(h.y);
 			const bool found = pi >= 0;
 			int mat = -1, hitprim = 0; bool nflip = false, tabframe = kPrims;
 			V3 Le = splat(0);
+			V3 Lc = mk(0, 0, 0);
 			if (found)
 			{
 				const float4 g3 = prims[4 * pi + 3];
@@ -349,13 +402,19 @@
 					const float4 l0 = lights[2 * li];
 					if (__float_as_int(l0.w) == JP_LIGHT_ENVIRONMENT && !isblack(xyz(l0)))
 					{
+						if (cam) { Lc = Lc + cmul(beta, xyz(l0)); continue; }
 						float4 L = q.lacc[slot];
 						V3 a = mk(L.x, L.y, L.z) + cmul(beta, xyz(l0));
 						q.lacc[slot] = make_float4(a.x, a.y, a.z, 0.f);
 					}
 				}
 			}
-			if (!isblack(Le))
+			if (cam)
+			{
+				if (!isblack(Le)) Lc = Lc + cmul(beta, Le);
+				q.lacc[slot] = make_float4(Lc.x, Lc.y, Lc.z, 0.f);
+			}
+			else if (!isblack(Le))
 			{
 				float4 L = q.lacc[slot];
 				V3 a = mk(L.x, L.y, L.z) + cmul(beta, Le);
diff --git a/jet-pbrt_amd/csrc/jp_render.h b/jet-pbrt_amd/csrc/jp_render.h
--- a/jet-pbrt_amd/csrc/jp_render.h
+++ b/jet-pbrt_amd/csrc/jp_render.h
@@ -13,7 +13,8 @@
 	for (int b = 0; b < 2 && ok; b++) ok = alloc((void**)&q.ray_o[b], (size_t)cap * 16) && alloc((void**)&q.ray_d[b], (size_t)cap * 16) && alloc((void**)&q.beta[b], (size_t)cap * 16)
 	                                       && alloc((void**)&q.blk_q[b], (size_t)nblocks * 4);
 	ok = ok && alloc((void**)&q.hit, (size_t)cap * 8) && alloc((void**)&q.lacc, (size_t)cap * 16) && alloc((void**)&q.sh_o, (size_t)cap * 16)
-	     && alloc((void**)&q.sh_d, (size_t)cap * 16 * planes) && alloc((void**)&q.sh_c, (size_t)cap * 16 * planes) && alloc((void**)&q.blk_sh, (size_t)nblocks * 4);
+	     && alloc((void**)&q.sh_d, (size_t)cap * 16 * planes) && alloc((void**)&q.sh_c, (size_t)cap * 16 * planes) && alloc((void**)&q.blk_sh, (size_t)nblocks * 4)
+	     && alloc((void**)&q.skey, (size_t)cap) && alloc((void**)&q.scnt, (size_t)nblocks * JP_SHADE_CLASSES * JP_SORT_SEG);
 	if (!ok) { free_queues(c); return fail(JP_ERR_DEVICE, "jp_render: out of device memory for the path queues"); }
 	c->cap = cap; c->planes_alloc = planes; c->blk_alloc = nblocks;
 	return JP_OK;
@@ -105,6 +106,17 @@
 	if (p.shade_prims_in_lds) return p.stage_nee ? shade_row<true, true, true>(p.shade_sort) : shade_row<true, true, false>(p.shade_sort);
 	if (p.tables_in_lds) return p.stage_nee ? shade_row<true, false, true>(p.shade_sort) : shade_row<true, false, false>(p.shade_sort);
 	return shade_row<false, false, false>(p.shade_sort);
+}
+
+typedef void (*ExtendCamKernel)(SceneView, Queues, RenderConst, int, DevCounters*);
+struct SeamPlan { ExtendCamKernel cam; bool keys; };
+SeamPlan seam_plan(const ScenePlan& p, const JpOptions& o, bool path_integrator)
+{
+	SeamPlan s = { nullptr, false };
+	if (!path_integrator || refill_walks(p) || p.textured) return s;
+	if (!(o.reserved[0] & 1)) s.cam = p.trav_mode == 5 ? k_extend_cam<5> : (p.trav_mode == 2 ? k_extend_cam<2> : (p.trav_mode == 1 ? k_extend_cam<1> : k_extend_cam<0>));
+	s.keys = p.shade_sort && p.sv.prim_class != nullptr && !(o.reserved[0] & 2);
+	return s;
 }
 
 typedef void (*OtherKernel)(SceneView, Queues, RenderConst, int, int, DevCounters*);
@@ -168,6 +180,8 @@
 			budget = (size_t)sbatch / 2 * (size_t)npix * per;
 		}
 		c->q.cap = cap; c->q.R = R;
+		const SeamPlan seam = seam_plan(p, c->opt, rp->integrator == JP_INTEGRATOR_PATH);
+		Queues q = c->q; if (!seam.keys) q.skey = q.scnt = nullptr;
 		const bool tex = p.textured && rp->integrator == JP_INTEGRATOR_PATH;
 		if (tex && c->side_n < cap)
 		{
@@ -191,12 +205,13 @@
 		for (int s0 = 0; s0 < rp->spp; s0 += sbatch)
 		{
 			rc.s0 = s0; rc.sbatch = std::min(sbatch, rp->spp - s0);
-			{ Stamper t(c, CLS_OTHER); hipLaunchKernelGGL(k_raygen, dim3(grid), dim3(JP_BLOCK), 0, c->stream, p.sv, c->q, rc, c->d_cnt); }
+			rc.cam_rays = 0;
+			if (!seam.cam) { Stamper t(c, CLS_OTHER); hipLaunchKernelGGL(k_raygen, dim3(grid), dim3(JP_BLOCK), 0, c->stream, p.sv, q, rc, c->d_cnt); }
 			if (rp->integrator != JP_INTEGRATOR_PATH)
 			{
 				Stamper t(c, CLS_OTHER);
 				const int ogrid = (int)std::min<unsigned int>((P + JP_BLOCK - 1) / JP_BLOCK, (unsigned int)(c->n_cus * 16));
-				hipLaunchKernelGGL(ok, dim3(ogrid), dim3(JP_BLOCK), p.lds_bytes, c->stream, p.sv, c->q, rc, rp->integrator, p.stack_depth, c->d_cnt);
+				hipLaunchKernelGGL(ok, dim3(ogrid), dim3(JP_BLOCK), p.lds_bytes, c->stream, p.sv, q, rc, rp->integrator, p.stack_depth, c->d_cnt);
 			}
 			int cur = 0;
 			int iters = rp->integrator != JP_INTEGRATOR_PATH ? 0 : rp->max_depth + 1;
@@ -210,30 +225,36 @@
 				}
 				{
 					Stamper t(c, CLS_EXTEND);
-					if (ek.refill) hipLaunchKernelGGL(ek.refill, dim3(grid), dim3(JP_BLOCK), ek.lds, c->stream, p.sv, c->q, cur, ek.words, c->d_spill, c->d_cnt);
-					else hipLaunchKernelGGL(ek.plain, dim3(grid), dim3(JP_BLOCK), ek.lds, c->stream, p.sv, c->q, cur, ek.words, c->d_cnt);
+					if (ek.refill) hipLaunchKernelGGL(ek.refill, dim3(grid), dim3(JP_BLOCK), ek.lds, c->stream, p.sv, q, cur, ek.words, c->d_spill, c->d_cnt);
+					else if (it == 0 && seam.cam) hipLaunchKernelGGL(seam.cam, dim3(grid), dim3(JP_BLOCK), ek.lds, c->stream, p.sv, q, rc, ek.words, c->d_cnt);
+					else hipLaunchKernelGGL(ek.plain, dim3(grid), dim3(JP_BLOCK), ek.lds, c->stream, p.sv, q, cur, ek.words, c->d_cnt);
 				}
 				{
 					Stamper t(c, CLS_SHADE);
 					if (tex)
 					{
-						hipLaunchKernelGGL(k_texel, dim3(grid), dim3(JP_BLOCK), 0, c->stream, p.sv, c->q, cur, tv);
-						hipLaunchKernelGGL(hk.tex, dim3(grid), dim3(JP_BLOCK), p.shade_lds_bytes, c->stream, p.sv, c->q, rc, cur, c->d_cnt, tv);
+						hipLaunchKernelGGL(k_texel, dim3(grid), dim3(JP_BLOCK), 0, c->stream, p.sv, q, cur, tv);
+						hipLaunchKernelGGL(hk.tex, dim3(grid), dim3(JP_BLOCK), p.shade_lds_bytes, c->stream, p.sv, q, rc, cur, c->d_cnt, tv);
 					}
-					else hipLaunchKernelGGL(hk.plain, dim3(grid), dim3(JP_BLOCK), p.shade_lds_bytes, c->stream, p.sv, c->q, rc, cur, c->d_cnt);
+					else
+					{
+						rc.cam_rays = (it == 0 && seam.cam) ? 1 : 0;
+						hipLaunchKernelGGL(hk.plain, dim3(grid), dim3(JP_BLOCK), p.shade_lds_bytes, c->stream, p.sv, q, rc, cur, c->d_cnt);
+						rc.cam_rays = 0;
+					}
 				}
 				HIP_TRY(hipGetLastError());
 				if (it < rp->max_depth || p.has_null_material)
 				{
 					Stamper t(c, CLS_SHADOW);
 					if (sk.cert_fell_back) c->cert_fell_back = true;
-					if (sk.refill) hipLaunchKernelGGL(sk.refill, dim3(grid), dim3(JP_BLOCK), sk.lds, c->stream, p.sv, c->q, rc, sk.words, c->d_spill, c->d_cnt);
-					else hipLaunchKernelGGL(sk.plain, dim3(grid), dim3(JP_BLOCK), sk.lds, c->stream, p.sv, c->q, rc, sk.words, c->d_cnt);
+					if (sk.refill) hipLaunchKernelGGL(sk.refill, dim3(grid), dim3(JP_BLOCK), sk.lds, c->stream, p.sv, q, rc, sk.words, c->d_spill, c->d_cnt);
+					else hipLaunchKernelGGL(sk.plain, dim3(grid), dim3(JP_BLOCK), sk.lds, c->stream, p.sv, q, rc, sk.words, c->d_cnt);
 					HIP_TRY(hipGetLastError());
 				}
 				cur ^= 1;
 			}
-			{ Stamper t(c, CLS_OTHER); hipLaunchKernelGGL(k_resolve, dim3((unsigned int)std::min<long long>(c->n_cus * 8, (npix + JP_BLOCK - 1) / JP_BLOCK)), dim3(JP_BLOCK), 0, c->stream, c->q, rc, c->d_pix_acc, film_dev, s0 == 0 ? 1 : 0, s0 + rc.sbatch >= rp->spp ? 1 : 0); }
+			{ Stamper t(c, CLS_OTHER); hipLaunchKernelGGL(k_resolve, dim3((unsigned int)std::min<long long>(c->n_cus * 8, (npix + JP_BLOCK - 1) / JP_BLOCK)), dim3(JP_BLOCK), 0, c->stream, q, rc, c->d_pix_acc, film_dev, s0 == 0 ? 1 : 0, s0 + rc.sbatch >= rp->spp ? 1 : 0); }
 			samples += (unsigned long long)rc.sbatch * (unsigned long long)npix;
 		}
 		HIP_TRY(hipGetLastError());
diff --git a/jet-pbrt_amd/csrc/jp_runtime.h b/jet-pbrt_amd/csrc/jp_runtime.h
--- a/jet-pbrt_amd/csrc/jp_runtime.h
+++ b/jet-pbrt_amd/csrc/jp_runtime.h
@@ -18,6 +18,7 @@
 		{ "JETPBRT_PLOC_RADIUS", 0, &o.ploc_radius, 0 }, { "JETPBRT_PLOC_MAX_ROUNDS", 0, &o.ploc_max_rounds, 0 }, { "JETPBRT_CERTIFIED", 1, &o.certified, 0 },
 		{ "JETPBRT_CERT_SLACK", 7, &o.cert_slack, 0 }, { "JETPBRT_CERT_SLACK_EYE", 7, &o.cert_slack_eye, 0 }, { "JETPBRT_CERT_EYE", 7, &o.cert_eye_tau, 0 },
 		{ "JETPBRT_SINCOSF", 2, &o.libm_sincosf, 0 }, { "JETPBRT_LIBM", 2, &o.libm_xbsdf, 0 },
+		{ "JETPBRT_SEAMS_OFF", 0, &o.reserved[0], 0 },
 		{ "JETPBRT_TRACE_BINARY", 5, &o.trace_walk, 1 }, { "JETPBRT_TRACE_WIDE", 5, &o.trace_walk, 2 }, { "JETPBRT_TRACE_VERBATIM", 5, &o.trace_walk, 3 }, { "JETPBRT_BOX_PAD", 7, &o.box_pad, 0 },
 	};
 	for (const Item& it : items)
@@ -61,7 +62,7 @@
 	ScenePlan plan;
 	void *d_flat = nullptr, *d_wide = nullptr, *d_q4 = nullptr;
 	void* d_refbox = nullptr; bool cert_fell_back = false; int cert_eye_leaves = 0;
-	void *d_nodes = nullptr, *d_prims = nullptr, *d_meta = nullptr, *d_mats = nullptr, *d_mat_type = nullptr, *d_lights = nullptr, *d_shade_tab = nullptr;
+	void *d_nodes = nullptr, *d_prims = nullptr, *d_meta = nullptr, *d_mats = nullptr, *d_mat_type = nullptr, *d_lights = nullptr, *d_shade_tab = nullptr, *d_prim_class = nullptr;
 	int sincosf_mode = 0, libm_mode = 0;
 	bool build_on_device = false; float build_ms = 0.f; int bvh_height = 0, bvh_nodes = 0;
 	Queues q = {}; unsigned int cap = 0; int planes_alloc = 0; unsigned int blk_alloc = 0; int blocks_per_cu = 16;
@@ -91,7 +92,7 @@
 
 static void free_scene(JpContext* c)
 {
-	void** ps[] = { &c->d_flat, &c->d_wide, &c->d_q4, &c->d_refbox, &c->d_nodes, &c->d_prims, &c->d_meta, &c->d_mats, &c->d_mat_type, &c->d_lights, &c->d_shade_tab,
+	void** ps[] = { &c->d_flat, &c->d_wide, &c->d_q4, &c->d_refbox, &c->d_nodes, &c->d_prims, &c->d_meta, &c->d_mats, &c->d_mat_type, &c->d_lights, &c->d_shade_tab, &c->d_prim_class,
 	                &c->d_tex_desc, &c->d_tex_col, &c->d_texels, &c->d_mat_tex, &c->d_prim_uv };
 	for (void** p : ps) { if (*p) hipFree(*p); *p = nullptr; }
 	c->plan.have_scene = false;
diff --git a/jet-pbrt_amd/csrc/jp_upload.h b/jet-pbrt_amd/csrc/jp_upload.h
--- a/jet-pbrt_amd/csrc/jp_upload.h
+++ b/jet-pbrt_amd/csrc/jp_upload.h
@@ -580,6 +580,12 @@
 	HIP_TRY(up(&c->d_mats, mats.data(), mats.size() * sizeof(float4)));
 	HIP_TRY(up(&c->d_mat_type, mtype.data(), mtype.size() * sizeof(int)));
 	HIP_TRY(up(&c->d_lights, lights.data(), lights.size() * sizeof(float4)));
+	if (!device_build)
+	{
+		std::vector<int> pclass(std::max<size_t>(1, meta.size()), 0);
+		for (size_t pi = 0; pi < meta.size(); pi++) pclass[pi] = meta[pi].y >= 0 ? 1 + mtype[meta[pi].y] : 0;
+		HIP_TRY(up(&c->d_prim_class, pclass.data(), pclass.size() * sizeof(int)));
+	}
 	{
 		std::vector<float4> tabv;
 		tabv.insert(tabv.end(), lights.begin(), lights.begin() + 2 * (size_t)s->n_lights);
@@ -615,6 +621,7 @@
 	v.prims = (const float4*)c->d_prims; v.meta = (const int4*)c->d_meta; v.n_prims = (int)nmeta;
 	v.mats = (const float4*)c->d_mats; v.mat_type = (const int*)c->d_mat_type; v.n_mats = s->n_materials;
 	v.lights = (const float4*)c->d_lights; v.n_lights = s->n_lights; v.shade_tab = (const float4*)c->d_shade_tab;
+	v.prim_class = (const int*)c->d_prim_class;
 	v.env_sum = make_float3(envsum[0], envsum[1], envsum[2]); v.n_env = nenv;
 	v.world_radius = s->world_radius; v.cam = s->camera;
 	v.flat = (const float4*)c->d_flat; v.n_flat = (int)(flat.size() / 2);
@@ -654,6 +661,7 @@
 		if (op.persist != 0) p.persist = op.persist < 0 ? 0 : op.persist;
 		p.vote = opt_flag(op.vote, p.trav_mode != 5 || p.cert);
 		p.class_mask = 1; for (int k = 0; k < 5; k++) if (kinds[k]) p.class_mask |= 2 << k;
+		v.class_mask = p.class_mask;
 		p.shade_sort = opt_flag(op.shade_sort, nk > 1);
 	}
 	p.has_null_material = hasNull; c->cert_fell_back = false;
```
